# bad-samaritan/Polmux

Measured on AMD Instinct MI355X. Metric: dual-pol Gsample/s through SSFM+Rx-DSP, higher is better.
Workload: dtype f64

## Files before the change

include/polmux_hip.h:

```cpp
#ifndef POLMUX_HIP_H
#define POLMUX_HIP_H

#include <stddef.h>
#include <stdint.h>

#ifdef __cplusplus
extern "C" {
#endif

#define PLX_OK 0
#define PLX_ERR_HIP (-1)
#define PLX_ERR_ARG (-2)
#define PLX_ERR_UNSUPPORTED (-3)
#define PLX_ERR_REFERENCE (-4)
#define PLX_ERR_TIMEOUT (-5)

const char *plx_last_error(void);
int plx_abi_version(void);
int plx_device_count(int *count);
int plx_set_device(int device);

int plx_release_all(void);
int plx_gateway_stats(int64_t *out);
int plx_gateway_stats_ex(int64_t *out, int n);

int plx_fastexp(const double *x, double *yr, double *yi, size_t count);
int plx_fastexp_dev(const double *d_x, double *d_y, size_t count, void *stream);

typedef struct plx_ssfm_desc {
    int64_t nfft;
    int32_t nfc;
    int32_t dual_pol;
    int32_t max_frames;
    int32_t fls[4];
    double dzmaxt;
    double dphimaxt;
    double alphalin;
    double length;
    int32_t nplates;
    int32_t manakov;
    const double *gam;
    const double *betat;
    const double *db1;
} plx_ssfm_desc;

typedef struct plx_ssfm plx_ssfm;

int plx_ssfm_create(plx_ssfm **plan, const plx_ssfm_desc *desc);
#define PLX_SSFM_SHARE_DEVICE 1u
#define PLX_SSFM_XPM_MANAKOV 2u
int plx_ssfm_create_ex(plx_ssfm **plan, const plx_ssfm_desc *desc, uint32_t flags);
typedef struct plx_ssfm_tuning {
    uint32_t size;
    int32_t no_fuse;
    int32_t short_rows;
    int32_t no_row_split;
    int32_t p1, logW;
    int32_t col_threads;
    int32_t rowr;
    int32_t rowsm;
    int32_t row256_split, row4k_split, rowg_split;
    int32_t no_pmd_tab;
    int32_t store_late;
    int32_t row_rev;
    int32_t safe_landing;
    int32_t reserved_[4];
    double barrier_timeout_ms;
} plx_ssfm_tuning;
int plx_ssfm_tuning_defaults(plx_ssfm_tuning *tuning);
int plx_ssfm_tuning_override(const plx_ssfm_tuning *tuning);
int plx_ssfm_create_tuned(plx_ssfm **plan, const plx_ssfm_desc *desc, uint32_t flags, const plx_ssfm_tuning *tuning);
int plx_ssfm_destroy(plx_ssfm *plan);
int plx_ssfm_set_birefringence(plx_ssfm *plan, const double *db0, const double *theta,
                               const double *epsilon, int nsets);
int plx_ssfm_set_birefringence_dev(plx_ssfm *plan, const double *db0, const double *theta,
                                   const double *epsilon, int nsets, void *stream);
int plx_ssfm_propagate_dev(plx_ssfm *plan, double *d_ux, double *d_uy, int nframes, void *stream);
int plx_ssfm_set_step_sequence(plx_ssfm *plan, const double *dz, int nsteps);
int plx_ssfm_log_steps(plx_ssfm *plan, int max_steps);
int plx_ssfm_step_sequence(plx_ssfm *plan, int frame, double *dz, int max_steps);
int plx_ssfm_results(plx_ssfm *plan, int nframes, double *firstdz, int32_t *ncycle);
int plx_ssfm_stats(plx_ssfm *plan, int64_t *row_pass_launches, int64_t *sample_steps);
int plx_ssfm_utilisation(plx_ssfm *plan, int64_t *frame_steps, int64_t *slots_listed, int64_t *slots_launched);
int plx_ssfm_info(plx_ssfm *plan, int32_t *info);
int plx_ssfm_barrier_timeouts(plx_ssfm *plan, int32_t *count, int rearm);
int plx_ssfm_profile(plx_ssfm *plan, int enable);
int plx_ssfm_kernel_times(plx_ssfm *plan, double *ms, int64_t *launches);

int plx_matrix_ssfm(double *uxr, double *uxi, double *uyr, double *uyi, const plx_ssfm_desc *desc,
                    const double *db0, const double *theta, const double *epsilon,
                    double *firstdz, int32_t *ncycle);
int plx_scalar_ssfm(double *ur, double *ui, const plx_ssfm_desc *desc, double *firstdz, int32_t *ncycle);
int plx_scalar_ssfm_adaptive(double *ur, double *ui, const plx_ssfm_desc *desc, int tolflag, double ltol,
                             double safety, double *firstdz, int32_t *ncycle, int32_t *nrej);

typedef struct plx_cde plx_cde;
int plx_cde_create(plx_cde **plan, int64_t fft_len, int64_t L, const double *H_interleaved);
int plx_cde_destroy(plx_cde *plan);
int plx_cde_apply_dev(plx_cde *plan, const double *d_x, double *d_y, int64_t nx, int nsig, void *stream);
int plx_cde_ofde(const double *xr, const double *xi, const double *yr, const double *yi, int64_t nx,
                 double fs, double lambda_ref, double span, double D, double S, int64_t fft_len,
                 int64_t L, double *oxr, double *oxi, double *oyr, double *oyi);

typedef struct plx_dbp_desc {
    int64_t nfft;
    int32_t max_frames;
    int32_t nspans;
    int32_t nsteps;
    int32_t manakov;
    double span_length;
    double alphalin;
    double gam;
    double xi;
    const double *betat;
    const double *dz;
} plx_dbp_desc;
typedef struct plx_dbp_plan plx_dbp_plan;
#define PLX_DBP_STREAMED 1u
int plx_dbp_create(plx_dbp_plan **plan, const plx_dbp_desc *desc, uint32_t flags);
int plx_dbp_destroy(plx_dbp_plan *plan);
int plx_dbp_apply_dev(plx_dbp_plan *plan, const double *d_in, double *d_out, int nframes, const double *d_scale, void *stream);
int plx_dbp(const double *xr, const double *xi, const double *yr, const double *yi, int64_t nx, const plx_dbp_desc *desc,
            double scale, double *oxr, double *oxi, double *oyr, double *oyi);

int plx_cmaadaptivefilter(const double *xr, const double *xi, int32_t Mdim, double *h1r, double *h1i,
                          double *h2r, double *h2i, double Ntap, double mu, const double *R, double sps,
                          double *yr, double *yi);
int plx_easiadaptivefilter(const double *xr, const double *xi, int32_t Mdim, double *h1r, double *h1i,
                           double *h2r, double *h2i, double Ntap, double mu, double sps, double *yr,
                           double *yi);

int plx_cmaadaptivefilter_m(const double *xr, const double *xi, int32_t Mdim, double *h1r, double *h1i,
                            double *h2r, double *h2i, int32_t ntap, double mu, const double *R, double *yr, double *yi);
int plx_easiadaptivefilter_m(const double *xr, const double *xi, int32_t Mdim, double *h1r, double *h1i,
                             double *h2r, double *h2i, int32_t ntap, double mu, double *yr, double *yi);

int plx_cmapolardemux(const double *xr, const double *xi, int64_t L, int32_t taps, double mu, const double *R,
                      const double *M, double *yr, double *yi, double *h1r, double *h1i, double *h2r, double *h2i,
                      int32_t *passes);
int plx_easipolardemux(const double *xr, const double *xi, int64_t L, double mu, const double *M, int32_t mfile_twin,
                       double *yr, double *yi, double *h1r, double *h1i, double *h2r, double *h2i, int32_t *passes);

#define PLX_DEMUX_CMA 1
#define PLX_DEMUX_EASI 2
#define PLX_DEMUX_EASI_M 3
int plx_poldemux_dev(int method, const double *d_x, double *d_y, int64_t L, int nframes, int32_t taps,
                     double mu, const double *R , const double *d_M,
                     double *d_h, int32_t *d_passes, void *stream);

typedef struct plx_dsp_params {
    int32_t workatbaudrate;
    int32_t applynlr;
    double nlralpha;
    double power_mw;
    int32_t applypol;
    int32_t polmethod;
    double cma_R[2];
    double cma_mu;
    int32_t cma_taps;
    int32_t cma_txpolars;
    double cma_phizero;
    double easi_mu;
    int32_t easi_txpolars;
    double easi_phizero;
    int32_t modorder, freqavg, phasavg, poworder;
    int32_t cma_has_mat, easi_has_mat;
    double cma_mat[8], easi_mat[8];
    int32_t mfile_twins;
    int32_t reserved_;
} plx_dsp_params;

typedef struct plx_dsp plx_dsp;
int plx_dsp_create(plx_dsp **plan, int64_t Lin, int32_t ncol, int32_t max_frames, const plx_dsp_params *p);
int plx_dsp_destroy(plx_dsp *plan);
int plx_dsp_run_dev(plx_dsp *plan, const double *d_in, double *d_out, int nframes, void *stream);
int64_t plx_dsp_out_len(const plx_dsp *plan);

int plx_decide_count_dev(const double *d_sym, int64_t L, int32_t ncol, int nframes, const uint8_t *d_pat,
                         uint8_t *d_pat_hat, int64_t *d_err, void *stream);
int plx_decide_count_frames_dev(const double *d_sym, int64_t L, int32_t ncol, int nframes, const uint8_t *d_pat,
                                int64_t pat_frame_stride, uint8_t *d_pat_hat, int64_t *d_err, void *stream);

int plx_evm_dev(const double *d_sym, int64_t L, int32_t ncol, int nframes, double *d_evm, void *stream);

int plx_decide_count_dqpsk_dev(const double *d_sym, int64_t L, int32_t ncol, int nframes, const uint8_t *d_pat_rx,
                               int64_t pat_frame_stride, int64_t *d_err, void *stream);

int plx_ampliflat_dev(double *d_ux, double *d_uy, int64_t nfft, int32_t nfc, int nframes, double gain_lin,
                      const double *sigma, const double *d_noise, uint64_t seed, const int64_t *d_keys,
                      int32_t asex, int32_t asey, void *stream);

#define PLX_PHASE_TX 2
#define PLX_PHASE_LO 3
int plx_phase_noise_dev(double *d_ux, double *d_uy, int64_t stride, int64_t pitch, double sign, int64_t nfft,
                        int32_t nfc, int nframes, const double *sigma, uint64_t seed, const int64_t *d_keys,
                        int32_t tag, const double *d_phi_in, double *d_phi_out, double *d_work, void *stream);

int plx_wdm_mux_dev(const double *d_sx, const double *d_sy, double *d_ux, double *d_uy, int64_t nfft, int32_t nch,
                    int nframes, const int64_t *shift, void *stream);
int plx_wdm_select_dev(const double *d_ux, const double *d_uy, double *d_rx, double *d_ry, int64_t nfft, int32_t nch,
                       int nframes, const int64_t *shift, const int64_t *delay, void *stream);

typedef struct plx_front plx_front;
typedef struct plx_front_desc {
    int64_t nfft;
    int32_t dual_pol;
    int32_t max_frames;
    int32_t balanced;
    int32_t adcbits;
    int32_t decim;
    int32_t ntaps;
    const double *fir;
    const double *hopt_re, *hopt_im;
    const double *hel_re, *hel_im;
    const double *elo_re, *elo_im;
    double elo_scalar;
} plx_front_desc;
int plx_front_create(plx_front **plan, const plx_front_desc *desc);
int plx_front_destroy(plx_front *plan);
int64_t plx_front_out_len(const plx_front *plan);
int plx_front_run_dev(plx_front *plan, double *d_ux, double *d_uy, int nframes, const int64_t *shift,
                      double *d_out, void *stream);
int plx_front_run_lo_dev(plx_front *plan, double *d_ux, double *d_uy, int nframes, const int64_t *shift,
                         const double *d_lophase, double *d_out, void *stream);
int plx_rx_front(const double *xr, const double *xi, const double *yr, const double *yi, const plx_front_desc *desc,
                 const int64_t *shift, double *outr, double *outi, double *cur_r, double *cur_i);

typedef struct plx_filter plx_filter;
int plx_filter_create(plx_filter **plan, int64_t nfft, int max_signals, const double *h_re, const double *h_im);
int plx_filter_destroy(plx_filter *plan);
int plx_filter_apply_dev(plx_filter *plan, double *d_x, int nsignals, void *stream);

typedef struct plx_pmdinv plx_pmdinv;
int plx_pmdinv_create(plx_pmdinv **plan, int64_t nfft, int max_frames);
int plx_pmdinv_destroy(plx_pmdinv *plan);
int plx_pmdinv_set_link(plx_pmdinv *plan, int nfibers, const int32_t *ntrunk, const double *db0, const double *theta,
                        const double *epsilon, const double *lcorr, const double *betat, const double *db1,
                        const double *mat, int apply_gvd, int nsets);
int plx_pmdinv_apply_dev(plx_pmdinv *plan, double *d_ux, double *d_uy, int nframes, void *stream);
int plx_pmdinv_matrices(plx_pmdinv *plan, int frame, double *U, double *Uinv);

int plx_pick_dev(const double *d_in, double *d_out, int64_t n_in, int64_t n_out, int64_t offset,
                 int64_t stride, double scale, int nsig, int64_t out_pitch, void *stream);

#ifdef __cplusplus
}
#endif
#endif
```

polmux_amd/_abi.py:

```python
import ctypes as C
import os

_HERE = os.path.dirname(os.path.abspath(__file__))
LIB_PATH = os.path.join(_HERE, "lib", "libpolmux_hip.so")

PLX_OK = 0
PLX_ERR_HIP = -1
PLX_ERR_ARG = -2
PLX_ERR_UNSUPPORTED = -3
PLX_ERR_REFERENCE = -4
PLX_ERR_TIMEOUT = -5
PLX_SSFM_SHARE_DEVICE = 1
PLX_SSFM_XPM_MANAKOV = 2
PLX_DBP_STREAMED = 1
PLX_PHASE_TX = 2
PLX_PHASE_LO = 3


class PolmuxError(RuntimeError):
    def __init__(self, code, msg):
        super().__init__(msg)
        self.code = code


class SsfmDesc(C.Structure):
    _fields_ = [("nfft", C.c_int64), ("nfc", C.c_int32), ("dual_pol", C.c_int32), ("max_frames", C.c_int32),
                ("fls", C.c_int32 * 4), ("dzmaxt", C.c_double), ("dphimaxt", C.c_double),
                ("alphalin", C.c_double), ("length", C.c_double), ("nplates", C.c_int32),
                ("manakov", C.c_int32), ("gam", C.c_void_p), ("betat", C.c_void_p), ("db1", C.c_void_p)]


class SsfmTuning(C.Structure):
    _fields_ = [("size", C.c_uint32), ("no_fuse", C.c_int32), ("short_rows", C.c_int32), ("no_row_split", C.c_int32),
                ("p1", C.c_int32), ("logW", C.c_int32), ("col_threads", C.c_int32), ("rowr", C.c_int32), ("rowsm", C.c_int32),
                ("row256_split", C.c_int32), ("row4k_split", C.c_int32), ("rowg_split", C.c_int32), ("no_pmd_tab", C.c_int32),
                ("store_late", C.c_int32), ("row_rev", C.c_int32), ("safe_landing", C.c_int32), ("reserved_", C.c_int32 * 4),
                ("barrier_timeout_ms", C.c_double)]


class DspParams(C.Structure):
    _fields_ = [("workatbaudrate", C.c_int32), ("applynlr", C.c_int32), ("nlralpha", C.c_double),
                ("power_mw", C.c_double), ("applypol", C.c_int32), ("polmethod", C.c_int32),
                ("cma_R", C.c_double * 2), ("cma_mu", C.c_double), ("cma_taps", C.c_int32),
                ("cma_txpolars", C.c_int32), ("cma_phizero", C.c_double), ("easi_mu", C.c_double),
                ("easi_txpolars", C.c_int32), ("easi_phizero", C.c_double), ("modorder", C.c_int32),
                ("freqavg", C.c_int32), ("phasavg", C.c_int32), ("poworder", C.c_int32),
                ("cma_has_mat", C.c_int32), ("easi_has_mat", C.c_int32), ("cma_mat", C.c_double * 8),
                ("easi_mat", C.c_double * 8), ("mfile_twins", C.c_int32), ("reserved_", C.c_int32)]


class FrontDesc(C.Structure):
    _fields_ = [("nfft", C.c_int64), ("dual_pol", C.c_int32), ("max_frames", C.c_int32), ("balanced", C.c_int32),
                ("adcbits", C.c_int32), ("decim", C.c_int32), ("ntaps", C.c_int32), ("fir", C.c_void_p),
                ("hopt_re", C.c_void_p), ("hopt_im", C.c_void_p), ("hel_re", C.c_void_p), ("hel_im", C.c_void_p),
                ("elo_re", C.c_void_p), ("elo_im", C.c_void_p), ("elo_scalar", C.c_double)]


class DbpDesc(C.Structure):
    _fields_ = [("nfft", C.c_int64), ("max_frames", C.c_int32), ("nspans", C.c_int32), ("nsteps", C.c_int32),
                ("manakov", C.c_int32), ("span_length", C.c_double), ("alphalin", C.c_double), ("gam", C.c_double),
                ("xi", C.c_double), ("betat", C.c_void_p), ("dz", C.c_void_p)]


_vp, _i32, _i64, _dbl, _sz = C.c_void_p, C.c_int32, C.c_int64, C.c_double, C.c_size_t

SIGNATURES = {
    "plx_abi_version": [],
    "plx_device_count": [C.POINTER(C.c_int)],
    "plx_set_device": [C.c_int],
    "plx_release_all": [],
    "plx_gateway_stats": [_vp],
    "plx_gateway_stats_ex": [_vp, C.c_int],
    "plx_fastexp": [_vp, _vp, _vp, _sz],
    "plx_fastexp_dev": [_vp, _vp, _sz, _vp],
    "plx_ssfm_create": [C.POINTER(_vp), C.POINTER(SsfmDesc)],
    "plx_ssfm_create_ex": [C.POINTER(_vp), C.POINTER(SsfmDesc), C.c_uint32],
    "plx_ssfm_tuning_defaults": [C.POINTER(SsfmTuning)],
    "plx_ssfm_tuning_override": [C.POINTER(SsfmTuning)],
    "plx_ssfm_create_tuned": [C.POINTER(_vp), C.POINTER(SsfmDesc), C.c_uint32, C.POINTER(SsfmTuning)],
    "plx_ssfm_destroy": [_vp],
    "plx_ssfm_set_step_sequence": [_vp, _vp, C.c_int],
    "plx_ssfm_log_steps": [_vp, C.c_int],
    "plx_ssfm_step_sequence": [_vp, C.c_int, _vp, C.c_int],
    "plx_ssfm_set_birefringence": [_vp, _vp, _vp, _vp, C.c_int],
    "plx_ssfm_set_birefringence_dev": [_vp, _vp, _vp, _vp, C.c_int, _vp],
    "plx_ssfm_propagate_dev": [_vp, _vp, _vp, C.c_int, _vp],
    "plx_ssfm_results": [_vp, C.c_int, _vp, _vp],
    "plx_ssfm_stats": [_vp, C.POINTER(_i64), C.POINTER(_i64)],
    "plx_ssfm_info": [_vp, _vp],
    "plx_ssfm_utilisation": [_vp, C.POINTER(_i64), C.POINTER(_i64), C.POINTER(_i64)],
    "plx_ssfm_barrier_timeouts": [_vp, C.POINTER(_i32), C.c_int],
    "plx_ssfm_profile": [_vp, C.c_int],
    "plx_ssfm_kernel_times": [_vp, _vp, _vp],
    "plx_matrix_ssfm": [_vp, _vp, _vp, _vp, C.POINTER(SsfmDesc), _vp, _vp, _vp, C.POINTER(_dbl),
                        C.POINTER(_i32)],
    "plx_scalar_ssfm": [_vp, _vp, C.POINTER(SsfmDesc), C.POINTER(_dbl), C.POINTER(_i32)],
    "plx_scalar_ssfm_adaptive": [_vp, _vp, C.POINTER(SsfmDesc), C.c_int, _dbl, _dbl, C.POINTER(_dbl), C.POINTER(_i32),
                                 C.POINTER(_i32)],
    "plx_cde_create": [C.POINTER(_vp), _i64, _i64, _vp],
    "plx_cde_destroy": [_vp],
    "plx_cde_apply_dev": [_vp, _vp, _vp, _i64, C.c_int, _vp],
    "plx_cde_ofde": [_vp, _vp, _vp, _vp, _i64, _dbl, _dbl, _dbl, _dbl, _dbl, _i64, _i64, _vp, _vp, _vp, _vp],
    "plx_dbp_create": [C.POINTER(_vp), C.POINTER(DbpDesc), C.c_uint32],
    "plx_dbp_destroy": [_vp],
    "plx_dbp_apply_dev": [_vp, _vp, _vp, C.c_int, _vp, _vp],
    "plx_dbp": [_vp, _vp, _vp, _vp, _i64, C.POINTER(DbpDesc), _dbl, _vp, _vp, _vp, _vp],
    "plx_cmaadaptivefilter": [_vp, _vp, _i32, _vp, _vp, _vp, _vp, _dbl, _dbl, _vp, _dbl, _vp, _vp],
    "plx_easiadaptivefilter": [_vp, _vp, _i32, _vp, _vp, _vp, _vp, _dbl, _dbl, _dbl, _vp, _vp],
    "plx_cmaadaptivefilter_m": [_vp, _vp, _i32, _vp, _vp, _vp, _vp, _i32, _dbl, _vp, _vp, _vp],
    "plx_easiadaptivefilter_m": [_vp, _vp, _i32, _vp, _vp, _vp, _vp, _i32, _dbl, _vp, _vp],
    "plx_cmapolardemux": [_vp, _vp, _i64, _i32, _dbl, _vp, _vp, _vp, _vp, _vp, _vp, _vp, _vp, _vp],
    "plx_easipolardemux": [_vp, _vp, _i64, _dbl, _vp, _i32, _vp, _vp, _vp, _vp, _vp, _vp, _vp],
    "plx_poldemux_dev": [C.c_int, _vp, _vp, _i64, C.c_int, _i32, _dbl, _vp, _vp, _vp, _vp, _vp],
    "plx_dsp_create": [C.POINTER(_vp), _i64, _i32, _i32, C.POINTER(DspParams)],
    "plx_dsp_destroy": [_vp],
    "plx_dsp_run_dev": [_vp, _vp, _vp, C.c_int, _vp],
    "plx_dsp_out_len": [_vp],
    "plx_decide_count_dev": [_vp, _i64, _i32, C.c_int, _vp, _vp, _vp, _vp],
    "plx_decide_count_frames_dev": [_vp, _i64, _i32, C.c_int, _vp, _i64, _vp, _vp, _vp],
    "plx_evm_dev": [_vp, _i64, _i32, C.c_int, _vp, _vp],
    "plx_decide_count_dqpsk_dev": [_vp, _i64, _i32, C.c_int, _vp, _i64, _vp, _vp],
    "plx_ampliflat_dev": [_vp, _vp, _i64, _i32, C.c_int, _dbl, _vp, _vp, C.c_uint64, _vp, _i32, _i32, _vp],
    "plx_phase_noise_dev": [_vp, _vp, _i64, _i64, _dbl, _i64, _i32, C.c_int, _vp, C.c_uint64, _vp, _i32, _vp, _vp, _vp,
                            _vp],
    "plx_wdm_mux_dev": [_vp, _vp, _vp, _vp, _i64, _i32, C.c_int, _vp, _vp],
    "plx_wdm_select_dev": [_vp, _vp, _vp, _vp, _i64, _i32, C.c_int, _vp, _vp, _vp],
    "plx_front_create": [C.POINTER(_vp), C.POINTER(FrontDesc)],
    "plx_front_destroy": [_vp],
    "plx_front_out_len": [_vp],
    "plx_front_run_dev": [_vp, _vp, _vp, C.c_int, _vp, _vp, _vp],
    "plx_front_run_lo_dev": [_vp, _vp, _vp, C.c_int, _vp, _vp, _vp, _vp],
    "plx_rx_front": [_vp, _vp, _vp, _vp, C.POINTER(FrontDesc), _vp, _vp, _vp, _vp, _vp],
    "plx_filter_create": [C.POINTER(_vp), _i64, C.c_int, _vp, _vp],
    "plx_filter_destroy": [_vp],
    "plx_filter_apply_dev": [_vp, _vp, C.c_int, _vp],
    "plx_pmdinv_create": [C.POINTER(_vp), _i64, C.c_int],
    "plx_pmdinv_destroy": [_vp],
    "plx_pmdinv_set_link": [_vp, C.c_int, _vp, _vp, _vp, _vp, _vp, _vp, _vp, _vp, C.c_int, C.c_int],
    "plx_pmdinv_apply_dev": [_vp, _vp, _vp, C.c_int, _vp],
    "plx_pmdinv_matrices": [_vp, C.c_int, _vp, _vp],
    "plx_pick_dev": [_vp, _vp, _i64, _i64, _i64, _i64, _dbl, C.c_int, _i64, _vp],
}
_RESTYPES = {"plx_dsp_out_len": _i64, "plx_front_out_len": _i64}


class Binding:

    def __init__(self, path=None):
        path = path or LIB_PATH
        if not os.path.exists(path):
            raise PolmuxError(PLX_ERR_HIP,
                              "libpolmux_hip.so not found at %s: build it with "
                              "`python -c 'import __graft_entry__ as g; g.build()'` "
                              "(hipcc --offload-arch=gfx950); there is no CPU fallback" % path)
        self.path = path
        if os.path.basename(path) == "libpolmux_hip.so":
            import torch
        self.lib = C.CDLL(path)
        _BINDINGS.append(self)
        self.lib.plx_last_error.restype = C.c_char_p
        for name, args in SIGNATURES.items():
            fn = getattr(self.lib, name)
            fn.argtypes = args
            fn.restype = _RESTYPES.get(name, C.c_int)

    def tuning(self, **fields):
        t = SsfmTuning()
        self.call("plx_ssfm_tuning_defaults", C.byref(t))
        for k, v in fields.items():
            if k not in dict(SsfmTuning._fields_) or k in ("size", "reserved_"):
                raise KeyError("plx_ssfm_tuning has no field %r" % k)
            setattr(t, k, v)
        return t

    def last_error(self):
        return self.lib.plx_last_error().decode("utf-8", "replace")

    def call(self, name, *args):
        rc = getattr(self.lib, name)(*args)
        if rc != PLX_OK:
            raise PolmuxError(rc, self.last_error() or ("%s failed with code %d" % (name, rc)))
        return rc


_default = None
_BINDINGS = []


def bindings():
    return list(_BINDINGS)


def get():
    global _default
    if _default is None:
        _default = Binding()
    return _default
```

polmux_amd/csrc/ssfm_args.h:

```cpp
#pragma once
#include "plx_fft.h"
#include "plx_internal.h"

#define BRF_STRIDE 4

#ifdef PLX_EMU
#define ROWR_SYNC() __syncthreads()
#else
#define ROWR_SYNC() asm volatile("s_waitcnt lgkmcnt(0)" ::: "memory")
#endif

namespace plxs {

struct FrameCtl {
    double zprop, dz;
    double cur;
    double leff, att;
    double dz_miss;
    double firstdz;
    double dzb_first, dzb_last;
    int ntot, nmem, ntrunk;
    int started, last, ncycle;
    int pad_[7];
    int done;
};
static_assert(sizeof(FrameCtl) == 128 && offsetof(FrameCtl, done) == 124, "done is the last word of the last 16-byte piece");

struct SsfmArgs {
    cplx *ux, *uy;
    const double *betat_p, *db1_p;
    const cplx *tpass;
    const cplx *hmul;
    const cplx *umat;
    const cplx *tw1, *tw2;
    const cplx *ctab;
    const cplx *tw2c, *twmid;
    const double *gam;
    const double *brf;
    cplx *e1tab, *e2tab;
    double d1slope;
    int tmax;
    union {
        double *psum;
        cplx *stokes;
    };
    FrameCtl *ctl;
    unsigned long long *umax;
    int *ndone;
    const int *active;
    int *nactive;
    long long spin_ticks;
    unsigned long long *slots;
    int row_rev;
    int store_late;
    int safe_land;
    int round;
    int *grab;
    unsigned long long *mbox;
    int mbox_stride;
    int p1, p2, nfc, dual, W, logW, T, logT, R, logR;
    int spm, xpm, manakov, pmd, nplates, brf_per_frame;
    int nframes;
    int force;
    double f_cur, f_leff, f_sc;
    const double *dzlist;
    int ndz, logcap;
    double *dzlog;
    int resume, ncycle0;
    double dz0, zdone0;
    double alphalin, Lf, dzmax, dphimax, lcorr, invN;
};

__device__ __forceinline__ double wave_max(double v)
{
    for (int m = 32; m >= 1; m >>= 1) {
        double o = __shfl_xor(v, m, 64);
        v = o > v ? o : v;
    }
    return v;
}

template <class ARGS> __device__ __forceinline__ bool all_done_or_aborted(const ARGS &a) { return a.ndone[0] >= a.nframes || a.ndone[1] != 0; }

__device__ __forceinline__ bool slot_frame(const SsfmArgs &a, int slot, int &f)
{
    if (!a.active) { f = slot; return slot < a.nframes; }
    if (slot >= a.nactive[0]) return false;
    f = a.active[slot];
    return true;
}

__device__ __forceinline__ bool row_slot(const SsfmArgs &a, int &slot)
{
    if (!a.row_rev) return true;
    const int n = a.active ? a.nactive[0] : a.nframes;
    if (slot >= n) return false;
    slot = n - 1 - slot;
    return true;
}

__device__ __forceinline__ void sincos_small(double a, double *s, double *c)
{
    if (fabs(a) < 0.0625) {
        const double z = a * a;
        double ps = fma(z, -1.0 / 39916800.0, 1.0 / 362880.0);
        ps = fma(z, ps, -1.0 / 5040.0);
        ps = fma(z, ps, 1.0 / 120.0);
        ps = fma(z, ps, -1.0 / 6.0);
        *s = fma(a * z, ps, a);
        double pc = fma(z, 1.0 / 479001600.0, -1.0 / 3628800.0);
        pc = fma(z, pc, 1.0 / 40320.0);
        pc = fma(z, pc, -1.0 / 720.0);
        pc = fma(z, pc, 1.0 / 24.0);
        pc = fma(z, pc, -0.5);
        *c = fma(z, pc, 1.0);
    } else {
        sincos(a, s, c);
    }
}

__device__ __forceinline__ double div3(double x)
{
    const double c = 1.0 / 3.0;
    const double q = x * c;
    return fma(fma(-3.0, q, x), c, q);
}
__device__ __forceinline__ void sincos_taylor(double a, double *s, double *c)
{
    const double z = a * a;
    double ps = fma(z, 1.0 / 362880.0, -1.0 / 5040.0);
    ps = fma(z, ps, 1.0 / 120.0);
    ps = fma(z, ps, -1.0 / 6.0);
    *s = fma(a * z, ps, a);
    double pc = fma(z, 1.0 / 40320.0, -1.0 / 720.0);
    pc = fma(z, pc, 1.0 / 24.0);
    pc = fma(z, pc, -0.5);
    *c = fma(z, pc, 1.0);
}

__device__ __forceinline__ void block_atomic_max(double v, double *red, unsigned long long *dst, int tid, int nthr)
{
    v = wave_max(v);
    if ((tid & 63) == 0) red[tid >> 6] = v;
    __syncthreads();
    if (tid == 0) {
        double m = red[0];
        for (int w = 1; w < (nthr + 63) / 64; w++) m = red[w] > m ? red[w] : m;
        atomicMax(dst, (unsigned long long)__double_as_longlong(m));
    }
}

}
```

polmux_amd/csrc/ssfm_colx.hip:

```cpp
#include "ssfm_ctrl.h"
#include "ssfm_kernels.h"
using namespace plxs;

namespace {

__device__ __noinline__ double ctrl_head_call(const PLX_LDS_QUAL CtrlK *k, PLX_LDS_QUAL FrameCtl *rec, int count, double pmax, int f)
{
    if (!ctrl_head<true>(*k, f, *rec, true, pmax, count != 0)) return -1.0;
    return rec->leff;
}
__device__ __noinline__ void ctrl_tail_call(const PLX_LDS_QUAL CtrlK *k, PLX_LDS_QUAL FrameCtl *rec)
{
    ctrl_tail(*k, *rec);
}
__device__ __noinline__ void kerr_full_range(int j, int t, double gamleff, int manakov)
{
    PLX_DYN_LDS(lds);
    cplx *s = (cplx *)lds;
    for (int k = 0; k < 16; k++) {
        cplx X = s[((j + 16 * k) << 4) + t], Y = s[((j + 16 * k) << 4) + t + 8];
        const double P = X.x * X.x + X.y * X.y + Y.x * Y.x + Y.y * Y.y;
        const cplx nl = cexpi(-gamleff * P);
        X = cmul(X, nl);
        Y = cmul(Y, nl);
        if (!manakov) {
            const double s3 = 2 * (X.x * Y.y - X.y * Y.x);
            double sp, cp;
            sincos(gamleff * s3 / 3, &sp, &cp);
            const cplx xx = make_double2(cp * X.x + sp * Y.x, cp * X.y + sp * Y.y);
            const cplx yy = make_double2(cp * Y.x - sp * X.x, cp * Y.y - sp * X.y);
            X = xx; Y = yy;
        }
        s[((j + 16 * k) << 4) + t] = X;
        s[((j + 16 * k) << 4) + t + 8] = Y;
    }
}

__device__ __noinline__ void kerr_full_range_scalar(int j, int t, double gam, double leff)
{
    PLX_DYN_LDS(lds);
    cplx *s = (cplx *)lds;
    for (int k = 0; k < 16; k++) {
        const cplx X = s[((j + 16 * k) << 4) + t];
        const double pw = X.x * X.x + X.y * X.y;
        s[((j + 16 * k) << 4) + t] = cmul(X, cexpi(-gam * pw * leff));
    }
}

#define PLX_REC_SENTINEL 0x7fffffff
#ifdef PLX_EMU
__device__ __forceinline__ void glds16(const cplx *src, cplx *lds_wave_base, int lane) { lds_wave_base[lane] = *src; }
__device__ __forceinline__ void glds_rows(const cplx *src, size_t stride, cplx *lds_wave_base, int lane)
{
    for (int i = 0; i < 16; i++) glds16(src + i * stride, lds_wave_base + 64 * i, lane);
}
__device__ __forceinline__ void lds_barrier() { __syncthreads(); }
__device__ __forceinline__ int lds_peek(const int *p) { return *(const volatile int *)p; }
__device__ __forceinline__ void lds_settle() {}
__device__ __forceinline__ void emu_lockstep() { __syncthreads(); }
#else
__device__ __forceinline__ void glds16(const cplx *src, cplx *lds_wave_base, int)
{
    const unsigned lb = __builtin_amdgcn_readfirstlane((unsigned)(size_t)(__attribute__((address_space(3))) void *)lds_wave_base);
    asm volatile("s_mov_b32 m0, %1\n\ts_nop 0\n\tglobal_load_lds_dwordx4 %0, off" : : "v"(src), "s"(lb) : "memory", "m0");
}
__device__ __forceinline__ void glds_rows(const cplx *src, size_t stride, cplx *lds_wave_base, int)
{
    unsigned lb = __builtin_amdgcn_readfirstlane((unsigned)(size_t)(__attribute__((address_space(3))) void *)lds_wave_base);
    unsigned long long p = (unsigned long long)src;
    const unsigned long long st = (unsigned long long)stride * sizeof(cplx);
#define PLX_GLDS_STEP "s_mov_b32 m0, %1\n\ts_nop 0\n\tglobal_load_lds_dwordx4 %0, off\n\tv_lshl_add_u64 %0, %0, 0, %2\n\ts_add_u32 %1, %1, 0x400\n\t"
    asm volatile(PLX_GLDS_STEP PLX_GLDS_STEP PLX_GLDS_STEP PLX_GLDS_STEP PLX_GLDS_STEP PLX_GLDS_STEP PLX_GLDS_STEP PLX_GLDS_STEP
                 PLX_GLDS_STEP PLX_GLDS_STEP PLX_GLDS_STEP PLX_GLDS_STEP PLX_GLDS_STEP PLX_GLDS_STEP PLX_GLDS_STEP PLX_GLDS_STEP
                 : "+v"(p), "+s"(lb) : "s"(st) : "memory", "m0", "scc");
#undef PLX_GLDS_STEP
}
__device__ __forceinline__ void lds_barrier() { asm volatile("s_waitcnt lgkmcnt(0)\n\ts_barrier" ::: "memory"); }
__device__ __forceinline__ int lds_peek(const int *p)
{
    int v;
    asm volatile("ds_read_b32 %0, %1\n\ts_waitcnt lgkmcnt(0)" : "=v"(v) : "v"((unsigned)(size_t)(const __attribute__((address_space(3))) void *)p) : "memory");
    return v;
}
__device__ __forceinline__ void lds_settle() { asm volatile("s_waitcnt lgkmcnt(0)" ::: "memory"); }
__device__ __forceinline__ void emu_lockstep() {}
#endif


template <bool D> __global__ __launch_bounds__(256, 2) void k_colx16(SsfmArgs a, int tiles_x, int tiles_pf)
{
    constexpr int CW = D ? 8 : 16;
    PLX_DYN_LDS(lds);
    if (all_done_or_aborted(a)) return;
    const int tid = threadIdx.x, t = tid & 15, j = tid >> 4;
    const int N2 = 1 << a.p2;
    const int LOGN = a.p1 + a.p2;
    cplx *s = (cplx *)lds;
    cplx *tw = s + 4096;
    double *red = (double *)(tw + 128);
    FrameCtl *lctl = (FrameCtl *)(red + 32);
    lds_load_twiddles(tw, a.tw1, 128, tid, 256);
    cplx *const fld = (D && t >= 8) ? a.uy : a.ux;
    const int round = a.round;
    const int colt = D ? t & 7 : t;
    const bool isx = !D || t < 8;
    const int lane = tid & 63, row0 = (tid >> 6) * 64;
    const int nact = a.nactive[0];
    const int NT = gridDim.x / tiles_pf, team = blockIdx.x / tiles_pf, ti = blockIdx.x - team * tiles_pf;
    const int c = ti / tiles_x, bx = ti - c * tiles_x;
    const unsigned long long rtag = (unsigned long long)(((unsigned)round + 1u) & 0xfffffu) << 22;
    unsigned long long *const mbox = a.mbox + (size_t)a.mbox_stride * team;
    if (blockIdx.x == 0 && tid == 0) a.grab[(round & 1) ^ 1] = 0;
    auto post = [&](int k) {
        const int sl = NT + atomicAdd(a.grab + (round & 1), 1);
        const int fr = sl < nact ? a.active[sl] : -1;
        if (k < a.mbox_stride) st_agent(mbox + k, ((rtag | (unsigned long long)(k + 1)) << 22) | (unsigned long long)(fr + 1));
    };
    auto posted = [&](int k, unsigned long long v) -> bool { return (v >> 22) == (rtag | (unsigned long long)(k + 1)); };
    int it = 0;
    auto stage = [&](int f, int par) {
        const int fc = f * a.nfc + c;
        int lq = lane >> 4;
        pin(lq);
        const cplx *src = fld + ((size_t)fc << LOGN) + (size_t)bx * CW + colt + (size_t)(row0 + lq) * N2;
        FrameCtl *const rec = lctl + 4 * par + (tid >> 6);
        if (lane == (int)(offsetof(FrameCtl, done) / 16)) rec->done = PLX_REC_SENTINEL;
        lds_settle();
        glds_rows(src, (size_t)4 * N2, s + (size_t)row0 * 16, lane);
        static_assert(sizeof(FrameCtl) % 16 == 0, "the record travels as 16-byte pieces");
        int ln = lane;
        pin(ln);
        if (ln < (int)(sizeof(FrameCtl) / 16)) glds16((const cplx *)(a.ctl + f) + ln, (cplx *)rec, ln);
    };
    double *const gaml = (double *)((char *)(lctl + 8) + 128);
    for (int k = tid; k < a.nfc; k += 256) gaml[k] = a.gam[k];
    cplx *const twn = (cplx *)(gaml + COLX_NFC);
    if (D && tid < 128) { const cplx w = a.tw1[tid]; twn[tid] = make_double2(-w.x, -w.y); }
#define COLX_TWA(tp) ((D && (tp) >= 8) ? (const cplx *)twn : (const cplx *)tw)
#define COLX_HSW(tp) ((D && (tp) >= 8) ? 2048 : 0)
    int f = team < nact ? a.active[team] : -1;
    if (f < 0) return;
    stage(f, 0);
    if (ti == 0 && tid == 64) post(1);
    CtrlK *const kk = (CtrlK *)(lctl + 8);
    if (tid == 0) {
        red[8] = -1.0;
        kk->dphimax = a.dphimax; kk->alphalin = a.alphalin; kk->dzmax = a.dzmax; kk->dz0 = a.dz0; kk->zdone0 = a.zdone0; kk->Lf = a.Lf; kk->lcorr = a.lcorr;
        kk->dual = a.dual ? 1 : 0; kk->resume = a.resume ? 1 : 0; kk->ncycle0 = a.ncycle0; kk->nfc = 0; kk->ndone = a.ndone; kk->umax = nullptr; kk->gam = nullptr;
        kk->dzlist = a.dzlist; kk->dzlog = a.dzlog; kk->ndz = a.ndz; kk->logcap = a.logcap;
    }
    auto settle = [&](int par) {
        const int pf = (int)red[8];
        if (pf < 0) return;
        FrameCtl *pr = lctl + 4 * par;
        if (!pr->done) ctrl_tail_call((const PLX_LDS_QUAL CtrlK *)kk, (PLX_LDS_QUAL FrameCtl *)pr);
        a.ctl[pf] = *pr;
        red[8] = -1.0;
    };
    __syncthreads();
    for (;; it++) {
        FrameCtl *const wrec = lctl + 4 * (it & 1) + (tid >> 6);
        const int fc = f * a.nfc + c;
        if (a.safe_land) drain_vmem();
        while (lds_peek(&wrec->done) == PLX_REC_SENTINEL) nap();
        emu_lockstep();
        if (wrec->done) {
            if (tid == 0) {
                settle((it & 1) ^ 1);
                unsigned long long v;
                unsigned spins = 0;
                bool dead = false;
                const long long t0 = plx_clock();
                while (!posted(it + 1, v = ld_agent(mbox + (it + 1)))) {
                    nap();
                    if ((++spins & 255u) == 0 && (ld_agent((const unsigned *)a.ndone + 1) != 0 || plx_clock() - t0 > a.spin_ticks)) {
                        st_agent((unsigned *)a.ndone + 1, 1u);
                        dead = true;
                        break;
                    }
                }
                red[10 + (it & 1)] = dead ? -2.0 : (double)((int)(v & 0x3fffffull) - 1);
            } else if (ti == 0 && tid == 64) {
                post(it + 2);
            }
            lds_barrier();
            f = (int)red[10 + (it & 1)];
            if (f == -2) return;
            if (f < 0) { it++; break; }
            stage(f, (it & 1) ^ 1);
            continue;
        }
        const size_t cbase = ((size_t)fc << LOGN) + (size_t)bx * CW + colt;
        const bool started = wrec->started != 0;
        {
            cplx x[16];
#pragma unroll
            for (int k = 0; k < 16; k++) x[k] = s[((16 * j + k) << 4) + t];
            if (started) {
                r16_dit(x);
#pragma unroll
                for (int k = 0; k < 16; k++) s[((16 * j + k) << 4) + t] = x[k];
            }
        }
        lds_barrier();
        cplx y[16];
        {
            int tp = t;
            pin(tp);
            const int ysw = started ? 0 : COLX_HSW(tp);
#pragma unroll
            for (int k = 0; k < 8; k++) y[k] = s[((j + 16 * k) << 4) + t + ysw];
#pragma unroll
            for (int k = 8; k < 16; k++) y[k] = s[((j + 16 * k) << 4) + t - ysw];
        }
        double sc = 1.0;
        if (started) {
            lvl2_dit256s(y, j, tw, COLX_TWA(t));
            sc = wrec->att * a.invN;
        }
#pragma unroll
        for (int k = 0; k < 16; k++) y[k] = cscale(y[k], sc);
        double m = 0;
        if (!D) {
#pragma unroll
            for (int k = 0; k < 16; k++) m = fmax(fma(y[k].y, y[k].y, y[k].x * y[k].x), m);
        } else
#pragma unroll
        for (int k = 0; k < 8; k++) {
            const double po = fma(y[k].y, y[k].y, y[k].x * y[k].x);
            const double pq = fma(y[k + 8].y, y[k + 8].y, y[k + 8].x * y[k + 8].x);
            const double p = po + lane_xchg<8>(pq);
            m = fmax(p, m);
        }
        m = wave_max(m);
        if ((tid & 63) == 0) red[tid >> 6] = m;
        lds_barrier();
        if (tid < 64) {
            const unsigned par = (unsigned)round & 1u;
            unsigned long long *slots = a.slots + ((size_t)par * a.nframes + f) * tiles_pf;
            double mm = red[0];
            for (int w = 1; w < 4; w++) mm = red[w] > mm ? red[w] : mm;
            const unsigned long long mine = (unsigned long long)__double_as_longlong(mm);
            if (tid == 0) {
                st_agent(slots + ti, mine);
                st_agent(a.slots + ((size_t)(par ^ 1u) * a.nframes + f) * tiles_pf + ti, ~0ull);
                settle((it & 1) ^ 1);
            }
            double pm;
            unsigned long long mv = 0;
            unsigned spins = 0;
            bool dead = false;
            const long long t0 = plx_clock();
            for (;;) {
                bool all = true;
                pm = -INFINITY;
                if (tid == 0) { mv = ld_agent(mbox + (it + 1)); all = posted(it + 1, mv); }
                int i0 = tid;
                pin(i0);
                for (int i = i0; i < tiles_pf; i += 64) {
                    const unsigned long long b = (i == ti) ? mine : ld_agent(slots + i);
                    if (b == ~0ull) all = false;
                    else { const double gp = gaml[i / tiles_x] * __longlong_as_double((long long)b); pm = gp > pm ? gp : pm; }
                }
                if (__all(all)) break;
                nap();
                if ((++spins & 255u) == 0) {
                    const int late = ld_agent((const unsigned *)a.ndone + 1) != 0 || plx_clock() - t0 > a.spin_ticks;
                    if (__any(late)) { dead = true; break; }
                }
            }
            pm = wave_max(pm);
            if (tid == 0) {
                red[10 + (it & 1)] = (double)((int)(mv & 0x3fffffull) - 1);
                if (dead) {
                    st_agent((unsigned *)a.ndone + 1, 1u);
                    red[19] = 1.0;
                } else {
                    const double pv = ctrl_head_call((const PLX_LDS_QUAL CtrlK *)kk, (PLX_LDS_QUAL FrameCtl *)wrec, ti == 0, pm, f);
                    if (ti == 0) red[8] = (double)f;
                    red[16] = pv; red[17] = pv < 0 ? 1.0 : 0.0; red[18] = mm; red[19] = 0.0;
                }
            }
        } else if (ti == 0 && tid == 64) {
            post(it + 2);
        }
        lds_barrier();
        if (red[19] != 0.0) return;
        const double leff = red[16];
        const bool finished = red[17] != 0.0;
        if (finished) {
            const int nf = (int)red[10 + (it & 1)];
            if (nf >= 0) stage(nf, (it & 1) ^ 1);
            {
                int tq = t, jq = j;
                pin(tq);
                pin(jq);
                const int rsw = (D && tq >= 8) ? 128 : 0;
#pragma unroll
                for (int k = 0; k < 8; k++) fld[cbase + (size_t)(jq + 16 * k + rsw) * N2] = y[k];
#pragma unroll
                for (int k = 8; k < 16; k++) fld[cbase + (size_t)(jq + 16 * k - rsw) * N2] = y[k];
            }
        } else {
            if (!D) {
                if (a.spm) {
                    const double gam = gaml[c];
                    if (fabs(gam * leff) * red[18] < 0.0625) {
#pragma unroll
                        for (int k = 0; k < 16; k++) {
                            const double pw = y[k].x * y[k].x + y[k].y * y[k].y;
                            double sn, cs;
                            sincos_taylor(-gam * pw * leff, &sn, &cs);
                            y[k] = cmul(y[k], make_double2(cs, sn));
                        }
                    } else {
#pragma unroll
                        for (int k = 0; k < 16; k++) s[((j + 16 * k) << 4) + t] = y[k];
                        lds_barrier();
                        kerr_full_range_scalar(j, t, gam, leff);
                        lds_barrier();
#pragma unroll
                        for (int k = 0; k < 16; k++) y[k] = s[((j + 16 * k) << 4) + t];
                        lds_barrier();
                    }
                }
            } else if (a.spm) {
                const double gamleff = gaml[c] * leff;
                int tq = t;
                pin(tq);
                const double sgn = tq < 8 ? 1.0 : -1.0, sgn2 = tq < 8 ? 2.0 : -2.0;
                if (fabs(gamleff) * red[18] < 0.0625) {
                    auto kerr16 = [&](auto cn) {
                        constexpr bool CNLSE = decltype(cn)::value;
#pragma unroll
                        for (int k = 0; k < 8; k++) {
                            const cplx own = y[k], snd = y[k + 8];
                            const cplx oth = make_double2(lane_xchg<8>(snd.x), lane_xchg<8>(snd.y));
                            const double P = fma(own.y, own.y, own.x * own.x) + fma(oth.y, oth.y, oth.x * oth.x);
                            double sn, cs;
                            sincos_taylor(-gamleff * P, &sn, &cs);
                            const cplx nl = make_double2(cs, sn);
                            cplx A = cmul(own, nl), B = cmul(oth, nl);
                            if (CNLSE) {
                                const double s3 = sgn2 * __dsub_rn(__dmul_rn(A.x, B.y), __dmul_rn(A.y, B.x));
                                double sp, cp;
                                sincos_taylor(div3(gamleff * s3), &sp, &cp);
                                const double sg = sgn * sp, ng = -sg;
                                const cplx A2 = make_double2(cp * A.x + sg * B.x, cp * A.y + sg * B.y);
                                B = make_double2(cp * B.x + ng * A.x, cp * B.y + ng * A.y);
                                A = A2;
                            }
                            const cplx back = make_double2(lane_xchg<8>(B.x), lane_xchg<8>(B.y));
                            y[k] = A;
                            y[k + 8] = back;
                            sched_fence();
                        }
                    };
                    if (a.manakov) kerr16(std::false_type{}); else kerr16(std::true_type{});
                } else {
                    int tp = t;
                    pin(tp);
                    const int ksw = COLX_HSW(tp);
#pragma unroll
                    for (int k = 0; k < 8; k++) s[((j + 16 * k) << 4) + t + ksw] = y[k];
#pragma unroll
                    for (int k = 8; k < 16; k++) s[((j + 16 * k) << 4) + t - ksw] = y[k];
                    lds_barrier();
                    if (isx) kerr_full_range(j, t, gamleff, a.manakov);
                    lds_barrier();
#pragma unroll
                    for (int k = 0; k < 8; k++) y[k] = s[((j + 16 * k) << 4) + t + ksw];
#pragma unroll
                    for (int k = 8; k < 16; k++) y[k] = s[((j + 16 * k) << 4) + t - ksw];
                    lds_barrier();
                }
            }
            lvl2_dif256s(y, j, tw, COLX_TWA(t));
#pragma unroll
            for (int k = 0; k < 16; k++) s[((j + 16 * k) << 4) + t] = y[k];
            lds_barrier();
            cplx x[16];
#pragma unroll
            for (int k = 0; k < 16; k++) x[k] = s[((16 * j + k) << 4) + t];
            lds_barrier();
            {
                const int nf = (int)red[10 + (it & 1)];
                if (nf >= 0) stage(nf, (it & 1) ^ 1);
            }
            r16_dif(x);
            if (a.store_late) {
                const int nf = (int)red[10 + (it & 1)];
                if (nf >= 0) {
                    FrameCtl *const nrec = lctl + 4 * ((it & 1) ^ 1) + (tid >> 6);
                    while (lds_peek(&nrec->done) == PLX_REC_SENTINEL) nap();
                }
            }
#pragma unroll
            for (int k = 0; k < 16; k++) fld[cbase + (size_t)(16 * j + k) * N2] = x[k];
        }
        f = (int)red[10 + (it & 1)];
        if (f < 0) { it++; break; }
    }
    if (tid == 0) settle((it & 1) ^ 1);
}


}

namespace plxs {
colx_kernel_t colx16_kernel(bool dual) { return dual ? (colx_kernel_t)k_colx16<true> : (colx_kernel_t)k_colx16<false>; }
}
```

polmux_amd/csrc/ssfm_ctrl.h:

```cpp
#pragma once
#include "ssfm_args.h"

namespace plxs {

template <bool AGENT, class ARGS, class REC> __device__ __forceinline__ bool ctrl_head(const ARGS &a, int f, REC &c, bool have_pmax, double pmax_in, bool count = true)
{
    if (c.started) {
        if (a.dual) c.ntot = c.ntot + c.ntrunk - c.nmem;
        if (c.last) {
            c.done = 1;
            if (count) atomicAdd(a.ndone, 1);
            return false;
        }
    }
    double Pmax = -INFINITY;
    if (have_pmax) {
        Pmax = pmax_in;
    } else {
        for (int k = 0; k < a.nfc; k++) {
            unsigned long long *up = a.umax + f * a.nfc + k;
            const unsigned long long bits = AGENT ? ld_agent(up) : *up;
            double Umax = __longlong_as_double((long long)bits);
            double gp = a.gam[k] * Umax;
            Pmax = gp > Pmax ? gp : Pmax;
            if (AGENT) st_agent(up, 0ull); else *up = 0ull;
        }
    }
    double leffn = a.dphimax / Pmax;
    double dl = a.alphalin * leffn;
    double dz;
    if (dl >= 1) {
        dz = a.dzmax;
    } else {
        double step = (a.alphalin == 0) ? leffn : -1 / a.alphalin * log(1 - dl);
        dz = step > a.dzmax ? a.dzmax : step;
    }
    {
        const int k = c.started ? c.ncycle : 0;
        if (a.dzlist && k < a.ndz) dz = a.dzlist[k];
        if (a.dzlog && count && k < a.logcap) a.dzlog[(size_t)f * a.logcap + k] = dz;
    }
    if (!c.started) {
        c.started = 1;
        if (a.resume) {
            dz = a.dz0;
            c.firstdz = a.zdone0;
            c.zprop = a.zdone0 + dz;
            c.ncycle = a.ncycle0 + 1;
        } else {
            c.firstdz = dz;
            c.zprop = dz;
            c.ncycle = 1;
        }
    } else {
        c.zprop = c.zprop + dz;
        c.ncycle = c.ncycle + 1;
    }
    c.dz = dz;
    if (c.zprop < a.Lf) {
        c.cur = dz; c.last = 0;
    } else {
        c.cur = a.Lf - c.zprop + dz; c.last = 1;
    }
    c.leff = (a.alphalin == 0) ? c.cur : (1 - exp(-a.alphalin * c.cur)) / a.alphalin;
    return true;
}
template <class ARGS, class REC> __device__ __forceinline__ void ctrl_tail(const ARGS &a, REC &c)
{
    const double zc = c.last ? a.Lf : c.zprop;
    c.att = exp(-(0.5 * a.alphalin) * c.cur);
    if (a.dual) {
        const double lcorr = a.lcorr;
        int nzc = (int)ceil(zc / lcorr);
        if (c.dz_miss == 0) {
            c.nmem = 0;
            c.ntrunk = nzc - c.ntot;
            double dzlast = c.cur - lcorr * (c.ntrunk - 1);
            c.dzb_first = c.ntrunk > 1 ? lcorr : dzlast;
            c.dzb_last = dzlast;
            c.dz_miss = lcorr - dzlast;
        } else {
            c.nmem = 1;
            c.ntrunk = nzc - c.ntot + 1;
            if (c.ntrunk == 1) {
                c.dzb_first = c.cur; c.dzb_last = c.cur;
                c.dz_miss = c.dz_miss - c.cur;
            } else {
                double dzlast = c.cur - c.dz_miss - lcorr * (c.ntrunk - 2);
                c.dzb_first = c.dz_miss; c.dzb_last = dzlast;
                c.dz_miss = lcorr - dzlast;
            }
        }
    }
}
template <bool AGENT, class ARGS> __device__ __forceinline__ void ctrl_core(const ARGS &a, int f, FrameCtl &c, bool have_pmax, double pmax_in)
{
    if (c.done) return;
    if (ctrl_head<AGENT>(a, f, c, have_pmax, pmax_in)) ctrl_tail(a, c);
}
struct CtrlK {
    double dphimax, alphalin, dzmax, dz0, zdone0, Lf, lcorr;
    int dual, resume, ncycle0, nfc;
    int *ndone;
    unsigned long long *umax;
    const double *gam;
    const double *dzlist;
    double *dzlog;
    int ndz, logcap;
};
static_assert(sizeof(CtrlK) <= 128, "k_colx16 reserves 128 bytes of LDS for the constants");
template <bool AGENT> __device__ __forceinline__ void ctrl_step(const SsfmArgs &a, int f, bool have_pmax = false, double pmax_in = 0.0)
{
    FrameCtl c = a.ctl[f];
    if (c.done) return;
    ctrl_core<AGENT>(a, f, c, have_pmax, pmax_in);
    a.ctl[f] = c;
}

}
```

polmux_amd/csrc/ssfm_kernels.h:

```cpp
#pragma once
#include "ssfm_args.h"
#include <tuple>
#include <utility>

#define COMPACT_THREADS 256
#define COL_THREADS_MAX 1024
#define ROW_THREADS 128
#define ROWR_THREADS 64
#define ROWR_LDS ((4 * 272 + 128 + 48) * sizeof(cplx))
#define ROWR_LDS_SC ((4 * 272 + 128 + 80) * sizeof(cplx))
#define ROWG_THREADS 256
#define ROWG_NTW(M) ((M) <= 1024 ? (M) / 2 : (M) / 8 + 4)
#define ROWG_LDS(M) ((size_t)((ROWG_THREADS / ((M) / 16)) * ((M) + (M) / 16) + ROWG_NTW(M) + 7 * 16 + PLX_CTAB + 17 * (ROWG_THREADS / ((M) / 16))) * sizeof(cplx))
#define ROWG_LDS_SPLIT(M) (ROWG_LDS(M) - (size_t)((ROWG_THREADS / ((M) / 16)) * ((M) + (M) / 16)) * sizeof(double))
#define ROWSM_LDS ((size_t)64 * 17 * sizeof(double) + (7 * 16 + PLX_CTAB) * sizeof(cplx))
#define COLX_NFC 64

namespace plxs {

typedef void (*sweep_kernel_t)(SsfmArgs);
typedef void (*colx_kernel_t)(SsfmArgs, int, int);

PLX_HIDDEN sweep_kernel_t col_fwd_kernel();
PLX_HIDDEN sweep_kernel_t col_fwd_xpm_kernel();
PLX_HIDDEN sweep_kernel_t col_inv_kernel();
PLX_HIDDEN colx_kernel_t colx16_kernel(bool dual);
PLX_HIDDEN sweep_kernel_t row_kernel();
PLX_HIDDEN sweep_kernel_t row256_kernel(bool pmd, bool scalar, bool split);
PLX_HIDDEN sweep_kernel_t row4k_kernel(bool pair, bool split);
PLX_HIDDEN sweep_kernel_t rowreg_kernel(int logm, bool pair, bool scalar, bool split);
PLX_HIDDEN sweep_kernel_t rowsm_kernel(int logm, bool scalar);

PLX_HIDDEN void launch_umax(dim3 grid, hipStream_t st, const SsfmArgs &a);
PLX_HIDDEN void launch_ctrl(int nframes, hipStream_t st, const SsfmArgs &a);
PLX_HIDDEN void launch_compact(const FrameCtl *ctl, int nframes, int *active, int *nactive, int serves, hipStream_t st);
PLX_HIDDEN void launch_rowsum(dim3 grid, hipStream_t st, const SsfmArgs &a);
PLX_HIDDEN void launch_stokes_sum(dim3 grid, hipStream_t st, const SsfmArgs &a);
PLX_HIDDEN void launch_pmd_tab(unsigned frames, hipStream_t st, const SsfmArgs &a);
PLX_HIDDEN void launch_nl_att(unsigned grid, hipStream_t st, cplx *u, const double *gam, size_t N, int nfc, int spm, int xpm, double leff, double att);
PLX_HIDDEN void launch_maxdiff(unsigned grid, hipStream_t st, const cplx *u, const cplx *uh, size_t n, unsigned long long *out);
PLX_HIDDEN void launch_richardson(unsigned grid, hipStream_t st, cplx *u, const cplx *uh, size_t n);

#ifndef PLX_EMU
namespace detail {
template <class... P, size_t... I> inline void launch_ptr(void (*k)(P...), dim3 g, dim3 b, size_t lds, hipStream_t st, std::tuple<P...> &v, std::index_sequence<I...>)
{
    void *ptrs[] = {(void *)&std::get<I>(v)...};
    (void)hipLaunchKernel((const void *)k, g, b, ptrs, lds, st);
}
}
template <class... P, class... A> inline void launch(void (*k)(P...), dim3 g, dim3 b, size_t lds, hipStream_t st, A &&...args)
{
    std::tuple<P...> v{P(std::forward<A>(args))...};
    detail::launch_ptr(k, g, b, lds, st, v, std::index_sequence_for<P...>{});
}
template <class K> inline hipError_t allow_lds(K kern, size_t bytes)
{
    return hipFuncSetAttribute((const void *)kern, hipFuncAttributeMaxDynamicSharedMemorySize, (int)bytes);
}
template <class K> inline int blocks_per_cu(K kern, int threads, size_t lds)
{
    int nb = 0;
    if (hipOccupancyMaxActiveBlocksPerMultiprocessor(&nb, (const void *)kern, threads, lds) != hipSuccess) return 0;
    return nb;
}
#else
template <class... P, class... A> inline void launch(void (*k)(P...), dim3 g, dim3 b, size_t lds, hipStream_t, A &&...args)
{
    std::tuple<P...> v{P(std::forward<A>(args))...};
    emu::launch(g, b, lds, [=]() { std::apply(k, v); });
}
template <class K> inline hipError_t allow_lds(K, size_t) { return hipSuccess; }
template <class K> inline int blocks_per_cu(K, int, size_t) { return 2; }
#endif

}
```

polmux_amd/csrc/ssfm_plan.h:

```cpp
#pragma once
#include "ssfm_kernels.h"
#include <vector>

using plxs::FrameCtl;
using plxs::SsfmArgs;

struct plx_ssfm {
    plx_ssfm_desc d;
    int p, p1, p2;
    size_t N;
    SsfmArgs a;
    double *d_betat = nullptr, *d_db1 = nullptr, *d_gam = nullptr, *d_brf = nullptr, *d_psum = nullptr;
    cplx *d_tpass = nullptr, *d_tw1 = nullptr, *d_tw2 = nullptr, *d_ctab = nullptr;
    FrameCtl *d_ctl = nullptr;
    unsigned long long *d_umax = nullptr;
    int *d_ndone = nullptr;
    int *h_ndone = nullptr;
    int *d_active = nullptr;
    hipEvent_t ev = nullptr;
    std::vector<FrameCtl> h_ctl;
    int brf_sets = 0;
    size_t lds_col = 0, lds_row = 0;
    cplx *d_e1 = nullptr, *d_e2 = nullptr;
    unsigned long long *d_slots = nullptr;
    unsigned long long *d_mbox = nullptr;
    size_t mbox_bytes = 0;
    int fused = 0, fused_grid = 0, tiles_pf = 0;
    uint32_t flags = 0;
    int xpm_dual = 0;
    int barrier_timeouts = 0;
    int calls_unfused = 0, rearm_after = 16;
    double *d_dzlist = nullptr, *d_dzlog = nullptr;
    int dzlist_cap = 0;
    int col_threads = 512;
    int row_threads = ROW_THREADS;
    int rowr = 0;
    int row4k_split = 0;
    int rowsm = 0;
    int row256_split = 0;
    int rowg_pair_split = 0;
    int rowg_split = 0;
    int rowreg = 0;
    cplx *d_tw2c = nullptr, *d_twmid = nullptr;
    int row_split = 0, rs_threads = 0;
    size_t rs_lds = 0;
    int tw_compact = 0;
    int row_pair4k = 0;
    size_t rs_lds_pair = 0;
    double *h_brf[2] = {nullptr, nullptr};
    hipEvent_t brf_ev[2] = {nullptr, nullptr};
    int brf_slot = 0;
    int64_t row_launches = 0, sample_steps = 0;
    int64_t slots_launched = 0, slots_listed = 0, frame_steps = 0;
    int profile = 0;
    struct ProfRun { std::vector<hipEvent_t> ev; std::vector<int> cls, step; int maxnc = 0; bool fused = false; };
    std::vector<hipEvent_t> evfree;
    std::vector<ProfRun> prof_pending;
    double k_ms[4] = {0, 0, 0, 0};
    int64_t k_launches[4] = {0, 0, 0, 0};
};

PLX_HIDDEN int plx_ssfm_linear_dev(plx_ssfm *P, const SsfmArgs &base, cplx *d_x, double dz, hipStream_t st);

static const double kInv2Pi = 0.15915494309189533577;
```

polmux_amd/csrc/ssfm_plan.hip:

```cpp
#include "ssfm_plan.h"
#include "ssfm_ctrl.h"
#include "plx_gateway.h"

#include <cmath>
#include <cstdlib>
#include <cstring>
#include <limits>
#include <vector>
using namespace plxs;

static int ilog2(int64_t v)
{
    int l = 0;
    while (((int64_t)1 << l) < v) l++;
    return l;
}

static void free_plan(plx_ssfm *P)
{
    if (!P) return;
    hipFree(P->d_betat); hipFree(P->d_db1); hipFree(P->d_gam); hipFree(P->d_brf); hipFree(P->d_psum);
    hipFree(P->d_tpass); hipFree(P->d_tw1); hipFree(P->d_tw2); hipFree(P->d_ctab); hipFree(P->d_ctl); hipFree(P->d_umax);
    hipFree(P->d_dzlist); hipFree(P->d_dzlog); hipFree(P->d_tw2c); hipFree(P->d_twmid);
    hipFree(P->d_ndone); hipFree(P->d_slots); hipFree(P->d_mbox); hipFree(P->d_active); hipFree(P->d_e1); hipFree(P->d_e2);
    if (P->h_ndone) hipHostFree(P->h_ndone);
    if (P->ev) hipEventDestroy(P->ev);
    for (hipEvent_t e : P->evfree) hipEventDestroy(e);
    for (auto &r : P->prof_pending) for (hipEvent_t e : r.ev) hipEventDestroy(e);
    for (int k = 0; k < 2; k++) {
        if (P->h_brf[k]) hipHostFree(P->h_brf[k]);
        if (P->brf_ev[k]) hipEventDestroy(P->brf_ev[k]);
    }
    delete P;
}

static void half_table(std::vector<cplx> &t, int M)
{
    t.resize(M / 2 > 0 ? M / 2 : 1);
    for (int k = 0; k < M / 2; k++) {
        long double ang = -2.0L * 3.14159265358979323846264338327950288L * (long double)k / (long double)M;
        t[k] = make_double2((double)cosl(ang), (double)sinl(ang));
    }
}


namespace {
plx_ssfm_tuning g_override;
bool g_have_override = false;
}

extern "C" int plx_ssfm_tuning_defaults(plx_ssfm_tuning *t)
{
    if (!t) PLX_FAIL(PLX_ERR_ARG, "plx_ssfm_tuning_defaults: null argument");
    std::memset(t, 0, sizeof(*t));
    t->size = (uint32_t)sizeof(*t);
    t->p1 = -1; t->logW = -1; t->col_threads = -1; t->store_late = -1;
    t->row_rev = 1; t->rowr = 1; t->rowsm = 1; t->row256_split = 1; t->row4k_split = 1; t->rowg_split = 1;
    t->barrier_timeout_ms = 500.0;
    if (const char *e = getenv("PLX_SSFM_NO_FUSE")) t->no_fuse = atoi(e);
    if (const char *e = getenv("PLX_SSFM_BARRIER_TIMEOUT_MS")) t->barrier_timeout_ms = atof(e);
    return PLX_OK;
}

extern "C" int plx_ssfm_tuning_override(const plx_ssfm_tuning *t)
{
    if (t && t->size != sizeof(plx_ssfm_tuning)) PLX_FAIL(PLX_ERR_ARG, "plx_ssfm_tuning_override: fill the struct with plx_ssfm_tuning_defaults first");
    g_have_override = t != nullptr;
    if (t) g_override = *t;
    return PLX_OK;
}

extern "C" int plx_ssfm_create(plx_ssfm **out, const plx_ssfm_desc *desc) { return plx_ssfm_create_tuned(out, desc, 0u, nullptr); }

extern "C" int plx_ssfm_create_ex(plx_ssfm **out, const plx_ssfm_desc *desc, uint32_t flags) { return plx_ssfm_create_tuned(out, desc, flags, nullptr); }

extern "C" int plx_ssfm_create_tuned(plx_ssfm **out, const plx_ssfm_desc *desc, uint32_t flags, const plx_ssfm_tuning *tuning)
{
    if (!out || !desc) PLX_FAIL(PLX_ERR_ARG, "plx_ssfm_create: null argument");
    if (flags & ~(uint32_t)(PLX_SSFM_SHARE_DEVICE | PLX_SSFM_XPM_MANAKOV)) PLX_FAIL(PLX_ERR_ARG, "plx_ssfm_create_ex: unknown flag");
    *out = nullptr;
    const int64_t N = desc->nfft;
    const int p = ilog2(N);
    if (N < 256 || ((int64_t)1 << p) != N || p > 20)
        PLX_FAIL(PLX_ERR_UNSUPPORTED, "plx_ssfm_create: nfft must be a power of two in [256, 2^20]");
    if (desc->nfc < 1 || desc->max_frames < 1) PLX_FAIL(PLX_ERR_ARG, "plx_ssfm_create: nfc and max_frames must be >= 1");
    if (!desc->gam || !desc->betat) PLX_FAIL(PLX_ERR_ARG, "plx_ssfm_create: gam and betat are required");
    const bool xpm_dual = desc->dual_pol && desc->fls[3] && desc->nfc > 1;
    if (xpm_dual && !((flags & PLX_SSFM_XPM_MANAKOV) && desc->manakov))
        PLX_FAIL(PLX_ERR_REFERENCE, "The CNLSE with separate fields is not yet implemented");
    if (desc->dual_pol && desc->fls[3] && desc->nfc == 1) {  }
    if (desc->nplates < 1) PLX_FAIL(PLX_ERR_ARG, "plx_ssfm_create: nplates must be >= 1");
    if (tuning && tuning->size != sizeof(plx_ssfm_tuning)) PLX_FAIL(PLX_ERR_ARG, "plx_ssfm_create_tuned: fill the struct with plx_ssfm_tuning_defaults first");
    plx_ssfm_tuning tune;
    if (tuning) tune = *tuning;
    else if (g_have_override) tune = g_override;
    else plx_ssfm_tuning_defaults(&tune);
    if (flags & PLX_SSFM_SHARE_DEVICE) tune.no_fuse = 1;
    if (xpm_dual) tune.no_fuse = 1;

    plx_ssfm *P = new plx_ssfm();
    P->d = *desc;
    P->flags = flags;
    P->p = p;
    int logW;
    {
        const int npol = desc->dual_pol ? 2 : 1;
        logW = desc->dual_pol ? 3 : 4;
        int p1 = 12 - (logW + (npol == 2 ? 1 : 0));
        const bool long_rows = !tune.no_row_split && !tune.short_rows;
        const int p2max = long_rows ? 12 : 11;
        if (p - p1 > p2max) p1 = p - p2max;
        if (p1 > p - 4) p1 = p - 4;
        if (p1 < 2) p1 = 2;
        while ((((size_t)1 << p1) << (logW + (npol == 2 ? 1 : 0))) * sizeof(cplx) > 128 * 1024 && logW > 3) logW--;
        if (tune.p1 >= 2 && tune.p1 <= p - 4) p1 = tune.p1;
        if (tune.logW >= 2 && tune.logW <= 6) logW = tune.logW;
        while (((int64_t)1 << (p - p1)) < ((int64_t)1 << logW)) logW--;
        P->p1 = p1;
    }
    P->p2 = p - P->p1;
    P->N = (size_t)N;
    const int N1 = 1 << P->p1, N2 = 1 << P->p2;
    const int nfc = desc->nfc, F = desc->max_frames;
    SsfmArgs &a = P->a;
    std::memset(&a, 0, sizeof(a));
    a.p1 = P->p1; a.p2 = P->p2; a.nfc = nfc; a.dual = desc->dual_pol ? 1 : 0;
    a.logW = logW; a.W = 1 << a.logW;
    a.logT = a.logW + (a.dual ? 1 : 0); a.T = 1 << a.logT;
    {
        int R = 1, npol = a.dual ? 2 : 1;
        while (R * npol * (N2 / 16) < ROW_THREADS / 2 && R * 2 <= N1) R *= 2;
        a.R = R; a.logR = ilog2(R);
        int rowthr = ROW_THREADS;
        const int64_t pts = (int64_t)npol * R * N2;
        while (rowthr < 1024 && (int64_t)rowthr * 8 < pts) rowthr *= 2;
        P->row_threads = rowthr;
    }
    P->tw_compact = P->p2 >= 12 ? 1 : 0;
    if (a.dual && (N2 >= 2048 && !tune.no_row_split)) {
        P->row_split = 1;
        P->rs_threads = N2 / 8 < ROW_THREADS ? ROW_THREADS : (N2 / 8 > 1024 ? 1024 : N2 / 8);
        P->rs_lds = ((size_t)(N2 + N2 / 16) + (P->tw_compact ? N2 / 8 + 4 + 16 + 160 + PLX_CTAB : N2 / 2)) * sizeof(cplx);
    }
    if (P->tw_compact && !a.dual && !tune.no_row_split) P->rs_lds = ((size_t)(N2 + N2 / 16) + N2 / 8 + 4 + 16 + 160 + PLX_CTAB) * sizeof(cplx);
    if (P->tw_compact && !P->row_split && a.dual) {
        free_plan(P);
        PLX_FAIL(PLX_ERR_UNSUPPORTED, "plx_ssfm_create: 4096-point rows need the one-polarisation row pass (PLX_SSFM_NO_ROW_SPLIT is set)");
    }
    if (P->tw_compact) {
        P->row_pair4k = desc->fls[1] ? 1 : 0;
        P->rs_lds_pair = P->rs_lds + (size_t)(N2 + N2 / 16) * sizeof(cplx);
    }
    a.spm = desc->fls[2]; a.xpm = desc->fls[3]; a.manakov = desc->manakov ? 1 : 0; a.pmd = desc->fls[1] ? 1 : 0;
    a.nplates = desc->nplates;
    a.alphalin = desc->alphalin; a.Lf = desc->length; a.dzmax = desc->dzmaxt; a.dphimax = desc->dphimaxt;
    a.lcorr = desc->length / desc->nplates;
    a.invN = 1.0 / (double)N;
    a.spin_ticks = (long long)(tune.barrier_timeout_ms * 1e5);
    a.safe_land = tune.safe_landing;
    a.row_rev = tune.row_rev;
    if ((int64_t)desc->max_frames + 4 >= ((int64_t)1 << 22)) { free_plan(P); PLX_FAIL(PLX_ERR_UNSUPPORTED, "plx_ssfm_create: max_frames must be below 2^22 - 4"); }

    std::vector<double> bt((size_t)nfc * N), d1;
    std::vector<cplx> tp((size_t)N);
    const bool have_db1 = desc->db1 != nullptr && a.dual;
    if (have_db1) d1.resize((size_t)nfc * N);
    for (int j = 0; j < N1; j++) {
        const unsigned k1 = plx_bitrev((unsigned)j, P->p1);
        for (int i = 0; i < N2; i++) {
            const unsigned k2 = plx_bitrev((unsigned)i, P->p2);
            const size_t k = (size_t)k1 + (size_t)N1 * k2, pos = (size_t)j * N2 + i;
            for (int c = 0; c < nfc; c++) {
                bt[(size_t)c * N + pos] = desc->betat[(size_t)c * N + k] * kInv2Pi;
                if (have_db1) d1[(size_t)c * N + pos] = desc->db1[(size_t)c * N + k] * kInv2Pi;
            }
            const uint64_t e = ((uint64_t)i * k1) & (uint64_t)(N - 1);
            long double ang = -2.0L * 3.14159265358979323846264338327950288L * (long double)e / (long double)N;
            tp[pos] = make_double2((double)cosl(ang), (double)sinl(ang));
        }
    }
    std::vector<cplx> t1, t2;
    half_table(t1, N1);
    if (P->tw_compact) {
        t2.resize(N2 / 8 + 4);
        for (int k = 0; k < N2 / 8 + 4; k++) {
            const int e = k < N2 / 8 ? 4 * k : k - N2 / 8;
            long double ang = -2.0L * 3.14159265358979323846264338327950288L * (long double)e / (long double)N2;
            t2[k] = make_double2((double)cosl(ang), (double)sinl(ang));
        }
    } else {
        half_table(t2, N2);
    }
    std::vector<double> gam(nfc);
    for (int c = 0; c < nfc; c++) gam[c] = (a.dual && a.manakov) ? desc->gam[c] * 8 / 9 : desc->gam[c];

#define UP(dst, vec, T)                                                                             \
    do {                                                                                            \
        if (hipMalloc((void **)&(dst), (vec).size() * sizeof(T)) != hipSuccess ||                   \
            hipMemcpy((dst), (vec).data(), (vec).size() * sizeof(T), hipMemcpyHostToDevice) != hipSuccess) { \
            free_plan(P);                                                                           \
            PLX_FAIL(PLX_ERR_HIP, "plx_ssfm_create: device allocation/upload failed");              \
        }                                                                                           \
    } while (0)
    UP(P->d_betat, bt, double);
    if (have_db1) UP(P->d_db1, d1, double);
    UP(P->d_tpass, tp, cplx);
    UP(P->d_tw1, t1, cplx);
    UP(P->d_tw2, t2, cplx);
    {
        std::vector<cplx> ctv(PLX_CTAB);
        for (int k = 0; k < PLX_CTAB; k++) {
            const long double ang = 2.0L * 3.14159265358979323846264338327950288L * (long double)k / (long double)PLX_CTAB;
            ctv[k] = make_double2((double)cosl(ang), (double)-sinl(ang));
        }
        UP(P->d_ctab, ctv, cplx);
    }
    const int rowsm_min = a.dual ? (tune.rowsm == 2 ? 5 : 7) : 5;
    if (tune.rowr && tune.rowsm && !desc->fls[1] && P->p2 >= rowsm_min && P->p2 <= 7 && (N1 * (a.dual ? 2 : 1)) % (64 / (N2 / 16)) == 0) {
        const long double tau = -2.0L * 3.14159265358979323846264338327950288L;
        std::vector<cplx> tm(7 * 16, make_double2(1.0, 0.0));
        const int R = N2 / 16;
        auto put = [&](int q, int j, int e, int m) { tm[16 * q + j] = make_double2((double)cosl(tau * e / m), (double)sinl(tau * e / m)); };
        for (int j = 0; j < 16; j++) {
            if (R == 2) put(0, j, j, 32);
            const int q0 = R == 8 ? 4 : 0;
            if (R >= 4) for (int q = 0; q < 3; q++) put(q0 + q, j, (q + 1) * j, 64);
            if (R == 8) for (int q = 0; q < 4; q++) put(q, j, j + 16 * q, 128);
        }
        UP(P->d_twmid, tm, cplx);
        if (allow_lds(rowsm_kernel(P->p2, !a.dual), ROWSM_LDS) == hipSuccess) P->rowsm = 1;
    }
    if (tune.rowr && P->p2 >= 9 && P->p2 <= 11 && N1 >= (ROWG_THREADS / (N2 / 16)) / (a.dual ? 2 : 1)) {
        const long double tau = -2.0L * 3.14159265358979323846264338327950288L;
        std::vector<cplx> tc(N2 / 8 + 4), tm(7 * 16, make_double2(1.0, 0.0));
        for (int k = 0; k < N2 / 8 + 4; k++) {
            const int e = k < N2 / 8 ? 4 * k : k - N2 / 8;
            tc[k] = make_double2((double)cosl(tau * e / N2), (double)sinl(tau * e / N2));
        }
        const int R = N2 / 256;
        auto put = [&](int q, int j, int e, int m) { tm[16 * q + j] = make_double2((double)cosl(tau * e / m), (double)sinl(tau * e / m)); };
        for (int j = 0; j < 16; j++) {
            if (R == 2) put(0, j, j, 32);
            const int q0 = R == 8 ? 4 : 0;
            if (R >= 4) for (int q = 0; q < 3; q++) put(q0 + q, j, (q + 1) * j, 64);
            if (R == 8) for (int q = 0; q < 4; q++) put(q, j, j + 16 * q, 128);
        }
        UP(P->d_tw2c, tc, cplx);
        UP(P->d_twmid, tm, cplx);
        const size_t lds_whole = ROWG_LDS((size_t)N2), lds_split = ROWG_LDS_SPLIT((size_t)N2);
        hipError_t e = allow_lds(rowreg_kernel(P->p2, false, false, false), lds_whole);
        if (e == hipSuccess) e = allow_lds(rowreg_kernel(P->p2, true, false, false), lds_whole);
        if (e == hipSuccess) e = allow_lds(rowreg_kernel(P->p2, false, true, false), lds_whole);
        if (e == hipSuccess) P->rowreg = 1;
        if (P->rowreg && tune.rowg_split) {
            if (allow_lds(rowreg_kernel(P->p2, false, !a.dual, true), lds_split) == hipSuccess) P->rowg_split = 1;
            if (P->rowg_split && a.dual && allow_lds(rowreg_kernel(P->p2, true, false, true), lds_split) == hipSuccess) P->rowg_pair_split = 1;
        }
    }
    UP(P->d_gam, gam, double);
#undef UP
    bool ok = hipMalloc((void **)&P->d_ctl, sizeof(FrameCtl) * F) == hipSuccess &&
              hipMalloc((void **)&P->d_umax, sizeof(unsigned long long) * F * nfc) == hipSuccess &&
              hipMalloc((void **)&P->d_ndone, 64) == hipSuccess &&
              hipMalloc((void **)&P->d_active, sizeof(int) * (size_t)F) == hipSuccess &&
              hipHostMalloc((void **)&P->h_ndone, 64, hipHostMallocDefault) == hipSuccess &&
              hipEventCreateWithFlags(&P->ev, hipEventDisableTiming) == hipSuccess;
    if (ok && !a.dual && a.xpm) ok = hipMalloc((void **)&P->d_psum, sizeof(double) * (size_t)F * N) == hipSuccess;
    P->xpm_dual = xpm_dual ? 1 : 0;
    if (ok && xpm_dual) ok = hipMalloc((void **)&P->d_psum, sizeof(double) * 4 * (size_t)F * N) == hipSuccess;
    if (!ok) { free_plan(P); PLX_FAIL(PLX_ERR_HIP, "plx_ssfm_create: device allocation failed"); }
    a.betat_p = P->d_betat; a.db1_p = P->d_db1; a.tpass = P->d_tpass; a.tw1 = P->d_tw1; a.tw2 = P->d_tw2; a.ctab = P->d_ctab; a.tw2c = P->d_tw2c; a.twmid = P->d_twmid;
    a.gam = P->d_gam; a.ctl = P->d_ctl; a.umax = P->d_umax; a.ndone = P->d_ndone; a.psum = P->d_psum;
    P->h_ctl.resize(F);

    P->lds_col = (((size_t)N1 << a.logT) + N1 / 2) * sizeof(cplx) + 32 * sizeof(double) + 8 * sizeof(FrameCtl) + 128 + COLX_NFC * sizeof(double) + 128 * sizeof(cplx);
    P->lds_row = ((size_t)(a.dual ? 2 : 1) * a.R * (N2 + N2 / 16) + N2 / 2) * sizeof(cplx);
    P->col_threads = P->lds_col > 80 * 1024 ? 1024 : 512;
    if (tune.col_threads == 128 || tune.col_threads == 256 || tune.col_threads == 512 || tune.col_threads == 1024) P->col_threads = tune.col_threads;
    if (allow_lds(colx16_kernel(true), P->lds_col) != hipSuccess || allow_lds(colx16_kernel(false), P->lds_col) != hipSuccess || allow_lds(col_fwd_kernel(), P->lds_col) != hipSuccess ||
        allow_lds(col_inv_kernel(), P->lds_col) != hipSuccess || (P->xpm_dual && allow_lds(col_fwd_xpm_kernel(), P->lds_col) != hipSuccess) ||
        (!P->tw_compact && allow_lds(row_kernel(), P->lds_row > P->rs_lds ? P->lds_row : P->rs_lds) != hipSuccess) ||
        (P->tw_compact && (allow_lds(row4k_kernel(false, false), P->rs_lds) != hipSuccess || allow_lds(row4k_kernel(true, false), P->rs_lds_pair) != hipSuccess ||
                           allow_lds(row4k_kernel(false, true), P->rs_lds) != hipSuccess))) {
        free_plan(P);
        PLX_FAIL(PLX_ERR_HIP, "plx_ssfm_create: cannot reserve LDS for the transform kernels");
    }
    P->row4k_split = (P->tw_compact && tune.row4k_split) ? 1 : 0;
    if (tune.rowr && a.dual && a.p1 == 8 && a.p2 == 8 && !P->row_split &&
        allow_lds(row256_kernel(a.pmd != 0, false, false), ROWR_LDS) == hipSuccess) P->rowr = 1;
    if (tune.rowr && !a.dual && a.p1 == 8 && a.p2 == 8 && allow_lds(row256_kernel(false, true, false), ROWR_LDS_SC) == hipSuccess) P->rowr = 1;
    if (P->rowr && a.dual && a.pmd && tune.row256_split && allow_lds(row256_kernel(true, false, true), ROWR_LDS) == hipSuccess) P->row256_split = 1;
    if (((a.dual && a.W == 8) || (!a.dual && a.W == 16 && !desc->fls[3])) && !tune.no_fuse && a.p1 == 8 && nfc <= COLX_NFC) {
        int ncu = 256;
        {
            int dev = 0, v = 0;
            if (hipGetDevice(&dev) == hipSuccess && hipDeviceGetAttribute(&v, hipDeviceAttributeMultiprocessorCount, dev) == hipSuccess && v > 0)
                ncu = v;
        }
        const int tiles_pf = nfc * (N2 / a.W);
        const int per_cu = blocks_per_cu(colx16_kernel(a.dual != 0), 256, P->lds_col);
        const int cap = ncu * per_cu;
        if (tiles_pf <= cap) {
            P->fused = 1;
            P->tiles_pf = tiles_pf;
            P->fused_grid = (cap / tiles_pf) * tiles_pf;
            a.store_late = tune.store_late >= 0 ? (tune.store_late ? 1 : 0) : (P->fused_grid > tiles_pf ? 1 : 0);
            const int mstride = F + 4;
            P->mbox_bytes = sizeof(unsigned long long) * ((size_t)mstride * (P->fused_grid / tiles_pf) + 1);
            if (hipMalloc((void **)&P->d_slots, sizeof(unsigned long long) * 2 * (size_t)F * tiles_pf) != hipSuccess ||
                hipMalloc((void **)&P->d_mbox, P->mbox_bytes) != hipSuccess) {
                free_plan(P);
                PLX_FAIL(PLX_ERR_HIP, "plx_ssfm_create: device allocation failed");
            }
            a.slots = P->d_slots;
            a.mbox = P->d_mbox;
            a.mbox_stride = mstride;
            a.grab = (int *)(P->d_mbox + (size_t)mstride * (P->fused_grid / tiles_pf));
        }
    }
    if (a.pmd && have_db1 && !tune.no_pmd_tab) {
        const double D = desc->db1[1] * kInv2Pi;
        bool lin = D != 0.0 && N >= 4;
        for (int c = 0; c < nfc && lin; c++)
            for (int64_t k = 0; k < N && lin; k++) {
                const double m = (double)(k < N / 2 ? k : k - N);
                if (fabs(desc->db1[(size_t)c * N + k] * kInv2Pi - D * m) > 4e-15 * fabs(D) * (double)N) lin = false;
            }
        if (lin) {
            const int tmax = (int)ceil(desc->dzmaxt / a.lcorr) + 2;
            const size_t n1 = (size_t)F * tmax * N1, n2 = (size_t)F * tmax * N2;
            if (tmax <= 64 && (n1 + n2) * sizeof(cplx) <= ((size_t)4 << 30)) {
                if (hipMalloc((void **)&P->d_e1, n1 * sizeof(cplx)) != hipSuccess || hipMalloc((void **)&P->d_e2, n2 * sizeof(cplx)) != hipSuccess) {
                    free_plan(P);
                    PLX_FAIL(PLX_ERR_HIP, "plx_ssfm_create: device allocation failed (trunk phasor tables)");
                }
                a.e1tab = P->d_e1; a.e2tab = P->d_e2; a.d1slope = D; a.tmax = tmax;
            }
        }
    }
    if (a.pmd && !a.dual) { free_plan(P); PLX_FAIL(PLX_ERR_ARG, "plx_ssfm_create: PMD needs a dual-polarisation plan"); }
    if (!a.pmd) {
        double z = 0;
        int rc = plx_ssfm_set_birefringence(P, &z, &z, &z, 1);
        if (rc) { free_plan(P); return rc; }
    }
    *out = P;
    return PLX_OK;
}

extern "C" int plx_ssfm_destroy(plx_ssfm *P)
{
    free_plan(P);
    return PLX_OK;
}

static int set_brf(plx_ssfm *P, const double *db0, const double *theta, const double *epsilon, int nsets, hipStream_t st,
                   bool wait)
{
    if (!P || !db0 || !theta || !epsilon) PLX_FAIL(PLX_ERR_ARG, "plx_ssfm_set_birefringence: null argument");
    if (nsets < 1 || (nsets != 1 && nsets > P->d.max_frames)) PLX_FAIL(PLX_ERR_ARG, "plx_ssfm_set_birefringence: more sets than frames");
    const int np = P->d.nplates;
    const size_t cap = (size_t)P->d.max_frames * np * BRF_STRIDE, cnt = (size_t)nsets * np * BRF_STRIDE;
    if (!P->d_brf) PLX_HIP(hipMalloc((void **)&P->d_brf, cap * sizeof(double)));
    const int slot = P->brf_slot;
    P->brf_slot ^= 1;
    if (!P->h_brf[slot]) {
        PLX_HIP(hipHostMalloc((void **)&P->h_brf[slot], cap * sizeof(double), hipHostMallocDefault));
        PLX_HIP(hipEventCreateWithFlags(&P->brf_ev[slot], hipEventDisableTiming));
    } else {
        PLX_HIP(hipEventSynchronize(P->brf_ev[slot]));
    }
    double *t = P->h_brf[slot];
    for (int sidx = 0; sidx < nsets; sidx++)
        for (int n = 0; n < np; n++) {
            const size_t i = (size_t)sidx * np + n;
            const double ct = cos(theta[i]), sn = sin(theta[i]), ce = cos(epsilon[i]), se = sin(epsilon[i]);
            const double r11x = ct * ce, r11y = -sn * se, r12x = -sn * ce, r12y = ct * se;
            const double r21x = sn * ce, r21y = ct * se, r22x = ct * ce, r22y = sn * se;
            double *m = &t[i * BRF_STRIDE];
            m[0] = (r11x * r11x + r11y * r11y) - (r12x * r12x + r12y * r12y);
            m[1] = (r11x * r21x + r11y * r21y) - (r12x * r22x + r12y * r22y);
            m[2] = (r11y * r21x - r11x * r21y) - (r12y * r22x - r12x * r22y);
            m[3] = db0[i] * kInv2Pi;
        }
    PLX_HIP(hipMemcpyAsync(P->d_brf, t, cnt * sizeof(double), hipMemcpyHostToDevice, st));
    PLX_HIP(hipEventRecord(P->brf_ev[slot], st));
    if (wait) PLX_HIP(hipStreamSynchronize(st));
    P->a.brf = P->d_brf;
    P->a.brf_per_frame = nsets > 1 ? 1 : 0;
    P->brf_sets = nsets;
    return PLX_OK;
}

extern "C" int plx_ssfm_set_birefringence(plx_ssfm *P, const double *db0, const double *theta,
                                          const double *epsilon, int nsets)
{
    return set_brf(P, db0, theta, epsilon, nsets, nullptr, true);
}

extern "C" int plx_ssfm_set_birefringence_dev(plx_ssfm *P, const double *db0, const double *theta,
                                              const double *epsilon, int nsets, void *stream)
{
    return set_brf(P, db0, theta, epsilon, nsets, (hipStream_t)stream, false);
}

static void launch_row(plx_ssfm *P, const SsfmArgs &a, unsigned FC, hipStream_t st)
{
    const int N1 = 1 << a.p1, N2 = 1 << a.p2;
    if (P->tw_compact && !a.dual) {
        if (P->row4k_split) launch(row4k_kernel(false, true), dim3((unsigned)N1 * FC), dim3(256), P->rs_lds - 4352 * sizeof(double), st, a);
        else launch(row4k_kernel(false, false), dim3((unsigned)N1 * FC), dim3(256), P->rs_lds, st, a);
        return;
    }
    if (P->tw_compact && a.dual && (a.pmd || a.umat)) {
        launch(row4k_kernel(true, false), dim3((unsigned)N1 * FC), dim3(512), P->rs_lds_pair, st, a);
        return;
    }
    if (P->rowsm && !a.pmd && !a.umat) {
        const dim3 g((unsigned)(N1 * (a.dual ? 2 : 1) / (64 / (N2 / 16))), FC), bs(64);
        launch(rowsm_kernel(a.p2, !a.dual), g, bs, ROWSM_LDS, st, a);
        return;
    }
    if (P->rowreg && !a.dual) {
        const dim3 g((unsigned)(N1 / (ROWG_THREADS / (N2 / 16))), FC), bs(ROWG_THREADS);
        if (P->rowg_split) launch(rowreg_kernel(a.p2, false, true, true), g, bs, ROWG_LDS_SPLIT((size_t)N2), st, a);
        else launch(rowreg_kernel(a.p2, false, true, false), g, bs, ROWG_LDS((size_t)N2), st, a);
        return;
    }
    if (P->rowreg && a.dual) {
        const unsigned gx = (unsigned)(N1 / ((ROWG_THREADS / (N2 / 16)) / 2));
        const dim3 g(gx, FC), bs(ROWG_THREADS);
        if (a.pmd && !a.umat && a.e1tab && P->rowg_split && P->rowg_pair_split)
            launch(rowreg_kernel(a.p2, true, false, true), g, bs, ROWG_LDS_SPLIT((size_t)N2), st, a);
        else if (a.pmd || a.umat)
            launch(rowreg_kernel(a.p2, true, false, false), g, bs, ROWG_LDS((size_t)N2), st, a);
        else if (P->rowg_split)
            launch(rowreg_kernel(a.p2, false, false, true), g, bs, ROWG_LDS_SPLIT((size_t)N2), st, a);
        else
            launch(rowreg_kernel(a.p2, false, false, false), g, bs, ROWG_LDS((size_t)N2), st, a);
        return;
    }
    if (P->row_split && a.dual && !a.pmd) {
        SsfmArgs b = a;
        b.dual = 0; b.R = 1; b.logR = 0;
        const dim3 gs((unsigned)N1, FC), bs((unsigned)P->rs_threads);
        if (P->tw_compact) {
            if (P->row4k_split) launch(row4k_kernel(false, true), dim3(gs.x * gs.y * 2u), dim3(256), P->rs_lds - 4352 * sizeof(double), st, b);
            else launch(row4k_kernel(false, false), dim3(gs.x * gs.y * 2u), dim3(256), P->rs_lds, st, b);
            return;
        }
        for (int pol = 0; pol < 2; pol++) {
            if (pol) b.ux = a.uy;
            launch(row_kernel(), gs, bs, P->rs_lds, st, b);
        }
        return;
    }
    if (P->rowr && !a.dual && !a.force && !a.hmul) {
        launch(row256_kernel(false, true, false), dim3(64u, FC), dim3(ROWR_THREADS), ROWR_LDS_SC, st, a);
        return;
    }
    if (P->rowr && a.dual && !a.force && !a.hmul && !a.umat) {
        if (a.pmd && P->row256_split && a.e1tab) launch(row256_kernel(true, false, true), dim3(128u, FC), dim3(ROWR_THREADS), ROWR_LDS - 4 * 272 * sizeof(double), st, a);
        else launch(row256_kernel(a.pmd != 0, false, false), dim3(128u, FC), dim3(ROWR_THREADS), ROWR_LDS, st, a);
        return;
    }
    launch(row_kernel(), dim3((unsigned)(N1 / a.R), FC), dim3((unsigned)P->row_threads), P->lds_row, st, a);
}

static int resolve_profiles(plx_ssfm *P)
{
    for (auto &r : P->prof_pending) {
        for (size_t i = 0; i + 1 < r.ev.size(); i++) {
            const int cls = r.cls[i], step = r.step[i];
            const bool active = (r.fused && cls == 0) ? step <= r.maxnc : step < r.maxnc;
            if (!active) continue;
            float ms = 0;
            PLX_HIP(hipEventElapsedTime(&ms, r.ev[i], r.ev[i + 1]));
            P->k_ms[cls] += ms;
            P->k_launches[cls]++;
        }
        for (hipEvent_t e : r.ev) P->evfree.push_back(e);
    }
    P->prof_pending.clear();
    return PLX_OK;
}

static int propagate_frames(plx_ssfm *P, cplx *d_ux, cplx *d_uy, int nframes, hipStream_t st)
{
    SsfmArgs a = P->a;
    const int nfc = a.nfc, N2 = 1 << a.p2;
    a.ux = d_ux;
    a.uy = d_uy;
    a.nframes = nframes;
    a.active = P->d_active;
    a.nactive = P->d_ndone + 2;
    unsigned FC = (unsigned)nframes * nfc;
    PLX_HIP(hipMemsetAsync(a.ctl, 0, sizeof(FrameCtl) * nframes, st));
    PLX_HIP(hipMemsetAsync(a.umax, 0, sizeof(unsigned long long) * FC, st));
    PLX_HIP(hipMemsetAsync(P->d_ndone, 0, 64, st));
    const bool fused = P->fused != 0;
    if (fused) {
        PLX_HIP(hipMemsetAsync(P->d_slots, 0xFF, sizeof(unsigned long long) * 2 * (size_t)nframes * P->tiles_pf, st));
        PLX_HIP(hipMemsetAsync(P->d_mbox, 0, P->mbox_bytes, st));
    } else {
        unsigned gx = (unsigned)((P->N + 255) / 256);
        if (gx > 64) gx = 64;
        launch_umax(dim3(gx, FC), st, a);
    }
    const dim3 blk(256);
    const dim3 bcol((unsigned)P->col_threads);
    const bool compact_every_step = nframes >= 64;
    int chunk = 4, steps = 0;
    const int kMaxSteps = 1 << 19;
    bool pending = false, aborted = false;
    struct ProfGuard {
        plx_ssfm *P;
        plx_ssfm::ProfRun run;
        ~ProfGuard() { for (hipEvent_t e : run.ev) P->evfree.push_back(e); }
    } guard{P, {}};
    plx_ssfm::ProfRun &run = guard.run;
    auto mark = [&](int cls, int step) -> int {
        if (!P->profile) return PLX_OK;
        hipEvent_t e;
        if (!P->evfree.empty()) { e = P->evfree.back(); P->evfree.pop_back(); }
        else PLX_HIP(hipEventCreate(&e));
        run.ev.push_back(e); run.cls.push_back(cls); run.step.push_back(step);
        PLX_HIP(hipEventRecord(e, st));
        return PLX_OK;
    };
#define PLX_MARK(cls, step) do { int rc_ = mark((cls), (step)); if (rc_) return rc_; } while (0)
    for (;;) {
        for (int sidx = 0; sidx < chunk; sidx++) {
            const dim3 gcol((unsigned)(N2 / a.W), FC);
            P->slots_launched += FC / nfc;
            if (fused) {
                const int tcx = (int)gcol.x, tct = (int)(gcol.x * FC);
                const dim3 gx((unsigned)(tct < P->fused_grid ? tct : P->fused_grid));
                if (compact_every_step || sidx == 0) {
                    PLX_MARK(3, steps + sidx);
                    launch_compact(a.ctl, nframes, P->d_active, P->d_ndone + 2, compact_every_step ? 1 : chunk, st);
                }
#ifdef PLX_EMU
                emu::g_concurrency = emu::starve_barriers() ? 1 : P->tiles_pf;
#endif
                a.round = steps + sidx;
                PLX_MARK(0, steps + sidx);
                launch(colx16_kernel(a.dual != 0), gx, blk, P->lds_col, st, a, tcx, P->tiles_pf);
#ifdef PLX_EMU
                emu::g_concurrency = 1;
#endif
                if (a.e1tab) {
                    PLX_MARK(3, steps + sidx);
                    launch_pmd_tab(FC / nfc, st, a);
                }
                PLX_MARK(1, steps + sidx);
                launch_row(P, a, FC, st);
                P->row_launches++;
                continue;
            }
            PLX_MARK(3, steps + sidx);
            launch_ctrl(nframes, st, a);
            if (compact_every_step || sidx == 0)
                launch_compact(a.ctl, nframes, P->d_active, P->d_ndone + 2, compact_every_step ? 1 : chunk, st);
            if (!a.dual && a.xpm) {
                unsigned gx = (unsigned)((P->N + 255) / 256);
                if (gx > 256) gx = 256;
                launch_rowsum(dim3(gx, (unsigned)nframes), st, a);
            }
            if (P->xpm_dual) {
                unsigned gx = (unsigned)((P->N + 255) / 256);
                if (gx > 256) gx = 256;
                launch_stokes_sum(dim3(gx, (unsigned)nframes), st, a);
            }
            if (a.e1tab) launch_pmd_tab(FC / nfc, st, a);
            PLX_MARK(0, steps + sidx);
            launch(P->xpm_dual ? col_fwd_xpm_kernel() : col_fwd_kernel(), gcol, bcol, P->lds_col, st, a);
            PLX_MARK(1, steps + sidx);
            launch_row(P, a, FC, st);
            PLX_MARK(2, steps + sidx);
            launch(col_inv_kernel(), gcol, bcol, P->lds_col, st, a);
            P->row_launches++;
        }
        PLX_MARK(3, steps + chunk);
        if (steps == 0 && !P->prof_pending.empty()) {
            const int rc_ = resolve_profiles(P);
            if (rc_) return rc_;
        }
        steps += chunk;
        if (pending) {
            PLX_HIP(hipEventSynchronize(P->ev));
            if (P->h_ndone[1]) { aborted = true; break; }
            if (P->h_ndone[0] >= nframes) break;
            const unsigned live = (unsigned)(nframes - P->h_ndone[0]) * nfc;
            if (live < FC) FC = live;
        }
        PLX_HIP(hipMemcpyAsync(P->h_ndone, P->d_ndone, 4 * sizeof(int), hipMemcpyDeviceToHost, st));
        PLX_HIP(hipEventRecord(P->ev, st));
        pending = true;
        if (chunk > 8) chunk = 4;
        else if (chunk < (compact_every_step ? 8 : 16)) chunk *= 2;
        if (steps > kMaxSteps) PLX_FAIL(PLX_ERR_HIP, "plx_ssfm_propagate_dev: step loop did not terminate");
    }
    PLX_HIP(hipMemcpyAsync(P->h_ctl.data(), a.ctl, sizeof(FrameCtl) * nframes, hipMemcpyDeviceToHost, st));
    PLX_HIP(hipMemcpyAsync(P->h_ndone, P->d_ndone, 4 * sizeof(int), hipMemcpyDeviceToHost, st));
    PLX_HIP(hipStreamSynchronize(st));
    P->slots_listed += P->h_ndone[3];
    if (aborted || P->h_ndone[1]) {
        P->barrier_timeouts++;
        P->fused = 0;
        PLX_FAIL(PLX_ERR_TIMEOUT, "plx_ssfm_propagate_dev: frame barrier timed out (the workgroups of a frame were not co-resident: "
                                  "another kernel holds the GPU); nothing was stored after the time-out and the field of this call is "
                                  "INVALID -- the plan now takes the barrier-free three-sweep step: restore the field and call again, "
                                  "or create such plans with plx_ssfm_create_ex(..., PLX_SSFM_SHARE_DEVICE)");
    }
    int maxnc = 0;
    for (int f = 0; f < nframes; f++) {
        P->frame_steps += P->h_ctl[f].ncycle + (fused ? 1 : 0);
        if (!P->h_ctl[f].done) PLX_FAIL(PLX_ERR_HIP, "plx_ssfm_propagate_dev: a frame did not reach the fibre end");
        P->sample_steps += (int64_t)P->h_ctl[f].ncycle * (int64_t)P->N * nfc;
        if (P->h_ctl[f].ncycle > maxnc) maxnc = P->h_ctl[f].ncycle;
    }
    if (!run.ev.empty()) {
        run.maxnc = maxnc; run.fused = fused;
        P->prof_pending.push_back(std::move(run));
        run.ev.clear();
    }
#undef PLX_MARK
    return PLX_OK;
}

extern "C" int plx_ssfm_propagate_dev(plx_ssfm *P, double *d_ux, double *d_uy, int nframes, void *stream)
{
    if (!P || !d_ux) PLX_FAIL(PLX_ERR_ARG, "plx_ssfm_propagate_dev: null argument");
    if (nframes < 1 || nframes > P->d.max_frames) PLX_FAIL(PLX_ERR_ARG, "plx_ssfm_propagate_dev: nframes out of range");
    if (P->a.dual && !d_uy) PLX_FAIL(PLX_ERR_ARG, "plx_ssfm_propagate_dev: dual-polarisation plan needs d_uy");
    if (P->a.brf_per_frame && P->brf_sets < nframes)
        PLX_FAIL(PLX_ERR_ARG, "plx_ssfm_propagate_dev: fewer birefringence sets than frames");
    P->slots_launched = 0; P->slots_listed = 0; P->row_launches = 0; P->sample_steps = 0; P->frame_steps = 0;
    const int rc = propagate_frames(P, (cplx *)d_ux, (cplx *)d_uy, nframes, (hipStream_t)stream);
    if (rc) return rc;
    PLX_HIP(hipGetLastError());
    return PLX_OK;
}

extern "C" int plx_ssfm_set_step_sequence(plx_ssfm *P, const double *dz, int nsteps)
{
    if (!P || nsteps < 0 || (nsteps > 0 && !dz)) PLX_FAIL(PLX_ERR_ARG, "plx_ssfm_set_step_sequence: bad argument");
    if (nsteps > P->dzlist_cap) {
        if (P->d_dzlist) { (void)hipFree(P->d_dzlist); P->d_dzlist = nullptr; P->dzlist_cap = 0; }
        PLX_HIP(hipMalloc((void **)&P->d_dzlist, sizeof(double) * (size_t)nsteps));
        P->dzlist_cap = nsteps;
    }
    if (nsteps > 0) PLX_HIP(hipMemcpy(P->d_dzlist, dz, sizeof(double) * (size_t)nsteps, hipMemcpyHostToDevice));
    P->a.dzlist = nsteps > 0 ? P->d_dzlist : nullptr;
    P->a.ndz = nsteps;
    return PLX_OK;
}

extern "C" int plx_ssfm_log_steps(plx_ssfm *P, int max_steps)
{
    if (!P || max_steps < 0) PLX_FAIL(PLX_ERR_ARG, "plx_ssfm_log_steps: bad argument");
    if (P->d_dzlog) { (void)hipFree(P->d_dzlog); P->d_dzlog = nullptr; }
    P->a.dzlog = nullptr; P->a.logcap = 0;
    if (max_steps > 0) {
        PLX_HIP(hipMalloc((void **)&P->d_dzlog, sizeof(double) * (size_t)max_steps * P->d.max_frames));
        P->a.dzlog = P->d_dzlog; P->a.logcap = max_steps;
    }
    return PLX_OK;
}

extern "C" int plx_ssfm_step_sequence(plx_ssfm *P, int frame, double *dz, int max_steps)
{
    if (!P || !dz || frame < 0 || frame >= P->d.max_frames || max_steps < 0) PLX_FAIL(PLX_ERR_ARG, "plx_ssfm_step_sequence: bad argument");
    if (!P->d_dzlog) PLX_FAIL(PLX_ERR_ARG, "plx_ssfm_step_sequence: no log (plx_ssfm_log_steps)");
    const int n = max_steps < P->a.logcap ? max_steps : P->a.logcap;
    PLX_HIP(hipMemcpy(dz, P->d_dzlog + (size_t)frame * P->a.logcap, sizeof(double) * (size_t)n, hipMemcpyDeviceToHost));
    return PLX_OK;
}

extern "C" int plx_ssfm_utilisation(plx_ssfm *P, int64_t *frame_steps, int64_t *slots_listed, int64_t *slots_launched)
{
    if (!P) PLX_FAIL(PLX_ERR_ARG, "plx_ssfm_utilisation: null plan");
    if (frame_steps) *frame_steps = P->frame_steps;
    if (slots_listed) *slots_listed = P->slots_listed;
    if (slots_launched) *slots_launched = P->slots_launched;
    return PLX_OK;
}

extern "C" int plx_ssfm_info(plx_ssfm *P, int32_t *info)
{
    if (!P || !info) PLX_FAIL(PLX_ERR_ARG, "plx_ssfm_info: null argument");
    info[0] = P->fused; info[1] = P->p1; info[2] = P->p2; info[3] = P->fused_grid; info[4] = P->tiles_pf;
    info[5] = P->col_threads; info[6] = (P->rowr || P->rowsm) ? ROWR_THREADS : P->rowreg ? ROWG_THREADS : (P->tw_compact ? (P->row_pair4k ? 512 : 256) : (P->row_split ? P->rs_threads : P->row_threads)); info[7] = (P->rowreg || P->rowsm) ? 2 : (P->row_pair4k ? 0 : ((P->tw_compact && !P->a.dual) ? 1 : P->row_split));
    return PLX_OK;
}

extern "C" int plx_ssfm_barrier_timeouts(plx_ssfm *P, int32_t *count, int rearm)
{
    if (!P) PLX_FAIL(PLX_ERR_ARG, "plx_ssfm_barrier_timeouts: null plan");
    if (count) *count = P->barrier_timeouts;
    if (rearm && !P->fused && P->fused_grid > 0 && P->tiles_pf > 0) { P->fused = 1; P->calls_unfused = 0; }
    return PLX_OK;
}

extern "C" int plx_ssfm_profile(plx_ssfm *P, int enable)
{
    if (!P) PLX_FAIL(PLX_ERR_ARG, "plx_ssfm_profile: null plan");
    P->profile = enable ? 1 : 0;
    return PLX_OK;
}

extern "C" int plx_ssfm_kernel_times(plx_ssfm *P, double *ms, int64_t *launches)
{
    if (!P || !ms || !launches) PLX_FAIL(PLX_ERR_ARG, "plx_ssfm_kernel_times: null argument");
    const int rc = resolve_profiles(P);
    if (rc) return rc;
    for (int k = 0; k < 4; k++) { ms[k] = P->k_ms[k]; launches[k] = P->k_launches[k]; P->k_ms[k] = 0; P->k_launches[k] = 0; }
    return PLX_OK;
}

int plx_ssfm_filter_table(plx_ssfm *P, const double *h_re, const double *h_im, cplx **d_out)
{
    if (!P || !h_re || !d_out) PLX_FAIL(PLX_ERR_ARG, "filter table: null argument");
    const int N1 = 1 << P->p1, N2 = 1 << P->p2;
    std::vector<cplx> h(P->N);
    for (int j = 0; j < N1; j++) {
        const unsigned k1 = plx_bitrev((unsigned)j, P->p1);
        for (int i = 0; i < N2; i++) {
            const size_t k = (size_t)k1 + (size_t)N1 * plx_bitrev((unsigned)i, P->p2);
            h[(size_t)j * N2 + i] = make_double2(h_re[k], h_im ? h_im[k] : 0.0);
        }
    }
    cplx *d = nullptr;
    if (hipMalloc((void **)&d, P->N * sizeof(cplx)) != hipSuccess ||
        hipMemcpy(d, h.data(), P->N * sizeof(cplx), hipMemcpyHostToDevice) != hipSuccess) {
        if (d) (void)hipFree(d);
        PLX_FAIL(PLX_ERR_HIP, "filter table: device allocation/upload failed");
    }
    *d_out = d;
    return PLX_OK;
}

void plx_ssfm_geometry(const plx_ssfm *P, int *p1, int *p2) { *p1 = P->p1; *p2 = P->p2; }

int plx_ssfm_filter_dev(plx_ssfm *P, cplx *d_ux, cplx *d_uy, const cplx *d_hmul, int nframes, void *stream, const cplx *d_umat)
{
    if (!P || !d_ux || (!d_hmul && !d_umat)) PLX_FAIL(PLX_ERR_ARG, "filter: null argument");
    if (d_umat && (!P->a.dual || P->a.nfc != 1)) PLX_FAIL(PLX_ERR_ARG, "filter: matrix tables need a dual-polarisation single-field plan");
    if (nframes < 1 || nframes > P->d.max_frames) PLX_FAIL(PLX_ERR_ARG, "filter: nframes outside [1, max_frames]");
    if (P->a.dual && !d_uy) PLX_FAIL(PLX_ERR_ARG, "filter: dual-polarisation plan needs d_uy");
    hipStream_t st = (hipStream_t)stream;
    SsfmArgs b = P->a;
    b.ux = d_ux; b.uy = d_uy; b.nframes = nframes; b.hmul = d_hmul; b.umat = d_umat;
    b.force = 1; b.spm = 0; b.xpm = 0; b.pmd = 0; b.f_cur = 0; b.f_leff = 0; b.f_sc = b.invN;
    const int N1 = 1 << b.p1, N2 = 1 << b.p2;
    const unsigned FC = (unsigned)nframes * b.nfc;
    PLX_HIP(hipMemsetAsync(P->d_ctl, 0, sizeof(FrameCtl) * nframes, st));
    PLX_HIP(hipMemsetAsync(P->d_ndone, 0, 64, st));
    const dim3 gcol((unsigned)(N2 / b.W), FC), grow((unsigned)(N1 / b.R), FC);
    launch(col_fwd_kernel(), gcol, dim3((unsigned)P->col_threads), P->lds_col, st, b);
    if (d_umat && !P->tw_compact && !P->rowreg) launch(row_kernel(), grow, dim3((unsigned)P->row_threads), P->lds_row, st, b);
    else launch_row(P, b, FC, st);
    launch(col_inv_kernel(), gcol, dim3((unsigned)P->col_threads), P->lds_col, st, b);
    PLX_HIP(hipGetLastError());
    return PLX_OK;
}

int plx_ssfm_linear_dev(plx_ssfm *P, const SsfmArgs &base, cplx *d_x, double dz, hipStream_t st)
{
    SsfmArgs b = base;
    b.ux = d_x; b.uy = nullptr; b.nframes = 1; b.hmul = nullptr; b.umat = nullptr;
    b.force = 1; b.spm = 0; b.xpm = 0; b.f_cur = dz; b.f_leff = 0; b.f_sc = b.invN;
    const unsigned FC = (unsigned)b.nfc;
    const dim3 gcol((unsigned)((1 << b.p2) / b.W), FC);
    launch(col_fwd_kernel(), gcol, dim3((unsigned)P->col_threads), P->lds_col, st, b);
    launch_row(P, b, FC, st);
    launch(col_inv_kernel(), gcol, dim3((unsigned)P->col_threads), P->lds_col, st, b);
    const hipError_t e = hipGetLastError();
    if (e != hipSuccess) PLX_FAIL(PLX_ERR_HIP, std::string("linear step: launch failed: ") + hipGetErrorString(e));
    return PLX_OK;
}

extern "C" int plx_ssfm_results(plx_ssfm *P, int nframes, double *firstdz, int32_t *ncycle)
{
    if (!P || nframes < 1 || nframes > P->d.max_frames) PLX_FAIL(PLX_ERR_ARG, "plx_ssfm_results: bad argument");
    for (int f = 0; f < nframes; f++) {
        if (firstdz) firstdz[f] = P->h_ctl[f].firstdz;
        if (ncycle) ncycle[f] = P->h_ctl[f].ncycle;
    }
    return PLX_OK;
}

extern "C" int plx_ssfm_stats(plx_ssfm *P, int64_t *row_pass_launches, int64_t *sample_steps)
{
    if (!P) PLX_FAIL(PLX_ERR_ARG, "plx_ssfm_stats: null plan");
    if (row_pass_launches) *row_pass_launches = P->row_launches;
    if (sample_steps) *sample_steps = P->sample_steps;
    return PLX_OK;
}
```

polmux_amd/csrc/ssfm_row.hip:

```cpp
#include "ssfm_pmd.h"
#include "ssfm_kernels.h"
using namespace plxs;

namespace {

#define ROW_CH 4
__global__ __launch_bounds__(1024) void k_row(SsfmArgs a)
{
    PLX_DYN_LDS(lds);
    if (all_done_or_aborted(a)) return;
    const int tid = threadIdx.x, nthr = blockDim.x;
    int slot = blockIdx.y / a.nfc;
    const int c = blockIdx.y - slot * a.nfc;
    if (!row_slot(a, slot)) return;
    int f;
    if (!slot_frame(a, slot, f)) return;
    const int fc = f * a.nfc + c;
    const FrameCtl *ctl = a.ctl + f;
    if (ctl->done) return;
    const int N2 = 1 << a.p2, R = a.R, TSp = row_pitch(N2);
    cplx *s = (cplx *)lds;
    cplx *tw = s + (size_t)(a.dual ? 2 : 1) * R * TSp;
    const int twn = N2 >> 1;
    const bool tw_one = twn <= nthr;
    cplx twv = make_double2(0, 0);
    if (tw_one) { if (tid < twn) twv = a.tw2[tid]; }
    else lds_load_twiddles(tw, a.tw2, twn, tid, nthr);
    const size_t N = (size_t)1 << (a.p1 + a.p2);
    const int j0 = blockIdx.x * R;
    const int nel = R << a.p2;
    cplx *const fx = a.ux;
    cplx *const fy = a.dual ? a.uy : a.ux;
    const size_t base = (size_t)fc * N + (size_t)j0 * N2;
    auto gofs = [&](int e) -> size_t { return base + e; };
    const size_t rowbase = (size_t)j0 * N2;
    const bool keep_tw = nel == nthr * ROW_CH;
    cplx tkeep[ROW_CH];
    const double *bt = a.betat_p + (size_t)c * N + rowbase;
    const bool fastmul = keep_tw && a.dual && !a.pmd && !a.umat && !a.hmul;
    double btk[ROW_CH];
    if (fastmul) {
#pragma unroll
        for (int k = 0; k < ROW_CH; k++) btk[k] = bt[row_lane_point(tid + k * nthr, N2)];
    }
    for (int e0 = tid; e0 < nel; e0 += nthr * ROW_CH) {
        cplx tv[ROW_CH], xv[ROW_CH], yv[ROW_CH];
#pragma unroll
        for (int k = 0; k < ROW_CH; k++) {
            const int e = row_lane_point(min(e0 + k * nthr, nel - 1), N2);
            tv[k] = a.tpass[rowbase + e];
            xv[k] = fx[gofs(e)];
            yv[k] = fy[gofs(e)];
        }
#pragma unroll
        for (int k = 0; k < ROW_CH; k++) { pin(tv[k]); pin(xv[k]); pin(yv[k]); }
#pragma unroll
        for (int k = 0; k < ROW_CH; k++) {
            const int el = e0 + k * nthr, e = row_lane_point(el, N2);
            tkeep[k] = tv[k];
            if (el < nel) {
                const int r = e >> a.p2, i = e & (N2 - 1);
                s[r * TSp + row_phys(i)] = cmul(xv[k], tv[k]);
                if (a.dual) s[(R + r) * TSp + row_phys(i)] = cmul(yv[k], tv[k]);
            }
        }
    }
    if (tw_one && tid < twn) tw[tid] = twv;
    __syncthreads();
    row_fft_dif(s, a.p2, a.logR + (a.dual ? 1 : 0), tw, tid, nthr);
    const double cur = a.force ? a.f_cur : ctl->cur;
    if (!a.dual) {
        for (int el = tid; el < nel; el += nthr) {
            const int e = row_lane_point(el, N2);
            const int o = (e >> a.p2) * TSp + row_phys(e & (N2 - 1));
            s[o] = cmul(s[o], a.hmul ? a.hmul[rowbase + e] : cexp_neg_turns(bt[e] * cur));
        }
    } else if (!a.pmd) {
        if (a.umat) {
            for (int el = tid; el < nel; el += nthr) {
            const int e = row_lane_point(el, N2);
                const int o = (e >> a.p2) * TSp + row_phys(e & (N2 - 1));
                const cplx *um = a.umat + 3 * ((size_t)f * N + rowbase + e);
                const cplx u11 = um[0], u12 = um[1], hg = um[2], x = s[o], y = s[o + R * TSp];
                s[o] = cmulc(csub(cmulc(x, u11), cmul(u12, y)), hg);
                s[o + R * TSp] = cmulc(cadd(cmulc(x, u12), cmul(u11, y)), hg);
            }
        } else if (a.hmul) {
            for (int el = tid; el < nel; el += nthr) {
            const int e = row_lane_point(el, N2);
                const int o = (e >> a.p2) * TSp + row_phys(e & (N2 - 1));
                const cplx h = a.hmul[rowbase + e];
                s[o] = cmul(h, s[o]);
                s[o + R * TSp] = cmul(h, s[o + R * TSp]);
            }
        } else if (fastmul) {
#pragma unroll
            for (int k = 0; k < ROW_CH; k++) {
                const int e = row_lane_point(tid + k * nthr, N2);
                const int o = (e >> a.p2) * TSp + row_phys(e & (N2 - 1));
                const cplx h = cexp_neg_turns(btk[k] * cur);
                s[o] = cmul(h, s[o]);
                s[o + R * TSp] = cmul(h, s[o + R * TSp]);
            }
        } else {
            for (int el = tid; el < nel; el += nthr) {
            const int e = row_lane_point(el, N2);
                const int o = (e >> a.p2) * TSp + row_phys(e & (N2 - 1));
                const cplx h = cexp_neg_turns(bt[e] * cur);
                s[o] = cmul(h, s[o]);
                s[o + R * TSp] = cmul(h, s[o + R * TSp]);
            }
        }
    } else {
        const double *d1 = a.db1_p + (size_t)c * N + rowbase;
        const double *brf = a.brf + (a.brf_per_frame ? (size_t)f * a.nplates * BRF_STRIDE : 0);
        const int ntrunk = ctl->ntrunk, n0 = ctl->ntot - ctl->nmem;
        const double dzb_first = ctl->dzb_first, dzb_last = ctl->dzb_last, lcorr = a.lcorr;
        if (a.e1tab && ntrunk <= a.tmax) {
            const int N1 = 1 << a.p1;
            const cplx *e1 = a.e1tab + (size_t)f * a.tmax * N1 + j0, *e2 = a.e2tab + (size_t)f * a.tmax * N2;
            for (int el = tid; el < nel; el += nthr) {
                const int e = row_lane_point(el, N2);
                const int r = e >> a.p2, i = e & (N2 - 1);
                const int o = r * TSp + row_phys(i);
                cplx x = s[o], y = s[o + R * TSp];
                pmd_trunks_tab(x, y, bt[e], e1 + r, N1, e2 + i, N2, brf, a.nplates, n0, ntrunk, cur);
                s[o] = x;
                s[o + R * TSp] = y;
            }
        } else
        for (int el = tid; el < nel; el += nthr) {
            const int e = row_lane_point(el, N2);
            const int o = (e >> a.p2) * TSp + row_phys(e & (N2 - 1));
            cplx x = s[o], y = s[o + R * TSp];
            pmd_trunks(x, y, bt[e], d1[e], brf, a.nplates, n0, ntrunk, dzb_first, dzb_last, lcorr, cur);
            s[o] = x;
            s[o + R * TSp] = y;
        }
    }
    __syncthreads();
    row_fft_dit(s, a.p2, a.logR + (a.dual ? 1 : 0), tw, tid, nthr);
    if (keep_tw) {
#pragma unroll
        for (int k = 0; k < ROW_CH; k++) {
            const int e = row_lane_point(tid + k * nthr, N2);
            const int o = (e >> a.p2) * TSp + row_phys(e & (N2 - 1));
            fx[gofs(e)] = cmulc(s[o], tkeep[k]);
            if (a.dual) fy[gofs(e)] = cmulc(s[o + R * TSp], tkeep[k]);
        }
        return;
    }
    for (int el = tid; el < nel; el += nthr) {
            const int e = row_lane_point(el, N2);
        const int o = (e >> a.p2) * TSp + row_phys(e & (N2 - 1));
        const cplx t = a.tpass[rowbase + e];
        fx[gofs(e)] = cmulc(s[o], t);
        if (a.dual) fy[gofs(e)] = cmulc(s[o + R * TSp], t);
    }
}

}

namespace plxs {
sweep_kernel_t row_kernel() { return k_row; }
}
```

polmux_amd/csrc/ssfm_row256.hip:

```cpp
#include "ssfm_pmd.h"
#include "ssfm_kernels.h"
using namespace plxs;

namespace {

template <bool PMD, bool SC = false, bool SPLIT = false> __global__ __launch_bounds__(ROWR_THREADS, SPLIT ? 3 : 2) void k_row256r(SsfmArgs a)
{
    static_assert(!(PMD && SC), "PMD needs two polarisations");
    static_assert(!SPLIT || PMD, "the split form is the PMD kernel's");
    PLX_DYN_LDS(lds);
    if (all_done_or_aborted(a)) return;
    const int tid = threadIdx.x;
    int slot = blockIdx.y / a.nfc;
    const int c = blockIdx.y - slot * a.nfc;
    if (!row_slot(a, slot)) return;
    int f;
    if (!slot_frame(a, slot, f)) return;
    const int fc = f * a.nfc + c;
    const FrameCtl *ctl = a.ctl + f;
    if (ctl->done) return;
    cplx *const s = (cplx *)lds + (tid >> 4) * 272;
    double *const sd = (double *)lds + (tid >> 4) * 272;
    cplx *const tw = SPLIT ? (cplx *)((double *)lds + 4 * 272) : (cplx *)lds + 4 * 272;
    cplx *const bk = tw + 128 + 17 * (SC ? tid >> 4 : (tid >> 4) & 1);
    const Tw256half w8{tw};
    const int j = tid & 15, r = SC ? tid >> 4 : (tid >> 4) & 1;
    const size_t N = (size_t)1 << 16;
    const size_t rowbase = ((size_t)blockIdx.x * (SC ? 4 : 2) + r) << 8;
    cplx *const u = (!SC && tid >= 32 ? a.uy : a.ux) + (size_t)fc * N + rowbase;
    const cplx *const tp = a.tpass + rowbase;
    cplx x[16];
    cplx v1, v2, v3;
    {
        const cplx ta = tp[j];
#pragma unroll
        for (int k = 0; k < 16; k++) x[k] = u[j + 16 * k];
        if (!PMD) { v1 = a.tw2[4 * j]; v2 = a.tw2[8 * j]; v3 = tw3(a.tw2, 12 * j, 128); }
        {
            const cplx t0 = a.tw2[tid], t1 = a.tw2[tid + 64], t3 = tp[16 * j];
            tw[tid] = t0; tw[tid + 64] = t1;
            if (SC || tid < 32) bk[j] = t3;
        }
        ROWR_SYNC();
#pragma unroll
        for (int k = 0; k < 16; k++) x[k] = cmul(x[k], cmul(ta, bk[k]));
    }
    sched_fence();
    if (PMD) lvl2_dif<16>(x, j, w8); else lvl2_dif<16>(x, j, w8, v1, v2, v3);
    sched_fence();
    if (SPLIT) {
#pragma unroll
        for (int k = 0; k < 16; k++) sd[j + 17 * k] = x[k].x;
        ROWR_SYNC();
#pragma unroll
        for (int k = 0; k < 16; k++) x[k].x = sd[17 * j + k];
        ROWR_SYNC();
#pragma unroll
        for (int k = 0; k < 16; k++) sd[j + 17 * k] = x[k].y;
        ROWR_SYNC();
#pragma unroll
        for (int k = 0; k < 16; k++) x[k].y = sd[17 * j + k];
        ROWR_SYNC();
    } else {
#pragma unroll
        for (int k = 0; k < 16; k++) s[row_phys(j + 16 * k)] = x[k];
        ROWR_SYNC();
    }
    double btv[SC ? 16 : 8];
    if (!SPLIT) {
        const double *bt = a.betat_p + (size_t)c * N + rowbase + 16 * j + (!SC && tid >= 32 ? 8 : 0);
#pragma unroll
        for (int k = 0; k < (SC ? 16 : 8); k++) btv[k] = bt[k];
    }
    if (!SPLIT) {
#pragma unroll
        for (int k = 0; k < 16; k++) x[k] = s[17 * j + k];
    }
    r16_dif(x);
    sched_fence();
    if (PMD) {
        const double cur = ctl->cur;
        const int ib = 16 * j + (tid >= 32 ? 8 : 0);
        const size_t rowf = (size_t)blockIdx.x * 2 + r;
        const double *brf = a.brf + (a.brf_per_frame ? (size_t)f * a.nplates * BRF_STRIDE : 0);
        const int ntrunk = ctl->ntrunk, n0 = ctl->ntot - ctl->nmem;
#pragma unroll
        for (int k = 0; k < 8; k++) half_trade(x[k], x[k + 8]);
        if (SPLIT || (a.e1tab && ntrunk <= a.tmax)) {
            const cplx *e1 = a.e1tab + (size_t)f * a.tmax * 256 + rowf, *e2 = a.e2tab + (size_t)f * a.tmax * 256 + ib;
            for (int t = 0; t < ntrunk; t++) {
                int plate = n0 + t;
                plate = plate < 0 ? 0 : (plate >= a.nplates ? a.nplates - 1 : plate);
                const double *m = brf + (size_t)plate * BRF_STRIDE;
                const double s11 = m[0];
                const cplx s12 = make_double2(m[1], m[2]);
                const cplx e1v = e1[(size_t)t * 256];
                const cplx *e2t = e2 + (size_t)t * 256;
#pragma unroll
                for (int k = 0; k < 8; k++) {
                    const cplx e = cmul(e1v, e2t[k]);
                    const cplx u = x[k], v = x[k + 8];
                    const cplx sx = cadd(cscale(u, s11), cmul(s12, v));
                    const cplx sy = csub(cmulc(u, s12), cscale(v, s11));
                    x[k] = make_double2(e.x * u.x - e.y * sx.y, e.x * u.y + e.y * sx.x);
                    x[k + 8] = make_double2(e.x * v.x - e.y * sy.y, e.x * v.y + e.y * sy.x);
                    if (SPLIT && (k & 1)) sched_fence();
                }
            }
            if (SPLIT) {
                int o = ib;
                pin(o);
                const double *bt = a.betat_p + (size_t)c * N + rowbase + o;
#pragma unroll
                for (int k = 0; k < 8; k++) btv[k] = bt[k];
            }
#pragma unroll
            for (int k = 0; k < 8; k++) {
                const cplx h = cexp_neg_turns(btv[k] * cur);
                x[k] = cmul(h, x[k]);
                x[k + 8] = cmul(h, x[k + 8]);
                sched_fence();
            }
        } else if (!SPLIT) {
            const double *d1 = a.db1_p + (size_t)c * N + rowbase + ib;
            const double dzb_first = ctl->dzb_first, dzb_last = ctl->dzb_last;
            for (int k = 0; k < 8; k++) pmd_trunks(x[k], x[k + 8], btv[k], d1[k], brf, a.nplates, n0, ntrunk, dzb_first, dzb_last, a.lcorr, cur);
        }
#pragma unroll
        for (int k = 0; k < 8; k++) half_trade(x[k], x[k + 8]);
    } else if (SC) {
        const double cur = ctl->cur;
#pragma unroll
        for (int k = 0; k < (SC ? 16 : 8); k++) {
            x[k] = cmul(cexp_neg_turns(btv[k] * cur), x[k]);
            sched_fence();
        }
    } else {
        const double cur = ctl->cur;
#pragma unroll
        for (int k = 0; k < 8; k++) {
            const cplx h = cexp_neg_turns(btv[k] * cur);
            cplx ha, hb;
            half_share(h, ha, hb);
            x[k] = cmul(ha, x[k]);
            x[k + 8] = cmul(hb, x[k + 8]);
            sched_fence();
        }
    }
    sched_fence();
    r16_dit(x);
    sched_fence();
    if (!SPLIT) {
#pragma unroll
        for (int k = 0; k < 16; k++) s[17 * j + k] = x[k];
        ROWR_SYNC();
    }
    const cplx tb = tp[j];
    if (SPLIT) {
#pragma unroll
        for (int k = 0; k < 16; k++) sd[17 * j + k] = x[k].x;
        ROWR_SYNC();
#pragma unroll
        for (int k = 0; k < 16; k++) x[k].x = sd[j + 17 * k];
        ROWR_SYNC();
#pragma unroll
        for (int k = 0; k < 16; k++) sd[17 * j + k] = x[k].y;
        ROWR_SYNC();
#pragma unroll
        for (int k = 0; k < 16; k++) x[k].y = sd[j + 17 * k];
    } else {
#pragma unroll
        for (int k = 0; k < 16; k++) x[k] = s[row_phys(j + 16 * k)];
    }
    sched_fence();
    if (PMD) lvl2_dit<16>(x, j, w8); else lvl2_dit<16>(x, j, w8, v1, v2, v3);
    sched_fence();
#pragma unroll
    for (int k = 0; k < 16; k++) u[j + 16 * k] = cmulc(x[k], cmul(tb, bk[k]));
}

}

namespace plxs {
sweep_kernel_t row256_kernel(bool pmd, bool scalar, bool split)
{
    if (scalar) return (pmd || split) ? nullptr : (sweep_kernel_t)k_row256r<false, true>;
    if (split) return pmd ? (sweep_kernel_t)k_row256r<true, false, true> : nullptr;
    return pmd ? (sweep_kernel_t)k_row256r<true> : (sweep_kernel_t)k_row256r<false>;
}
}
```

polmux_amd/csrc/ssfm_row4k.hip:

```cpp
#include "ssfm_pmd.h"
#include "ssfm_kernels.h"
using namespace plxs;

namespace {

struct Tw256pad {
    const cplx *t;
    __device__ __forceinline__ cplx operator()(int e) const
    {
        const int i = e & 127;
        const cplx w = t[i + (i >> 2)];
        const bool neg = e >= 128;
        return make_double2(neg ? -w.x : w.x, neg ? -w.y : w.y);
    }
};
template <bool PAIR, bool SPLIT = false> __global__ __launch_bounds__(PAIR ? 512 : 256, PAIR ? 1 : (SPLIT ? 3 : 2)) void k_row4k(SsfmArgs a)
{
    static_assert(!(PAIR && SPLIT), "the split exchange belongs to the one-polarisation form");
    PLX_DYN_LDS(lds);
    if (all_done_or_aborted(a)) return;
    const int tid = PAIR ? (int)((threadIdx.x >> 6) * 32u + (threadIdx.x & 31u)) : (int)threadIdx.x;
    const int ts = threadIdx.x;
    const int K = (int)(gridDim.x >> a.p1), lg = a.p1 < 3 ? a.p1 : 3, G = 1 << lg;
    const bool unit_fc = PAIR || a.uy == nullptr;
    int brow, by, bpol;
    if (K >= (unit_fc ? 16 : 32)) {
        const int g8 = (int)blockIdx.x / (G * K), rem = (int)blockIdx.x - g8 * G * K, bk2 = rem >> lg;
        brow = g8 * G + (rem & (G - 1)); by = unit_fc ? bk2 : bk2 >> 1; bpol = unit_fc ? 0 : bk2 & 1;
    } else if (unit_fc) {
        const int N1 = 1 << a.p1;
        brow = (int)blockIdx.x & (N1 - 1); by = (int)blockIdx.x >> a.p1; bpol = 0;
    } else {
        const int N1 = 1 << a.p1, q = (int)blockIdx.x >> a.p1, FCn = K >> 1;
        brow = (int)blockIdx.x & (N1 - 1); bpol = q / FCn; by = q - bpol * FCn;
    }
    if (PAIR) bpol = (int)((threadIdx.x >> 5) & 1u);
    int slot = by / a.nfc;
    const int c = by - slot * a.nfc;
    if (!row_slot(a, slot)) return;
    int f;
    if (!slot_frame(a, slot, f)) return;
    const int fc = f * a.nfc + c;
    const FrameCtl *ctl = a.ctl + f;
    if (ctl->done) return;
    cplx *s = (cplx *)lds + (PAIR ? bpol * 4352 : 0);
    double *const sd = (double *)lds;
    cplx *tw = SPLIT ? (cplx *)((double *)lds + 4352) : (cplx *)lds + (PAIR ? 2 : 1) * 4352;
    cplx *bk = tw + 516;
    cplx *t8 = bk + 16;
    cplx *ct = t8 + 160;
    const size_t N = (size_t)1 << (a.p1 + a.p2);
    const size_t rowbase = (size_t)brow << 12;
    cplx *const u = (bpol ? a.uy : a.ux) + (size_t)fc * N + rowbase;
    const cplx *const tp = a.tpass + rowbase;

    const Tw4096 w1{tw};
    const Tw256pad w2{t8};
    const int b = tid >> 4, j2 = tid & 15;
    cplx x[16];
    auto exchange_split = [&](auto wi, auto ri, bool outer) {
#pragma unroll
        for (int k = 0; k < 16; k++) sd[wi(k)] = x[k].x;
        if (outer) __syncthreads(); else ROWR_SYNC();
#pragma unroll
        for (int k = 0; k < 16; k++) x[k].x = sd[ri(k)];
        if (outer) __syncthreads(); else ROWR_SYNC();
#pragma unroll
        for (int k = 0; k < 16; k++) sd[wi(k)] = x[k].y;
        if (outer) __syncthreads(); else ROWR_SYNC();
#pragma unroll
        for (int k = 0; k < 16; k++) x[k].y = sd[ri(k)];
        if (!outer) ROWR_SYNC();
    };
    const int obase = tid + (tid >> 4), cbase = 272 * b + j2, tbase = 17 * tid;
    const auto outerp = [&](int k) { return obase + 272 * k; };
    const auto chunkp = [&](int k) { return cbase + 17 * k; };
    const auto own16p = [&](int k) { return tbase + k; };
    {
        cplx ta = tp[tid];
#pragma unroll
        for (int k = 0; k < 16; k++) x[k] = u[tid + 256 * k];
        if (!PAIR || ts < 256) {
            const cplx t0 = a.tw2[ts], t1 = a.tw2[ts + 256], t2 = a.tw2[512 + (ts & 3)], t3 = tp[256 * (ts & 15)], t4 = a.tw2[4 * (ts & 127)];
            tw[ts] = t0; tw[ts + 256] = t1;
            if (ts < 4) tw[512 + ts] = t2;
            if (ts < 16) bk[ts] = t3;
            if (ts < 128) t8[ts + (ts >> 2)] = t4;
            if (ts < PLX_CTAB) ct[ts] = a.ctab[ts];
        }
#pragma unroll
        for (int k = 0; k < 16; k++) pin(x[k]);
        pin(ta);
        __syncthreads();
#pragma unroll
        for (int k = 0; k < 16; k++) x[k] = cmul(x[k], cmul(ta, bk[k]));
    }
    lvl2_dif<256>(x, tid, w1);
    if (SPLIT) exchange_split(outerp, chunkp, true);
    else {
#pragma unroll
        for (int k = 0; k < 16; k++) s[row_phys(tid + 256 * k)] = x[k];
        __syncthreads();
#pragma unroll
        for (int k = 0; k < 16; k++) x[k] = s[row_phys(256 * b + j2 + 16 * k)];
    }
    lvl2_dif<16>(x, j2, w2);
    if (SPLIT) exchange_split(chunkp, own16p, false);
    else {
#pragma unroll
        for (int k = 0; k < 16; k++) s[row_phys(256 * b + j2 + 16 * k)] = x[k];
        ROWR_SYNC();
    }
    const int ib = 16 * tid + (PAIR && bpol ? 8 : 0);
    double btv[PAIR ? 8 : 16];
    if (!SPLIT && !a.hmul && !(PAIR && a.umat)) {
        const double *bt = a.betat_p + (size_t)c * N + rowbase + ib;
#pragma unroll
        for (int k = 0; k < (PAIR ? 8 : 16); k++) btv[k] = bt[k];
    }
    if (!SPLIT) {
#pragma unroll
        for (int k = 0; k < 16; k++) x[k] = s[17 * tid + k];
    }
    r16_dif(x);
    if (PAIR && !a.hmul) {
        pair_multiplier<12>(a, x, btv, ct, ctl, f, c, brow, rowbase, ib);
    } else {
        if (a.hmul) {
            int o16 = 16 * tid;
            pin(o16);
            const cplx *h = a.hmul + rowbase + o16;
#pragma unroll
            for (int k = 0; k < 16; k++) x[k] = cmul(h[k], x[k]);
        } else {
            const double cur = a.force ? a.f_cur : ctl->cur;
            if (SPLIT) {
#pragma unroll
                for (int h = 0; h < 16; h += 8) {
                    int o = ib + h;
                    pin(o);
                    const double *bt = a.betat_p + (size_t)c * N + rowbase + o;
                    double bh[8];
#pragma unroll
                    for (int k = 0; k < 8; k++) bh[k] = bt[k];
#pragma unroll
                    for (int k = 0; k < 8; k++) x[h + k] = cmul(cexp_neg_turns_tab(bh[k] * cur, ct), x[h + k]);
                }
            } else
#pragma unroll
            for (int k = 0; k < (PAIR ? 8 : 16); k++) x[k] = cmul(cexp_neg_turns_tab(btv[k] * cur, ct), x[k]);
        }
    }
    r16_dit(x);
    if (SPLIT) exchange_split(own16p, chunkp, false);
    else {
#pragma unroll
        for (int k = 0; k < 16; k++) s[17 * tid + k] = x[k];
        ROWR_SYNC();
#pragma unroll
        for (int k = 0; k < 16; k++) x[k] = s[row_phys(256 * b + j2 + 16 * k)];
    }
    lvl2_dit<16>(x, j2, w2);
    if (!SPLIT) {
#pragma unroll
        for (int k = 0; k < 16; k++) s[row_phys(256 * b + j2 + 16 * k)] = x[k];
        __syncthreads();
    }
    int jo = tid;
    pin(jo);
    int rq = brow, pq = bpol, fq = fc;
    if (SPLIT) { pin(rq); pin(pq); pin(fq); }
    const size_t rowbase2 = SPLIT ? (size_t)rq << 12 : rowbase;
    cplx *const u2 = SPLIT ? (pq ? a.uy : a.ux) + ((size_t)fq << (a.p1 + 12)) + rowbase2 : u;
    const cplx tb = (SPLIT ? a.tpass + rowbase2 : tp)[jo];
    if (SPLIT) exchange_split(chunkp, outerp, true);
    else {
#pragma unroll
        for (int k = 0; k < 16; k++) x[k] = s[row_phys(tid + 256 * k)];
    }
    lvl2_dit<256>(x, SPLIT ? jo : tid, w1);
#pragma unroll
    for (int k = 0; k < 16; k++) u2[jo + 256 * k] = cmulc(x[k], cmul(tb, bk[k]));
}

}

namespace plxs {
sweep_kernel_t row4k_kernel(bool pair, bool split)
{
    if (pair) return split ? nullptr : (sweep_kernel_t)k_row4k<true>;
    return split ? (sweep_kernel_t)k_row4k<false, true> : (sweep_kernel_t)k_row4k<false>;
}
}
```

polmux_amd/csrc/ssfm_rowreg.hip:

```cpp
#include "ssfm_pmd.h"
#include "ssfm_kernels.h"
using namespace plxs;

namespace {

template <int LOGM, bool PAIR, bool SC = false, bool SPLIT = false> __global__ __launch_bounds__(ROWG_THREADS, SPLIT ? 3 : 2) void k_rowreg(SsfmArgs a)
{
    static_assert(!(PAIR && SC), "a scalar plan has no second polarisation to pair with");
    constexpr bool HALF_TW = LOGM <= 10;
    constexpr int M = 1 << LOGM, S = M / 16, R = M / 256, RP = ROWG_THREADS / S, PITCH = M + M / 16, NTW = ROWG_NTW(M);
    PLX_DYN_LDS(lds);
    if (all_done_or_aborted(a)) return;
    const int tid = threadIdx.x;
    int slot = blockIdx.y / a.nfc;
    const int c = blockIdx.y - slot * a.nfc;
    if (!row_slot(a, slot)) return;
    int f;
    if (!slot_frame(a, slot, f)) return;
    const int fc = f * a.nfc + c;
    const FrameCtl *ctl = a.ctl + f;
    if (ctl->done) return;
    constexpr int WPR = S / 32 > 0 ? S / 32 : 1;
    const int rl = PAIR ? (tid >> 6) / WPR : (SC ? tid / S : (tid / S) >> 1), pol = PAIR ? (tid >> 5) & 1 : (SC ? 0 : (tid / S) & 1);
    const int t = PAIR ? ((tid >> 6) % WPR) * 32 + (tid & 31) : tid % S;
    const int rp = SC ? rl : 2 * rl + pol;
    constexpr int ROWS = SC ? RP : RP / 2;
    constexpr bool WAVE_LOCAL = PAIR ? S <= 32 : S <= 64;
    cplx *const s = (cplx *)lds + rp * PITCH;
    double *const sd = (double *)lds + rp * PITCH;
    cplx *const tw = SPLIT ? (cplx *)((double *)lds + RP * PITCH) : (cplx *)lds + RP * PITCH;
    cplx *const tm = tw + NTW;
    cplx *const ct = tm + 7 * 16;
    cplx *const bk = ct + PLX_CTAB + 17 * rl;
    const size_t N = (size_t)M << a.p1;
    const size_t rowbase = ((size_t)blockIdx.x * ROWS + rl) << LOGM;
    cplx *const u = (pol ? a.uy : a.ux) + (size_t)fc * N + rowbase;
    const cplx *const tp = a.tpass + rowbase;
    typename std::conditional<HALF_TW, TwHalf<M>, TwCompact<M>>::type wm{tw};
    const int b = t >> 4, j2 = t & 15;
    cplx x[16];
    auto exchange_split = [&](auto wi, auto ri, bool block = false) {
#pragma unroll
        for (int k = 0; k < 16; k++) sd[wi(k)] = x[k].x;
        if (block) __syncthreads(); else ROWR_SYNC();
#pragma unroll
        for (int k = 0; k < 16; k++) x[k].x = sd[ri(k)];
        if (block) __syncthreads(); else ROWR_SYNC();
#pragma unroll
        for (int k = 0; k < 16; k++) sd[wi(k)] = x[k].y;
        if (block) __syncthreads(); else ROWR_SYNC();
#pragma unroll
        for (int k = 0; k < 16; k++) x[k].y = sd[ri(k)];
        if (!block) ROWR_SYNC();
    };
    const int obase = t + (t >> 4), cbase = 272 * b + j2, tbase = 17 * t;
    const auto outer = [&](int k) { return obase + (S + S / 16) * k; };
    const auto chunk = [&](int k) { return cbase + 17 * k; };
    const auto own16 = [&](int k) { return tbase + k; };
    {
        const cplx ta = tp[t];
#pragma unroll
        for (int k = 0; k < 16; k++) x[k] = u[t + S * k];
        for (int i = tid; i < NTW; i += ROWG_THREADS) tw[i] = HALF_TW ? a.tw2[i] : a.tw2c[i];
        if (tid < 7 * 16) tm[tid] = a.twmid[tid];
        if (tid < PLX_CTAB) ct[tid] = a.ctab[tid];
        if (pol == 0 && t < 16) bk[t] = tp[S * t];
        __syncthreads();
#pragma unroll
        for (int k = 0; k < 16; k++) x[k] = cmul(x[k], cmul(ta, bk[k]));
    }
    lvl2_dif<S>(x, t, wm);
    if (SPLIT) exchange_split(outer, chunk, !WAVE_LOCAL);
    else {
#pragma unroll
        for (int k = 0; k < 16; k++) s[row_phys(t + S * k)] = x[k];
        if (!WAVE_LOCAL) __syncthreads(); else ROWR_SYNC();
#pragma unroll
        for (int k = 0; k < 16; k++) x[k] = s[row_phys(256 * b + j2 + 16 * k)];
    }
    cplx wl[7];
#pragma unroll
    for (int q = 0; q < (R == 8 ? 7 : (R == 4 ? 3 : 1)); q++) wl[q] = tm[16 * q + j2];
    lvlmid_dif<R>(x, wl);
    if (SPLIT) exchange_split(chunk, own16);
    else {
#pragma unroll
        for (int k = 0; k < 16; k++) s[row_phys(256 * b + j2 + 16 * k)] = x[k];
        ROWR_SYNC();
    }
    constexpr bool SHARE = !PAIR && !SC && LOGM == 9, HALF_BINS = PAIR || SHARE;
    const int ib = 16 * t + (HALF_BINS && pol ? 8 : 0);
    double btv[HALF_BINS ? 8 : 16];
    constexpr bool LATE_BT = SPLIT && !HALF_BINS;
    if (!LATE_BT && !(PAIR && SPLIT) && !a.hmul && !(PAIR && a.umat)) {
        const double *bt = a.betat_p + (size_t)c * N + rowbase + ib;
#pragma unroll
        for (int k = 0; k < (HALF_BINS ? 8 : 16); k++) btv[k] = bt[k];
    }
    if (!SPLIT) {
#pragma unroll
        for (int k = 0; k < 16; k++) x[k] = s[17 * t + k];
    }
    r16_dif(x);
    if (PAIR && !a.hmul) {
        pair_multiplier<LOGM, SPLIT>(a, x, btv, ct, ctl, f, c, (int)blockIdx.x * ROWS + rl, rowbase, ib);
    } else if (a.hmul) {
        int o16 = 16 * t;
        pin(o16);
        const cplx *h = a.hmul + rowbase + o16;
#pragma unroll
        for (int k = 0; k < 16; k++) x[k] = cmul(h[k], x[k]);
    } else {
        const double cur = a.force ? a.f_cur : ctl->cur;
        if (SHARE) {
#pragma unroll
            for (int k = 0; k < 8; k++) {
                const cplx h = cexp_neg_turns_tab(btv[k] * cur, ct);
                cplx ha, hb;
                half_share(h, ha, hb);
                x[k] = cmul(ha, x[k]);
                x[k + 8] = cmul(hb, x[k + 8]);
            }
        } else if (LATE_BT) {
#pragma unroll
            for (int h = 0; h < 16; h += 8) {
                int o = ib + h;
                pin(o);
                const double *bt = a.betat_p + (size_t)c * N + rowbase + o;
                double bh[8];
#pragma unroll
                for (int k = 0; k < 8; k++) bh[k] = bt[k];
#pragma unroll
                for (int k = 0; k < 8; k++) x[h + k] = cmul(cexp_neg_turns_tab(bh[k] * cur, ct), x[h + k]);
            }
        } else {
#pragma unroll
            for (int k = 0; k < (HALF_BINS ? 8 : 16); k++) x[k] = cmul(cexp_neg_turns_tab(btv[k] * cur, ct), x[k]);
        }
    }
    r16_dit(x);
    if (SPLIT) exchange_split(own16, chunk);
    else {
#pragma unroll
        for (int k = 0; k < 16; k++) s[17 * t + k] = x[k];
        ROWR_SYNC();
#pragma unroll
        for (int k = 0; k < 16; k++) x[k] = s[row_phys(256 * b + j2 + 16 * k)];
    }
    {
        int jq = j2;
        pin(jq);
#pragma unroll
        for (int q = 0; q < (R == 8 ? 7 : (R == 4 ? 3 : 1)); q++) wl[q] = tm[16 * q + jq];
    }
    lvlmid_dit<R>(x, wl);
    if (!SPLIT) {
#pragma unroll
        for (int k = 0; k < 16; k++) s[row_phys(256 * b + j2 + 16 * k)] = x[k];
        if (!WAVE_LOCAL) __syncthreads(); else ROWR_SYNC();
    }
    int jo = t;
    pin(jo);
    int rq = rl, pq = pol, fq = fc;
    if (SPLIT) { pin(rq); pin(pq); pin(fq); }
    const size_t rowbase2 = SPLIT ? ((size_t)blockIdx.x * ROWS + rq) << LOGM : rowbase;
    cplx *const u2 = SPLIT ? (pq ? a.uy : a.ux) + ((size_t)fq << (LOGM + a.p1)) + rowbase2 : u;
    const cplx tb = (SPLIT ? a.tpass + rowbase2 : tp)[jo];
    if (SPLIT) exchange_split(chunk, outer, !WAVE_LOCAL);
    else {
#pragma unroll
        for (int k = 0; k < 16; k++) x[k] = s[row_phys(t + S * k)];
    }
    lvl2_dit<S>(x, (PAIR || SPLIT) ? jo : t, wm);
#pragma unroll
    for (int k = 0; k < 16; k++) u2[jo + S * k] = cmulc(x[k], cmul(tb, bk[k]));
}
}

namespace plxs {
namespace {
template <int LOGM> sweep_kernel_t rowreg_pick(bool pair, bool scalar, bool split)
{
    if (pair) return scalar ? nullptr : (split ? (sweep_kernel_t)k_rowreg<LOGM, true, false, true> : (sweep_kernel_t)k_rowreg<LOGM, true>);
    if (scalar) return split ? (sweep_kernel_t)k_rowreg<LOGM, false, true, true> : (sweep_kernel_t)k_rowreg<LOGM, false, true>;
    return split ? (sweep_kernel_t)k_rowreg<LOGM, false, false, true> : (sweep_kernel_t)k_rowreg<LOGM, false>;
}
}
sweep_kernel_t rowreg_kernel(int logm, bool pair, bool scalar, bool split)
{
    return logm == 9 ? rowreg_pick<9>(pair, scalar, split) : logm == 10 ? rowreg_pick<10>(pair, scalar, split) : logm == 11 ? rowreg_pick<11>(pair, scalar, split) : nullptr;
}
}
```

polmux_amd/csrc/ssfm_rowsm.hip:

```cpp
#include "ssfm_kernels.h"
using namespace plxs;

namespace {

template <int LOGM, bool SC> __global__ __launch_bounds__(64, 3) void k_rowsm(SsfmArgs a)
{
    constexpr int M = 1 << LOGM, R = M / 16, NS = 16 / R, RPW = 64 / R, NQ = R == 8 ? 7 : (R == 4 ? 3 : 1);
    PLX_DYN_LDS(lds);
    if (all_done_or_aborted(a)) return;
    const int tid = threadIdx.x;
    int slot = blockIdx.y / a.nfc;
    const int c = blockIdx.y - slot * a.nfc;
    if (!row_slot(a, slot)) return;
    int f;
    if (!slot_frame(a, slot, f)) return;
    const int fc = f * a.nfc + c;
    const FrameCtl *ctl = a.ctl + f;
    if (ctl->done) return;
    const int g = tid / R, j = tid - g * R;
    const int rp = (int)blockIdx.x * RPW + g, row = SC ? rp : rp >> 1, pol = SC ? 0 : rp & 1;
    double *const sd = (double *)lds + g * (17 * R);
    cplx *const tm = (cplx *)((double *)lds + 64 * 17);
    cplx *const ct = tm + 7 * 16;
    const size_t N = (size_t)M << a.p1;
    const size_t rowbase = (size_t)row << LOGM;
    cplx *const u = (pol ? a.uy : a.ux) + (size_t)fc * N + rowbase;
    const cplx *const tp = a.tpass + rowbase;
    cplx x[16];
#pragma unroll
    for (int k = 0; k < 16; k++) x[R * (k % NS) + k / NS] = u[j + R * k];
    tm[tid] = a.twmid[tid];
    if (tid < 7 * 16 - 64) tm[64 + tid] = a.twmid[64 + tid];
    ct[tid] = a.ctab[tid];
    {
        cplx tv[16];
#pragma unroll
        for (int k = 0; k < 16; k++) tv[k] = tp[j + R * k];
#pragma unroll
        for (int k = 0; k < 16; k++) x[R * (k % NS) + k / NS] = cmul(x[R * (k % NS) + k / NS], tv[k]);
    }
    ROWR_SYNC();
#pragma unroll
    for (int par = 0; par < NS; par++) {
        cplx w[7];
#pragma unroll
        for (int q = 0; q < NQ; q++) w[q] = tm[16 * q + j + R * par];
        radset_dif<R>(x + R * par, w);
    }
#pragma unroll
    for (int k = 0; k < 16; k++) sd[j + R * (k / R) + 17 * (k % R)] = x[k].x;
    ROWR_SYNC();
#pragma unroll
    for (int k = 0; k < 16; k++) x[k].x = sd[17 * j + k];
    ROWR_SYNC();
#pragma unroll
    for (int k = 0; k < 16; k++) sd[j + R * (k / R) + 17 * (k % R)] = x[k].y;
    ROWR_SYNC();
#pragma unroll
    for (int k = 0; k < 16; k++) x[k].y = sd[17 * j + k];
    ROWR_SYNC();
    r16_dif(x);
    if (a.hmul) {
        const cplx *h = a.hmul + rowbase + 16 * j;
#pragma unroll
        for (int k = 0; k < 16; k++) x[k] = cmul(h[k], x[k]);
    } else {
        const double cur = a.force ? a.f_cur : ctl->cur;
#pragma unroll
        for (int h = 0; h < 16; h += 8) {
            int o = 16 * j + h;
            pin(o);
            const double *bt = a.betat_p + (size_t)c * N + rowbase + o;
            double bh[8];
#pragma unroll
            for (int k = 0; k < 8; k++) bh[k] = bt[k];
#pragma unroll
            for (int k = 0; k < 8; k++) x[h + k] = cmul(cexp_neg_turns_tab(bh[k] * cur, ct), x[h + k]);
        }
    }
    r16_dit(x);
#pragma unroll
    for (int k = 0; k < 16; k++) sd[17 * j + k] = x[k].x;
    ROWR_SYNC();
#pragma unroll
    for (int k = 0; k < 16; k++) x[k].x = sd[j + R * (k / R) + 17 * (k % R)];
    ROWR_SYNC();
#pragma unroll
    for (int k = 0; k < 16; k++) sd[17 * j + k] = x[k].y;
    ROWR_SYNC();
#pragma unroll
    for (int k = 0; k < 16; k++) x[k].y = sd[j + R * (k / R) + 17 * (k % R)];
#pragma unroll
    for (int par = 0; par < NS; par++) {
        cplx w[7];
#pragma unroll
        for (int q = 0; q < NQ; q++) w[q] = tm[16 * q + j + R * par];
        radset_dit<R>(x + R * par, w);
    }
    {
        int jo = j;
        pin(jo);
        cplx tv[16];
#pragma unroll
        for (int k = 0; k < 16; k++) tv[k] = tp[jo + R * k];
#pragma unroll
        for (int k = 0; k < 16; k++) u[jo + R * k] = cmulc(x[R * (k % NS) + k / NS], tv[k]);
    }
}
}

namespace plxs {
sweep_kernel_t rowsm_kernel(int logm, bool scalar)
{
    if (scalar) return logm == 5 ? (sweep_kernel_t)k_rowsm<5, true> : logm == 6 ? (sweep_kernel_t)k_rowsm<6, true> : logm == 7 ? (sweep_kernel_t)k_rowsm<7, true> : nullptr;
    return logm == 5 ? (sweep_kernel_t)k_rowsm<5, false> : logm == 6 ? (sweep_kernel_t)k_rowsm<6, false> : logm == 7 ? (sweep_kernel_t)k_rowsm<7, false> : nullptr;
}
}
```

polmux_amd/csrc/ssfm_small.hip:

```cpp
#include "ssfm_ctrl.h"
#include "ssfm_kernels.h"
using namespace plxs;

namespace {

__global__ __launch_bounds__(256) void k_umax(SsfmArgs a)
{
    PLX_DYN_LDS(lds);
    double *red = (double *)lds;
    const int fc = blockIdx.y;
    const size_t N = (size_t)1 << (a.p1 + a.p2);
    const cplx *x = a.ux + (size_t)fc * N;
    const cplx *y = a.dual ? a.uy + (size_t)fc * N : nullptr;
    double m = 0;
    for (size_t i = (size_t)blockIdx.x * blockDim.x + threadIdx.x; i < N; i += (size_t)gridDim.x * blockDim.x) {
        cplx v = x[i];
        double p = v.x * v.x + v.y * v.y;
        if (y) {
            cplx w = y[i];
            p = p + w.x * w.x;
            p = p + w.y * w.y;
        }
        m = p > m ? p : m;
    }
    block_atomic_max(m, red, a.umax + fc, threadIdx.x, blockDim.x);
}

__global__ __launch_bounds__(64) void k_ctrl(SsfmArgs a, int nframes)
{
    const int f = blockIdx.x * blockDim.x + threadIdx.x;
    if (f >= nframes) return;
    ctrl_step<false>(a, f);
}

__global__ __launch_bounds__(COMPACT_THREADS) void k_compact(const FrameCtl *ctl, int nframes, int *active, int *nactive, int serves)
{
    PLX_DYN_LDS(lds);
    int *cnt = (int *)lds;
    const int tid = threadIdx.x, per = (nframes + COMPACT_THREADS - 1) / COMPACT_THREADS;
    const int f0 = tid * per, f1 = min(nframes, f0 + per);
    int n = 0;
    for (int f = f0; f < f1; f++) n += ctl[f].done ? 0 : 1;
    cnt[tid] = n;
    __syncthreads();
    for (int d = 1; d < COMPACT_THREADS; d <<= 1) {
        const int v = tid >= d ? cnt[tid - d] : 0;
        __syncthreads();
        cnt[tid] += v;
        __syncthreads();
    }
    int o = cnt[tid] - n;
    for (int f = f0; f < f1; f++)
        if (!ctl[f].done) active[o++] = f;
    if (tid == COMPACT_THREADS - 1) { nactive[0] = cnt[tid]; nactive[1] += cnt[tid] * serves; }
}

__global__ __launch_bounds__(256) void k_nl_att(cplx *u, const double *gam, size_t N, int nfc, int spm, int xpm,
                                                double leff, double att)
{
    for (size_t i = (size_t)blockIdx.x * blockDim.x + threadIdx.x; i < N; i += (size_t)gridDim.x * blockDim.x) {
        double tot = 0;
        if (xpm)
            for (int k = 0; k < nfc; k++) {
                const cplx v = u[(size_t)k * N + i];
                tot += v.x * v.x + v.y * v.y;
            }
        for (int k = 0; k < nfc; k++) {
            cplx v = u[(size_t)k * N + i];
            if (spm || xpm) {
                double pw = v.x * v.x + v.y * v.y;
                if (xpm) pw = spm ? 2 * tot - pw : 2 * (tot - pw);
                v = cmul(v, cexpi(-gam[k] * pw * leff));
            }
            u[(size_t)k * N + i] = cscale(v, att);
        }
    }
}

__global__ __launch_bounds__(256) void k_maxdiff(const cplx *u, const cplx *uh, size_t n, unsigned long long *out)
{
    PLX_DYN_LDS(lds);
    double *red = (double *)lds;
    double m = 0;
    for (size_t i = (size_t)blockIdx.x * blockDim.x + threadIdx.x; i < n; i += (size_t)gridDim.x * blockDim.x) {
        const double dr = u[i].x - uh[i].x, di = u[i].y - uh[i].y;
        const double e = sqrt(dr * dr + di * di);
        m = e > m ? e : m;
    }
    block_atomic_max(m, red, out, threadIdx.x, blockDim.x);
}

__global__ __launch_bounds__(256) void k_richardson(cplx *u, const cplx *uh, size_t n)
{
    const double c43 = 4.0 / 3, c13 = 1.0 / 3;
    for (size_t i = (size_t)blockIdx.x * blockDim.x + threadIdx.x; i < n; i += (size_t)gridDim.x * blockDim.x)
        u[i] = make_double2(c43 * uh[i].x - c13 * u[i].x, c43 * uh[i].y - c13 * u[i].y);
}

__global__ __launch_bounds__(256) void k_rowsum(SsfmArgs a)
{
    const int f = blockIdx.y;
    if (a.ctl[f].done) return;
    const size_t N = (size_t)1 << (a.p1 + a.p2);
    for (size_t i = (size_t)blockIdx.x * blockDim.x + threadIdx.x; i < N; i += (size_t)gridDim.x * blockDim.x) {
        double sum = 0;
        for (int k = 0; k < a.nfc; k++) {
            cplx v = a.ux[((size_t)f * a.nfc + k) * N + i];
            sum += v.x * v.x + v.y * v.y;
        }
        a.psum[(size_t)f * N + i] = sum;
    }
}

#define STOKES_CH 4
__global__ __launch_bounds__(256) void k_stokes_sum(SsfmArgs a)
{
    const int f = blockIdx.y;
    if (a.ctl[f].done) return;
    const size_t N = (size_t)1 << (a.p1 + a.p2);
    const cplx *ux = a.ux + (size_t)f * a.nfc * N, *uy = a.uy + (size_t)f * a.nfc * N;
    cplx *rec = a.stokes + 2 * (size_t)f * N;
    for (size_t i = (size_t)blockIdx.x * blockDim.x + threadIdx.x; i < N; i += (size_t)gridDim.x * blockDim.x) {
        double axx = 0, ayy = 0, axr = 0, axi = 0;
        int k = 0;
        for (; k + STOKES_CH <= a.nfc; k += STOKES_CH) {
            cplx xv[STOKES_CH], yv[STOKES_CH];
#pragma unroll
            for (int j = 0; j < STOKES_CH; j++) { xv[j] = ux[(size_t)(k + j) * N + i]; yv[j] = uy[(size_t)(k + j) * N + i]; }
#pragma unroll
            for (int j = 0; j < STOKES_CH; j++) { pin(xv[j]); pin(yv[j]); }
#pragma unroll
            for (int j = 0; j < STOKES_CH; j++) {
                const cplx x = xv[j], y = yv[j];
                axx += x.x * x.x + x.y * x.y;
                ayy += y.x * y.x + y.y * y.y;
                axr += x.x * y.x + x.y * y.y;
                axi += x.y * y.x - x.x * y.y;
            }
        }
        for (; k < a.nfc; k++) {
            const cplx x = ux[(size_t)k * N + i], y = uy[(size_t)k * N + i];
            axx += x.x * x.x + x.y * x.y;
            ayy += y.x * y.x + y.y * y.y;
            axr += x.x * y.x + x.y * y.y;
            axi += x.y * y.x - x.x * y.y;
        }
        rec[2 * i] = make_double2(axx, ayy);
        rec[2 * i + 1] = make_double2(axr, axi);
    }
}

__global__ __launch_bounds__(256) void k_pmd_tab(SsfmArgs a)
{
    if (all_done_or_aborted(a)) return;
    int f;
    if (!slot_frame(a, blockIdx.x, f)) return;
    const FrameCtl *ctl = a.ctl + f;
    if (ctl->done) return;
    const int N1 = 1 << a.p1, N2 = 1 << a.p2;
    const int ntrunk = ctl->ntrunk, n0 = ctl->ntot - ctl->nmem;
    if (ntrunk > a.tmax) return;
    const double *brf = a.brf + (a.brf_per_frame ? (size_t)f * a.nplates * BRF_STRIDE : 0);
    const double lcorr = a.lcorr, rl = 1.0 / lcorr;
    cplx *e1 = a.e1tab + (size_t)f * a.tmax * N1, *e2 = a.e2tab + (size_t)f * a.tmax * N2;
    for (int k = 1; k <= ntrunk; k++) {
        int plate = n0 + k - 1;
        plate = plate < 0 ? 0 : (plate >= a.nplates ? a.nplates - 1 : plate);
        const double db0 = brf[(size_t)plate * BRF_STRIDE + 3];
        const double dzk = (k == 1) ? ctl->dzb_first : (k == ntrunk ? ctl->dzb_last : lcorr);
        const double na = 0.5 * a.d1slope * dzk, qa = na * rl, A = fma(fma(-lcorr, qa, na), rl, qa);
        const double nb = 0.5 * db0 * dzk, qb = nb * rl, B = fma(fma(-lcorr, qb, nb), rl, qb);
        for (int j = threadIdx.x; j < N1; j += blockDim.x)
            e1[(size_t)(k - 1) * N1 + j] = cexp_neg_turns(fma(A, (double)plx_bitrev((unsigned)j, a.p1), B));
        for (int i = threadIdx.x; i < N2; i += blockDim.x) {
            const int k2 = (int)plx_bitrev((unsigned)i, a.p2), m2 = k2 >= (N2 >> 1) ? k2 - N2 : k2;
            e2[(size_t)(k - 1) * N2 + i] = cexp_neg_turns(A * (double)((long long)N1 * m2));
        }
    }
}

}

namespace plxs {
void launch_umax(dim3 grid, hipStream_t st, const SsfmArgs &a) { PLX_LAUNCH(k_umax, grid, dim3(256), 16 * sizeof(double), st, a); }
void launch_ctrl(int nframes, hipStream_t st, const SsfmArgs &a) { PLX_LAUNCH(k_ctrl, dim3((unsigned)((nframes + 63) / 64)), dim3(64), 0, st, a, nframes); }
void launch_compact(const FrameCtl *ctl, int nframes, int *active, int *nactive, int serves, hipStream_t st)
{
    PLX_LAUNCH(k_compact, dim3(1), dim3(COMPACT_THREADS), COMPACT_THREADS * sizeof(int), st, ctl, nframes, active, nactive, serves);
}
void launch_rowsum(dim3 grid, hipStream_t st, const SsfmArgs &a) { PLX_LAUNCH(k_rowsum, grid, dim3(256), 0, st, a); }
void launch_stokes_sum(dim3 grid, hipStream_t st, const SsfmArgs &a) { PLX_LAUNCH(k_stokes_sum, grid, dim3(256), 0, st, a); }
void launch_pmd_tab(unsigned frames, hipStream_t st, const SsfmArgs &a) { PLX_LAUNCH(k_pmd_tab, dim3(frames), dim3(256), 0, st, a); }
void launch_nl_att(unsigned grid, hipStream_t st, cplx *u, const double *gam, size_t N, int nfc, int spm, int xpm, double leff, double att)
{
    PLX_LAUNCH(k_nl_att, dim3(grid), dim3(256), 0, st, u, gam, N, nfc, spm, xpm, leff, att);
}
void launch_maxdiff(unsigned grid, hipStream_t st, const cplx *u, const cplx *uh, size_t n, unsigned long long *out)
{
    PLX_LAUNCH(k_maxdiff, dim3(grid), dim3(256), 16 * sizeof(double), st, u, uh, n, out);
}
void launch_richardson(unsigned grid, hipStream_t st, cplx *u, const cplx *uh, size_t n) { PLX_LAUNCH(k_richardson, dim3(grid), dim3(256), 0, st, u, uh, n); }
}
```

Before: 0.6556.

## Fold active-list compaction into row kernel tail and bound host step chunking

The separate compact kernel launched per step is replaced by a wave in block 0 of the row kernel that rebuilds the next active frame list into a double-buffered list. It also estimates the remaining steps, which the host uses to shrink its chunk size near the end and so avoid launching wasted steps. The per-call memsets are merged into one init kernel, and the control code precomputes -1/alpha and an alpha==0 flag. The row kernels gain a prologue, and the list is built from control state while other blocks may still be updating it, which could race. Debug logging and probe entry points are added as well.

```diff
diff --git a/include/polmux_hip.h b/include/polmux_hip.h
--- a/include/polmux_hip.h
+++ b/include/polmux_hip.h
@@ -64,7 +64,9 @@
     int32_t store_late;
     int32_t row_rev;
     int32_t safe_landing;
-    int32_t reserved_[4];
+    int32_t row_tail;
+    int32_t step_bound;
+    int32_t reserved_[2];
     double barrier_timeout_ms;
 } plx_ssfm_tuning;
 int plx_ssfm_tuning_defaults(plx_ssfm_tuning *tuning);
@@ -79,6 +81,9 @@
 int plx_ssfm_set_step_sequence(plx_ssfm *plan, const double *dz, int nsteps);
 int plx_ssfm_log_steps(plx_ssfm *plan, int max_steps);
 int plx_ssfm_step_sequence(plx_ssfm *plan, int frame, double *dz, int max_steps);
+int plx_ssfm_ctrl_probe(plx_ssfm *plan, int n, const double *umax, const double *zprop, double *out);
+int plx_ssfm_log_active(plx_ssfm *plan, int max_steps);
+int plx_ssfm_active_log(plx_ssfm *plan, int step, int which, int32_t *count, int32_t *list);
 int plx_ssfm_results(plx_ssfm *plan, int nframes, double *firstdz, int32_t *ncycle);
 int plx_ssfm_stats(plx_ssfm *plan, int64_t *row_pass_launches, int64_t *sample_steps);
 int plx_ssfm_utilisation(plx_ssfm *plan, int64_t *frame_steps, int64_t *slots_listed, int64_t *slots_launched);
diff --git a/polmux_amd/_abi.py b/polmux_amd/_abi.py
--- a/polmux_amd/_abi.py
+++ b/polmux_amd/_abi.py
@@ -34,7 +34,8 @@
     _fields_ = [("size", C.c_uint32), ("no_fuse", C.c_int32), ("short_rows", C.c_int32), ("no_row_split", C.c_int32),
                 ("p1", C.c_int32), ("logW", C.c_int32), ("col_threads", C.c_int32), ("rowr", C.c_int32), ("rowsm", C.c_int32),
                 ("row256_split", C.c_int32), ("row4k_split", C.c_int32), ("rowg_split", C.c_int32), ("no_pmd_tab", C.c_int32),
-                ("store_late", C.c_int32), ("row_rev", C.c_int32), ("safe_landing", C.c_int32), ("reserved_", C.c_int32 * 4),
+                ("store_late", C.c_int32), ("row_rev", C.c_int32), ("safe_landing", C.c_int32), ("row_tail", C.c_int32),
+                ("step_bound", C.c_int32), ("reserved_", C.c_int32 * 2),
                 ("barrier_timeout_ms", C.c_double)]
 
 
@@ -82,6 +83,9 @@
     "plx_ssfm_set_step_sequence": [_vp, _vp, C.c_int],
     "plx_ssfm_log_steps": [_vp, C.c_int],
     "plx_ssfm_step_sequence": [_vp, C.c_int, _vp, C.c_int],
+    "plx_ssfm_ctrl_probe": [_vp, C.c_int, _vp, _vp, _vp],
+    "plx_ssfm_log_active": [_vp, C.c_int],
+    "plx_ssfm_active_log": [_vp, C.c_int, C.c_int, C.POINTER(_i32), _vp],
     "plx_ssfm_set_birefringence": [_vp, _vp, _vp, _vp, C.c_int],
     "plx_ssfm_set_birefringence_dev": [_vp, _vp, _vp, _vp, C.c_int, _vp],
     "plx_ssfm_propagate_dev": [_vp, _vp, _vp, C.c_int, _vp],
diff --git a/polmux_amd/csrc/ssfm_args.h b/polmux_amd/csrc/ssfm_args.h
--- a/polmux_amd/csrc/ssfm_args.h
+++ b/polmux_amd/csrc/ssfm_args.h
@@ -49,6 +49,8 @@
     int *ndone;
     const int *active;
     int *nactive;
+    int *next_active, *next_nactive;
+    int *loopw;
     long long spin_ticks;
     unsigned long long *slots;
     int row_rev;
@@ -69,6 +71,8 @@
     int resume, ncycle0;
     double dz0, zdone0;
     double alphalin, Lf, dzmax, dphimax, lcorr, invN;
+    double ninv_alpha;
+    int alpha0;
 };
 
 __device__ __forceinline__ double wave_max(double v)
@@ -97,6 +101,46 @@
     if (slot >= n) return false;
     slot = n - 1 - slot;
     return true;
+}
+
+static __device__ __noinline__ void rebuild_active(const FrameCtl *ctl, int nframes, int *next_active, int *next_nactive, int *loopw,
+                                                   double Lf, double dzmax, double alphalin, int est)
+{
+    const int lane = threadIdx.x, per = (nframes + 63) >> 6;
+    const int f0 = min(lane * per, nframes), f1 = min(nframes, f0 + per);
+    int n = 0, need = 0;
+    for (int f = f0; f < f1; f++) {
+        const FrameCtl *c = ctl + f;
+        if (c->done) continue;
+        n++;
+        if (!est) continue;
+        int s = 1;
+        if (!c->last) {
+            const double dz = c->dz, rem = Lf - c->zprop;
+            double q = ceil(rem / dz);
+            if (dz < dzmax) {
+                const double g = ceil(exp(-alphalin * dz) * ((1 - exp(-alphalin * rem)) / alphalin) / c->leff);
+                q = g < q ? g : q;
+            }
+            s = (q >= 1 && q < 1e6 ? (int)q : 1000000) + 1;
+        }
+        need = max(need, s);
+    }
+    int incl = n;
+    for (int d = 1; d < 64; d <<= 1) {
+        const int v = __shfl(incl, (lane - d) & 63, 64);
+        if (lane >= d) incl += v;
+    }
+    for (int m = 32; m >= 1; m >>= 1) need = max(need, __shfl_xor(need, m, 64));
+    int o = incl - n;
+    for (int f = f0; f < f1; f++)
+        if (!ctl[f].done) next_active[o++] = f;
+    if (lane == 63) { next_nactive[0] = incl; loopw[0] += incl; loopw[1] = est ? need : -1; }
+}
+__device__ __forceinline__ void row_tail(const SsfmArgs &a)
+{
+    if (!a.next_active || blockIdx.x != 0 || blockIdx.y != 0 || threadIdx.x >= 64) return;
+    rebuild_active(a.ctl, a.nframes, a.next_active, a.next_nactive, a.loopw, a.Lf, a.dzmax, a.alphalin, (!a.alpha0 && !(a.dzlist && a.ndz > 0)) ? 1 : 0);
 }
 
 __device__ __forceinline__ void sincos_small(double a, double *s, double *c)
diff --git a/polmux_amd/csrc/ssfm_colx.hip b/polmux_amd/csrc/ssfm_colx.hip
--- a/polmux_amd/csrc/ssfm_colx.hip
+++ b/polmux_amd/csrc/ssfm_colx.hip
@@ -6,7 +6,7 @@
 
 __device__ __noinline__ double ctrl_head_call(const PLX_LDS_QUAL CtrlK *k, PLX_LDS_QUAL FrameCtl *rec, int count, double pmax, int f)
 {
-    if (!ctrl_head<true>(*k, f, *rec, true, pmax, count != 0)) return -1.0;
+    if (!ctrl_head<true, false>(*k, f, *rec, true, pmax, count != 0)) return -1.0;
     return rec->leff;
 }
 __device__ __noinline__ void ctrl_tail_call(const PLX_LDS_QUAL CtrlK *k, PLX_LDS_QUAL FrameCtl *rec)
@@ -145,8 +145,8 @@
     CtrlK *const kk = (CtrlK *)(lctl + 8);
     if (tid == 0) {
         red[8] = -1.0;
-        kk->dphimax = a.dphimax; kk->alphalin = a.alphalin; kk->dzmax = a.dzmax; kk->dz0 = a.dz0; kk->zdone0 = a.zdone0; kk->Lf = a.Lf; kk->lcorr = a.lcorr;
-        kk->dual = a.dual ? 1 : 0; kk->resume = a.resume ? 1 : 0; kk->ncycle0 = a.ncycle0; kk->nfc = 0; kk->ndone = a.ndone; kk->umax = nullptr; kk->gam = nullptr;
+        kk->dphimax = a.dphimax; kk->alphalin = a.alphalin; kk->ninv_alpha = a.ninv_alpha; kk->dzmax = a.dzmax; kk->dz0 = a.dz0; kk->zdone0 = a.zdone0; kk->Lf = a.Lf; kk->lcorr = a.lcorr;
+        kk->dual = a.dual ? 1 : 0; kk->resume = a.resume ? 1 : 0; kk->ncycle0 = a.ncycle0; kk->alpha0 = a.alpha0; kk->ndone = a.ndone;
         kk->dzlist = a.dzlist; kk->dzlog = a.dzlog; kk->ndz = a.ndz; kk->logcap = a.logcap;
     }
     auto settle = [&](int par) {
diff --git a/polmux_amd/csrc/ssfm_ctrl.h b/polmux_amd/csrc/ssfm_ctrl.h
--- a/polmux_amd/csrc/ssfm_ctrl.h
+++ b/polmux_amd/csrc/ssfm_ctrl.h
@@ -3,7 +3,7 @@
 
 namespace plxs {
 
-template <bool AGENT, class ARGS, class REC> __device__ __forceinline__ bool ctrl_head(const ARGS &a, int f, REC &c, bool have_pmax, double pmax_in, bool count = true)
+template <bool AGENT, bool GATHER = true, class ARGS, class REC> __device__ __forceinline__ bool ctrl_head(const ARGS &a, int f, REC &c, bool have_pmax, double pmax_in, bool count = true)
 {
     if (c.started) {
         if (a.dual) c.ntot = c.ntot + c.ntrunk - c.nmem;
@@ -14,9 +14,9 @@
         }
     }
     double Pmax = -INFINITY;
-    if (have_pmax) {
+    if (have_pmax || !GATHER) {
         Pmax = pmax_in;
-    } else {
+    } else if constexpr (GATHER) {
         for (int k = 0; k < a.nfc; k++) {
             unsigned long long *up = a.umax + f * a.nfc + k;
             const unsigned long long bits = AGENT ? ld_agent(up) : *up;
@@ -32,7 +32,7 @@
     if (dl >= 1) {
         dz = a.dzmax;
     } else {
-        double step = (a.alphalin == 0) ? leffn : -1 / a.alphalin * log(1 - dl);
+        double step = a.alpha0 ? leffn : a.ninv_alpha * log(1 - dl);
         dz = step > a.dzmax ? a.dzmax : step;
     }
     {
@@ -62,7 +62,7 @@
     } else {
         c.cur = a.Lf - c.zprop + dz; c.last = 1;
     }
-    c.leff = (a.alphalin == 0) ? c.cur : (1 - exp(-a.alphalin * c.cur)) / a.alphalin;
+    c.leff = a.alpha0 ? c.cur : (1 - exp(-a.alphalin * c.cur)) / a.alphalin;
     return true;
 }
 template <class ARGS, class REC> __device__ __forceinline__ void ctrl_tail(const ARGS &a, REC &c)
@@ -99,11 +99,9 @@
     if (ctrl_head<AGENT>(a, f, c, have_pmax, pmax_in)) ctrl_tail(a, c);
 }
 struct CtrlK {
-    double dphimax, alphalin, dzmax, dz0, zdone0, Lf, lcorr;
-    int dual, resume, ncycle0, nfc;
+    double dphimax, alphalin, ninv_alpha, dzmax, dz0, zdone0, Lf, lcorr;
+    int dual, resume, ncycle0, alpha0;
     int *ndone;
-    unsigned long long *umax;
-    const double *gam;
     const double *dzlist;
     double *dzlog;
     int ndz, logcap;
diff --git a/polmux_amd/csrc/ssfm_kernels.h b/polmux_amd/csrc/ssfm_kernels.h
--- a/polmux_amd/csrc/ssfm_kernels.h
+++ b/polmux_amd/csrc/ssfm_kernels.h
@@ -34,6 +34,7 @@
 PLX_HIDDEN void launch_umax(dim3 grid, hipStream_t st, const SsfmArgs &a);
 PLX_HIDDEN void launch_ctrl(int nframes, hipStream_t st, const SsfmArgs &a);
 PLX_HIDDEN void launch_compact(const FrameCtl *ctl, int nframes, int *active, int *nactive, int serves, hipStream_t st);
+PLX_HIDDEN void launch_call_init(const SsfmArgs &a, unsigned FC, size_t nslots, size_t nmbox, int *ndone, int *active, int *nactive, int serves, hipStream_t st);
 PLX_HIDDEN void launch_rowsum(dim3 grid, hipStream_t st, const SsfmArgs &a);
 PLX_HIDDEN void launch_stokes_sum(dim3 grid, hipStream_t st, const SsfmArgs &a);
 PLX_HIDDEN void launch_pmd_tab(unsigned frames, hipStream_t st, const SsfmArgs &a);
diff --git a/polmux_amd/csrc/ssfm_plan.h b/polmux_amd/csrc/ssfm_plan.h
--- a/polmux_amd/csrc/ssfm_plan.h
+++ b/polmux_amd/csrc/ssfm_plan.h
@@ -17,6 +17,10 @@
     int *d_ndone = nullptr;
     int *h_ndone = nullptr;
     int *d_active = nullptr;
+    int row_tail = 1;
+    int step_bound = 1;
+    struct ActiveLog { std::vector<int> tail, ref; int ntail = 0, nref = 0; };
+    std::vector<ActiveLog> alog;
     hipEvent_t ev = nullptr;
     std::vector<FrameCtl> h_ctl;
     int brf_sets = 0;
diff --git a/polmux_amd/csrc/ssfm_plan.hip b/polmux_amd/csrc/ssfm_plan.hip
--- a/polmux_amd/csrc/ssfm_plan.hip
+++ b/polmux_amd/csrc/ssfm_plan.hip
@@ -55,7 +55,7 @@
     std::memset(t, 0, sizeof(*t));
     t->size = (uint32_t)sizeof(*t);
     t->p1 = -1; t->logW = -1; t->col_threads = -1; t->store_late = -1;
-    t->row_rev = 1; t->rowr = 1; t->rowsm = 1; t->row256_split = 1; t->row4k_split = 1; t->rowg_split = 1;
+    t->row_rev = 1; t->row_tail = 1; t->step_bound = 1; t->rowr = 1; t->rowsm = 1; t->row256_split = 1; t->row4k_split = 1; t->rowg_split = 1;
     t->barrier_timeout_ms = 500.0;
     if (const char *e = getenv("PLX_SSFM_NO_FUSE")) t->no_fuse = atoi(e);
     if (const char *e = getenv("PLX_SSFM_BARRIER_TIMEOUT_MS")) t->barrier_timeout_ms = atof(e);
@@ -155,6 +155,10 @@
     a.nplates = desc->nplates;
     a.alphalin = desc->alphalin; a.Lf = desc->length; a.dzmax = desc->dzmaxt; a.dphimax = desc->dphimaxt;
     a.lcorr = desc->length / desc->nplates;
+    a.ninv_alpha = -1 / desc->alphalin;
+    a.alpha0 = desc->alphalin == 0 ? 1 : 0;
+    P->row_tail = tune.row_tail;
+    P->step_bound = tune.step_bound ? 1 : 0;
     a.invN = 1.0 / (double)N;
     a.spin_ticks = (long long)(tune.barrier_timeout_ms * 1e5);
     a.safe_land = tune.safe_landing;
@@ -262,7 +266,7 @@
     bool ok = hipMalloc((void **)&P->d_ctl, sizeof(FrameCtl) * F) == hipSuccess &&
               hipMalloc((void **)&P->d_umax, sizeof(unsigned long long) * F * nfc) == hipSuccess &&
               hipMalloc((void **)&P->d_ndone, 64) == hipSuccess &&
-              hipMalloc((void **)&P->d_active, sizeof(int) * (size_t)F) == hipSuccess &&
+              hipMalloc((void **)&P->d_active, sizeof(int) * 3 * (size_t)F) == hipSuccess &&
               hipHostMalloc((void **)&P->h_ndone, 64, hipHostMallocDefault) == hipSuccess &&
               hipEventCreateWithFlags(&P->ev, hipEventDisableTiming) == hipSuccess;
     if (ok && !a.dual && a.xpm) ok = hipMalloc((void **)&P->d_psum, sizeof(double) * (size_t)F * N) == hipSuccess;
@@ -450,7 +454,7 @@
             return;
         }
         for (int pol = 0; pol < 2; pol++) {
-            if (pol) b.ux = a.uy;
+            if (pol) { b.ux = a.uy; b.next_active = nullptr; }
             launch(row_kernel(), gs, bs, P->rs_lds, st, b);
         }
         return;
@@ -485,6 +489,20 @@
     return PLX_OK;
 }
 
+static int log_active(plx_ssfm *P, const SsfmArgs &a, int nframes, int step, hipStream_t st)
+{
+    int *const ref = P->d_active + 2 * (size_t)P->d.max_frames;
+    launch_compact(a.ctl, nframes, ref, P->d_ndone + 8, 0, st);
+    plx_ssfm::ActiveLog &l = P->alog[step];
+    l.tail.assign(nframes, -1); l.ref.assign(nframes, -1);
+    PLX_HIP(hipMemcpyAsync(l.tail.data(), a.next_active, sizeof(int) * nframes, hipMemcpyDeviceToHost, st));
+    PLX_HIP(hipMemcpyAsync(l.ref.data(), ref, sizeof(int) * nframes, hipMemcpyDeviceToHost, st));
+    PLX_HIP(hipMemcpyAsync(&l.ntail, a.next_nactive, sizeof(int), hipMemcpyDeviceToHost, st));
+    PLX_HIP(hipMemcpyAsync(&l.nref, P->d_ndone + 8, sizeof(int), hipMemcpyDeviceToHost, st));
+    PLX_HIP(hipStreamSynchronize(st));
+    return PLX_OK;
+}
+
 static int propagate_frames(plx_ssfm *P, cplx *d_ux, cplx *d_uy, int nframes, hipStream_t st)
 {
     SsfmArgs a = P->a;
@@ -495,21 +513,21 @@
     a.active = P->d_active;
     a.nactive = P->d_ndone + 2;
     unsigned FC = (unsigned)nframes * nfc;
-    PLX_HIP(hipMemsetAsync(a.ctl, 0, sizeof(FrameCtl) * nframes, st));
-    PLX_HIP(hipMemsetAsync(a.umax, 0, sizeof(unsigned long long) * FC, st));
-    PLX_HIP(hipMemsetAsync(P->d_ndone, 0, 64, st));
     const bool fused = P->fused != 0;
-    if (fused) {
-        PLX_HIP(hipMemsetAsync(P->d_slots, 0xFF, sizeof(unsigned long long) * 2 * (size_t)nframes * P->tiles_pf, st));
-        PLX_HIP(hipMemsetAsync(P->d_mbox, 0, P->mbox_bytes, st));
-    } else {
+    const bool compact_every_step = nframes >= 64 || P->row_tail == 2;
+    launch_call_init(a, FC, fused ? 2 * (size_t)nframes * P->tiles_pf : 0, fused ? P->mbox_bytes / sizeof(unsigned long long) : 0,
+                     P->d_ndone, P->d_active, P->d_ndone + 2, compact_every_step ? 1 : 4, st);
+    if (!fused) {
         unsigned gx = (unsigned)((P->N + 255) / 256);
         if (gx > 64) gx = 64;
         launch_umax(dim3(gx, FC), st, a);
     }
     const dim3 blk(256);
     const dim3 bcol((unsigned)P->col_threads);
-    const bool compact_every_step = nframes >= 64;
+    const bool tail = fused && compact_every_step && P->row_tail;
+    int *const lists[2] = {P->d_active, P->d_active + P->d.max_frames};
+    int *const lens[2] = {P->d_ndone + 2, P->d_ndone + 5};
+    if (tail) a.loopw = P->d_ndone + 3;
     int chunk = 4, steps = 0;
     const int kMaxSteps = 1 << 19;
     bool pending = false, aborted = false;
@@ -536,7 +554,12 @@
             if (fused) {
                 const int tcx = (int)gcol.x, tct = (int)(gcol.x * FC);
                 const dim3 gx((unsigned)(tct < P->fused_grid ? tct : P->fused_grid));
-                if (compact_every_step || sidx == 0) {
+                if (tail) {
+                    const int par = (steps + sidx) & 1;
+                    a.active = lists[par]; a.nactive = lens[par];
+                    a.next_active = lists[par ^ 1]; a.next_nactive = lens[par ^ 1];
+                }
+                if (!tail && steps + sidx > 0 && (compact_every_step || sidx == 0)) {
                     PLX_MARK(3, steps + sidx);
                     launch_compact(a.ctl, nframes, P->d_active, P->d_ndone + 2, compact_every_step ? 1 : chunk, st);
                 }
@@ -556,11 +579,15 @@
                 PLX_MARK(1, steps + sidx);
                 launch_row(P, a, FC, st);
                 P->row_launches++;
+                if (tail && steps + sidx < (int)P->alog.size()) {
+                    const int rc_ = log_active(P, a, nframes, steps + sidx, st);
+                    if (rc_) return rc_;
+                }
                 continue;
             }
             PLX_MARK(3, steps + sidx);
             launch_ctrl(nframes, st, a);
-            if (compact_every_step || sidx == 0)
+            if (steps + sidx > 0 && (compact_every_step || sidx == 0))
                 launch_compact(a.ctl, nframes, P->d_active, P->d_ndone + 2, compact_every_step ? 1 : chunk, st);
             if (!a.dual && a.xpm) {
                 unsigned gx = (unsigned)((P->N + 255) / 256);
@@ -594,15 +621,21 @@
             const unsigned live = (unsigned)(nframes - P->h_ndone[0]) * nfc;
             if (live < FC) FC = live;
         }
-        PLX_HIP(hipMemcpyAsync(P->h_ndone, P->d_ndone, 4 * sizeof(int), hipMemcpyDeviceToHost, st));
+        int to_come = -1;
+        if (tail && P->step_bound && pending && P->h_ndone[4] >= 0) to_come = P->h_ndone[4] > chunk ? P->h_ndone[4] - chunk : 0;
+        PLX_HIP(hipMemcpyAsync(P->h_ndone, P->d_ndone, 8 * sizeof(int), hipMemcpyDeviceToHost, st));
         PLX_HIP(hipEventRecord(P->ev, st));
         pending = true;
         if (chunk > 8) chunk = 4;
         else if (chunk < (compact_every_step ? 8 : 16)) chunk *= 2;
+        if (to_come >= 0) {
+            const int want = to_come >= 4 ? to_come / 2 : 1;
+            if (want < chunk) chunk = want;
+        }
         if (steps > kMaxSteps) PLX_FAIL(PLX_ERR_HIP, "plx_ssfm_propagate_dev: step loop did not terminate");
     }
     PLX_HIP(hipMemcpyAsync(P->h_ctl.data(), a.ctl, sizeof(FrameCtl) * nframes, hipMemcpyDeviceToHost, st));
-    PLX_HIP(hipMemcpyAsync(P->h_ndone, P->d_ndone, 4 * sizeof(int), hipMemcpyDeviceToHost, st));
+    PLX_HIP(hipMemcpyAsync(P->h_ndone, P->d_ndone, 8 * sizeof(int), hipMemcpyDeviceToHost, st));
     PLX_HIP(hipStreamSynchronize(st));
     P->slots_listed += P->h_ndone[3];
     if (aborted || P->h_ndone[1]) {
@@ -666,6 +699,48 @@
         PLX_HIP(hipMalloc((void **)&P->d_dzlog, sizeof(double) * (size_t)max_steps * P->d.max_frames));
         P->a.dzlog = P->d_dzlog; P->a.logcap = max_steps;
     }
+    return PLX_OK;
+}
+
+extern "C" int plx_ssfm_ctrl_probe(plx_ssfm *P, int n, const double *umax, const double *zprop, double *out)
+{
+    if (!P || !umax || !zprop || !out || n < 1 || n > P->d.max_frames) PLX_FAIL(PLX_ERR_ARG, "plx_ssfm_ctrl_probe: bad argument");
+    SsfmArgs a = P->a;
+    a.nframes = n; a.active = nullptr; a.dzlist = nullptr; a.ndz = 0; a.dzlog = nullptr; a.logcap = 0;
+    std::vector<FrameCtl> rec((size_t)n);
+    std::vector<unsigned long long> um((size_t)n * a.nfc, 0ull);
+    std::memset(rec.data(), 0, sizeof(FrameCtl) * (size_t)n);
+    for (int f = 0; f < n; f++) {
+        rec[f].started = 1; rec[f].ncycle = 1; rec[f].zprop = zprop[f];
+        std::memcpy(&um[(size_t)f * a.nfc], &umax[f], sizeof(double));
+    }
+    PLX_HIP(hipMemcpy(a.ctl, rec.data(), sizeof(FrameCtl) * (size_t)n, hipMemcpyHostToDevice));
+    PLX_HIP(hipMemcpy(a.umax, um.data(), sizeof(unsigned long long) * um.size(), hipMemcpyHostToDevice));
+    PLX_HIP(hipMemset(P->d_ndone, 0, 64));
+    launch_ctrl(n, nullptr, a);
+    PLX_HIP(hipDeviceSynchronize());
+    PLX_HIP(hipMemcpy(rec.data(), a.ctl, sizeof(FrameCtl) * (size_t)n, hipMemcpyDeviceToHost));
+    for (int f = 0; f < n; f++) {
+        double *o = out + 6 * (size_t)f;
+        o[0] = rec[f].dz; o[1] = rec[f].cur; o[2] = rec[f].leff; o[3] = rec[f].att; o[4] = rec[f].zprop; o[5] = rec[f].last;
+    }
+    return PLX_OK;
+}
+
+extern "C" int plx_ssfm_log_active(plx_ssfm *P, int max_steps)
+{
+    if (!P || max_steps < 0) PLX_FAIL(PLX_ERR_ARG, "plx_ssfm_log_active: bad argument");
+    P->alog.assign((size_t)max_steps, plx_ssfm::ActiveLog());
+    return PLX_OK;
+}
+
+extern "C" int plx_ssfm_active_log(plx_ssfm *P, int step, int which, int32_t *count, int32_t *list)
+{
+    if (!P || !count || !list || step < 0 || step >= (int)P->alog.size()) PLX_FAIL(PLX_ERR_ARG, "plx_ssfm_active_log: bad argument");
+    const plx_ssfm::ActiveLog &l = P->alog[step];
+    const std::vector<int> &v = which ? l.ref : l.tail;
+    *count = v.empty() ? -1 : (which ? l.nref : l.ntail);
+    for (int k = 0; k < *count; k++) list[k] = v[k];
     return PLX_OK;
 }
 
diff --git a/polmux_amd/csrc/ssfm_row.hip b/polmux_amd/csrc/ssfm_row.hip
--- a/polmux_amd/csrc/ssfm_row.hip
+++ b/polmux_amd/csrc/ssfm_row.hip
@@ -8,6 +8,7 @@
 __global__ __launch_bounds__(1024) void k_row(SsfmArgs a)
 {
     PLX_DYN_LDS(lds);
+    row_tail(a);
     if (all_done_or_aborted(a)) return;
     const int tid = threadIdx.x, nthr = blockDim.x;
     int slot = blockIdx.y / a.nfc;
diff --git a/polmux_amd/csrc/ssfm_row256.hip b/polmux_amd/csrc/ssfm_row256.hip
--- a/polmux_amd/csrc/ssfm_row256.hip
+++ b/polmux_amd/csrc/ssfm_row256.hip
@@ -9,6 +9,7 @@
     static_assert(!(PMD && SC), "PMD needs two polarisations");
     static_assert(!SPLIT || PMD, "the split form is the PMD kernel's");
     PLX_DYN_LDS(lds);
+    row_tail(a);
     if (all_done_or_aborted(a)) return;
     const int tid = threadIdx.x;
     int slot = blockIdx.y / a.nfc;
diff --git a/polmux_amd/csrc/ssfm_row4k.hip b/polmux_amd/csrc/ssfm_row4k.hip
--- a/polmux_amd/csrc/ssfm_row4k.hip
+++ b/polmux_amd/csrc/ssfm_row4k.hip
@@ -18,6 +18,7 @@
 {
     static_assert(!(PAIR && SPLIT), "the split exchange belongs to the one-polarisation form");
     PLX_DYN_LDS(lds);
+    row_tail(a);
     if (all_done_or_aborted(a)) return;
     const int tid = PAIR ? (int)((threadIdx.x >> 6) * 32u + (threadIdx.x & 31u)) : (int)threadIdx.x;
     const int ts = threadIdx.x;
diff --git a/polmux_amd/csrc/ssfm_rowreg.hip b/polmux_amd/csrc/ssfm_rowreg.hip
--- a/polmux_amd/csrc/ssfm_rowreg.hip
+++ b/polmux_amd/csrc/ssfm_rowreg.hip
@@ -10,6 +10,7 @@
     constexpr bool HALF_TW = LOGM <= 10;
     constexpr int M = 1 << LOGM, S = M / 16, R = M / 256, RP = ROWG_THREADS / S, PITCH = M + M / 16, NTW = ROWG_NTW(M);
     PLX_DYN_LDS(lds);
+    row_tail(a);
     if (all_done_or_aborted(a)) return;
     const int tid = threadIdx.x;
     int slot = blockIdx.y / a.nfc;
diff --git a/polmux_amd/csrc/ssfm_rowsm.hip b/polmux_amd/csrc/ssfm_rowsm.hip
--- a/polmux_amd/csrc/ssfm_rowsm.hip
+++ b/polmux_amd/csrc/ssfm_rowsm.hip
@@ -7,6 +7,7 @@
 {
     constexpr int M = 1 << LOGM, R = M / 16, NS = 16 / R, RPW = 64 / R, NQ = R == 8 ? 7 : (R == 4 ? 3 : 1);
     PLX_DYN_LDS(lds);
+    row_tail(a);
     if (all_done_or_aborted(a)) return;
     const int tid = threadIdx.x;
     int slot = blockIdx.y / a.nfc;
diff --git a/polmux_amd/csrc/ssfm_small.hip b/polmux_amd/csrc/ssfm_small.hip
--- a/polmux_amd/csrc/ssfm_small.hip
+++ b/polmux_amd/csrc/ssfm_small.hip
@@ -53,6 +53,24 @@
     for (int f = f0; f < f1; f++)
         if (!ctl[f].done) active[o++] = f;
     if (tid == COMPACT_THREADS - 1) { nactive[0] = cnt[tid]; nactive[1] += cnt[tid] * serves; }
+}
+
+struct InitArgs {
+    unsigned long long *ctl, *umax, *ndone, *slots, *mbox;
+    size_t nctl, numax, nslots, nmbox;
+    int *active, *nactive;
+    int nframes, serves;
+};
+__global__ __launch_bounds__(256) void k_call_init(InitArgs i)
+{
+    const size_t t = (size_t)blockIdx.x * blockDim.x + threadIdx.x, n = (size_t)gridDim.x * blockDim.x;
+    for (size_t k = t; k < i.nctl; k += n) i.ctl[k] = 0ull;
+    for (size_t k = t; k < i.numax; k += n) i.umax[k] = 0ull;
+    for (size_t k = t; k < i.nslots; k += n) i.slots[k] = ~0ull;
+    for (size_t k = t; k < i.nmbox; k += n) i.mbox[k] = 0ull;
+    for (size_t k = t; k < (size_t)i.nframes; k += n) i.active[k] = (int)k;
+    if (t < 8) i.ndone[t] = 0ull;
+    if (t == 1) { i.nactive[0] = i.nframes; i.nactive[1] = i.nframes * i.serves; }
 }
 
 __global__ __launch_bounds__(256) void k_nl_att(cplx *u, const double *gam, size_t N, int nfc, int spm, int xpm,
@@ -188,6 +206,19 @@
 {
     PLX_LAUNCH(k_compact, dim3(1), dim3(COMPACT_THREADS), COMPACT_THREADS * sizeof(int), st, ctl, nframes, active, nactive, serves);
 }
+void launch_call_init(const SsfmArgs &a, unsigned FC, size_t nslots, size_t nmbox, int *ndone, int *active, int *nactive, int serves, hipStream_t st)
+{
+    InitArgs i;
+    i.ctl = (unsigned long long *)a.ctl; i.nctl = (size_t)a.nframes * (sizeof(FrameCtl) / 8);
+    i.umax = a.umax; i.numax = FC;
+    i.ndone = (unsigned long long *)ndone;
+    i.slots = a.slots; i.nslots = nslots;
+    i.mbox = a.mbox; i.nmbox = nmbox;
+    i.active = active; i.nactive = nactive; i.nframes = a.nframes; i.serves = serves;
+    const size_t most = i.nctl > i.nslots ? (i.nctl > i.nmbox ? i.nctl : i.nmbox) : (i.nslots > i.nmbox ? i.nslots : i.nmbox);
+    unsigned g = (unsigned)((most + 255) / 256);
+    PLX_LAUNCH(k_call_init, dim3(g < 1 ? 1 : (g > 512 ? 512 : g)), dim3(256), 0, st, i);
+}
 void launch_rowsum(dim3 grid, hipStream_t st, const SsfmArgs &a) { PLX_LAUNCH(k_rowsum, grid, dim3(256), 0, st, a); }
 void launch_stokes_sum(dim3 grid, hipStream_t st, const SsfmArgs &a) { PLX_LAUNCH(k_stokes_sum, grid, dim3(256), 0, st, a); }
 void launch_pmd_tab(unsigned frames, hipStream_t st, const SsfmArgs &a) { PLX_LAUNCH(k_pmd_tab, dim3(frames), dim3(256), 0, st, a); }
```

After: 0.6550. No clear change (-0.1%).
